# jiahuei/COMIC-Compact-Image-Captioning-with-Attention

Measured on NVIDIA B200. Metric: captions/sec COMIC-256 beam-3, higher is better.
Workload: dtype f32 storage and accumulation; GEMM / conv operands split into 3 bf16 terms on tcgen05 (bf16x3)

## Files before the change

### comic-compact-image-captioning-with-attention_b200/csrc/api.cu

```cuda
#include <stdarg.h>
#include <string.h>

#include <new>

#include "comic_internal.cuh"

namespace comic {

static thread_local char g_err[1024] = "";

void set_error(const char* fmt, ...) {
  va_list ap;
  va_start(ap, fmt);
  vsnprintf(g_err, sizeof(g_err), fmt, ap);
  va_end(ap);
}

}

using namespace comic;

extern "C" const char* comic_last_error(void) { return g_err; }
extern "C" const char* comic_version(void) { return "comic_b200 0.2 (sm_100a; fp32 FFMA + tcgen05 bf16x3)"; }

extern "C" int comic_create(const comic_cfg_t* cfg, comic_handle_t* out) {
  COMIC_REQUIRE(cfg && out, COMIC_E_BADARG, "create: null argument");
  COMIC_REQUIRE(cfg->rnn_size > 0 && cfg->rnn_size % 128 == 0, COMIC_E_UNSUPPORTED,
                "create: rnn_size %d must be a positive multiple of 128", cfg->rnn_size);
  COMIC_REQUIRE(cfg->word_size > 0 && cfg->word_size % 4 == 0, COMIC_E_UNSUPPORTED, "create: word_size %% 4 != 0");
  COMIC_REQUIRE(cfg->num_heads > 0 && cfg->rnn_size % cfg->num_heads == 0 &&
                    (cfg->rnn_size / cfg->num_heads) % 4 == 0,
                COMIC_E_UNSUPPORTED, "create: heads %d incompatible with rnn_size %d", cfg->num_heads, cfg->rnn_size);
  COMIC_REQUIRE(cfg->fm_channels > 0 && cfg->fm_channels % 4 == 0 && cfg->fm_positions > 0, COMIC_E_SHAPE,
                "create: bad feature map %d x %d", cfg->fm_positions, cfg->fm_channels);
  COMIC_REQUIRE(cfg->vocab > 1 && cfg->eos_id >= 0 && cfg->eos_id < cfg->vocab, COMIC_E_SHAPE, "create: bad vocab / eos");
  COMIC_REQUIRE(cfg->fm_projection >= 0 && cfg->fm_projection <= 2, COMIC_E_BADARG, "create: fm_projection");
  COMIC_REQUIRE(cfg->alignment == 0 || cfg->alignment == 1, COMIC_E_BADARG,
                "create: Invalid alignment method.");
  COMIC_REQUIRE(cfg->prob_fn == 0 || cfg->prob_fn == 1, COMIC_E_BADARG, "create: Invalid alignment method.");
  COMIC_REQUIRE(cfg->embed_size % 4 == 0, COMIC_E_SHAPE, "create: embed_size %% 4 != 0");
  comic_handle_s* h = new (std::nothrow) comic_handle_s();
  COMIC_REQUIRE(h, COMIC_E_BADARG, "create: out of host memory");
  h->cfg = *cfg;
  COMIC_CHECK_CUDA(cudaGetDevice(&h->dev));
  cudaDeviceProp prop;
  COMIC_CHECK_CUDA(cudaGetDeviceProperties(&prop, h->dev));
  h->num_sms = prop.multiProcessorCount;
  h->R = cfg->rnn_size; h->W = cfg->word_size; h->H = cfg->num_heads;
  h->C = cfg->fm_channels; h->M = cfg->fm_positions; h->E = cfg->embed_size; h->V = cfg->vocab;
  h->Vp = round_up(h->V, 4);
  h->VAL = (cfg->fm_projection == 0) ? h->C : h->R;
  h->A = (cfg->fm_projection == 0 && !cfg->context_layer) ? h->C : h->R;
  h->LQ = h->Vp + h->R;
  h->KX = h->W + h->A + h->R;
  if (h->VAL % h->H != 0) {
    delete h;
    set_error("create: value width %d not divisible by heads %d", h->VAL, h->H);
    return COMIC_E_SHAPE;
  }
  memset(&h->w, 0, sizeof(h->w));
  int rc = decoder_configure();
  if (rc) { delete h; return rc; }
  if (cudaMallocHost(&h->attn2_host, 16 * sizeof(float)) != cudaSuccess) {
    h->attn2_host = nullptr;
    (void)cudaGetLastError();
  }
  *out = h;
  return COMIC_OK;
}

extern "C" int comic_destroy(comic_handle_t h) {
  if (h && h->prof_ev) {
    for (int i = 0; i < 2 * kMaxProfEvents; ++i) cudaEventDestroy(h->prof_ev[i]);
    delete[] h->prof_ev;
    delete[] h->prof_tag;
  }
  if (h && h->attn2_host) cudaFreeHost(h->attn2_host);
  delete h;
  return COMIC_OK;
}

extern "C" int comic_profile_enable(comic_handle_t h, uint32_t tag_mask) {
  COMIC_REQUIRE(h, COMIC_E_BADARG, "profile_enable: null handle");
  if (tag_mask && !h->prof_ev) {
    h->prof_ev = new cudaEvent_t[2 * kMaxProfEvents];
    h->prof_tag = new int[kMaxProfEvents];
    for (int i = 0; i < 2 * kMaxProfEvents; ++i) COMIC_CHECK_CUDA(cudaEventCreate(&h->prof_ev[i]));
  }
  h->prof_mask = tag_mask;
  h->prof_used = 0;
  return COMIC_OK;
}

extern "C" int comic_profile_read(comic_handle_t h, int tag, double* total_ms, int64_t* count) {
  COMIC_REQUIRE(h && total_ms && count, COMIC_E_BADARG, "profile_read: null argument");
  double tot = 0.0;
  int64_t n = 0;
  for (int i = 0; i < h->prof_used; ++i) {
    if (h->prof_tag[i] != tag) continue;
    COMIC_CHECK_CUDA(cudaEventSynchronize(h->prof_ev[2 * i + 1]));
    float ms = 0.f;
    COMIC_CHECK_CUDA(cudaEventElapsedTime(&ms, h->prof_ev[2 * i], h->prof_ev[2 * i + 1]));
    tot += ms;
    ++n;
  }
  *total_ms = tot;
  *count = n;
  return COMIC_OK;
}

namespace comic {
int pack_tc_weight(comic_handle_t h, Carver& cv, const float* W, int K, int N, int ldw, int cin_src, int cin_dst,
                   tc::TcWeight& out, cudaStream_t st, bool dry, int gate_R) {
  (void)h;
  int ntaps = K / cin_src;
  int Kd = (cin_src == cin_dst) ? K : ntaps * cin_dst;
  out.N = N;
  out.K = Kd;
  out.Npad = round_up(N, 16);
  out.Kpad = round_up(Kd, tc::BK);
  size_t n = (size_t)out.Npad * out.Kpad;
  out.hi = cv.take<uint16_t>(n);
  out.lo = cv.take<uint16_t>(n);
  out.ready = false;
  if (dry) return COMIC_OK;
  tc::pack_bt_kernel<<<(unsigned)((n + 255) / 256), 256, 0, st>>>(W, K, N, ldw, out.hi, out.lo, out.Kpad, out.Npad,
                                                                 cin_src, cin_dst, gate_R);
  COMIC_CHECK_CUDA(cudaGetLastError());
  COMIC_REQUIRE(tc::make_weight_maps(out), COMIC_E_CUDA, "cuTensorMapEncodeTiled failed for a %d x %d weight", N, Kd);
  return COMIC_OK;
}
}

extern "C" int comic_set_precision(comic_handle_t h, int mode) {
  COMIC_REQUIRE(h && mode >= 0 && mode <= 2, COMIC_E_BADARG, "set_precision: mode must be 0 (f32), 1 (split tensor) or 2 (fast)");
  h->precision = mode;
  return COMIC_OK;
}

extern "C" int comic_set_option(comic_handle_t h, int option, int value) {
  COMIC_REQUIRE(h, COMIC_E_BADARG, "set_option: null handle");
  switch (option) {
    case COMIC_OPT_FUSED_ATTN_MIN_IMAGES: h->fused_min_images = value; return COMIC_OK;
    case COMIC_OPT_PERSISTENT_MAX_ROWS: h->persist_max_rows = value; return COMIC_OK;
    case COMIC_OPT_PERSISTENT_TRACE: h->persist_trace = value; return COMIC_OK;
    case COMIC_OPT_PERSISTENT_WATCHDOG_MS:
      if (value < 0) break;
      h->persist_watchdog_ms = value;
      return COMIC_OK;
    case COMIC_OPT_ENC_PLANES: h->enc_planes = value; return COMIC_OK;
    case COMIC_OPT_STEM_S2D: h->stem_s2d = value; return COMIC_OK;
    case COMIC_OPT_TC_MIN_ROWS: h->tc_min_rows = value; return COMIC_OK;
    case COMIC_OPT_TC_SPLITK: h->tc_splitk = value; return COMIC_OK;
    case COMIC_OPT_ATTN2: h->attn2 = value; return COMIC_OK;
    case COMIC_OPT_FUSE_LSTM: h->fuse_lstm = value; return COMIC_OK;
    case COMIC_OPT_TMA_A: h->tma_a = value; return COMIC_OK;
    case COMIC_OPT_GEMM_SMALL_TILES: tc::small_tiles() = value; return COMIC_OK;
    case COMIC_OPT_PDL: pdl_mode() = value; return COMIC_OK;
    case COMIC_OPT_GEMM_RESIDENT_B: tc::bres_mode() = value; return COMIC_OK;
    case COMIC_OPT_GEMM_PAIR: tc::pair_mode() = value; return COMIC_OK;
    case COMIC_OPT_GEMM_PAIR_MIN_TILES: tc::pair_min_tiles() = value; return COMIC_OK;
    case COMIC_OPT_GEMM_MC:
      if (value != 0 && value != 1 && value != 2 && value != 4) break;
      tc::mc_mode() = value;
      return COMIC_OK;
    case COMIC_OPT_ENC_CHUNK_STEM:
    case COMIC_OPT_ENC_CHUNK_28:
    case COMIC_OPT_ENC_CHUNK_14:
      COMIC_REQUIRE(value >= 1, COMIC_E_BADARG, "set_option: encoder chunk must be >= 1");
      h->enc_chunk[option - COMIC_OPT_ENC_CHUNK_STEM] = value;
      return COMIC_OK;
    default: break;
  }
  set_error("set_option: unknown option %d", option);
  return COMIC_E_BADARG;
}

extern "C" int comic_decode_trace(comic_handle_t h, int64_t* out, int max_steps, int* steps, void* stream) {
  COMIC_REQUIRE(h && out && steps, COMIC_E_BADARG, "decode_trace: null argument");
  int n = h->last_trace_steps < max_steps ? h->last_trace_steps : max_steps;
  *steps = n;
  if (n <= 0 || !h->last_trace) { *steps = 0; return COMIC_OK; }
  COMIC_CHECK_CUDA(cudaMemcpyAsync(out, h->last_trace, (size_t)n * 32 * sizeof(int64_t), cudaMemcpyDeviceToHost,
                                   (cudaStream_t)stream));
  COMIC_CHECK_CUDA(cudaStreamSynchronize((cudaStream_t)stream));
  return COMIC_OK;
}

extern "C" int comic_packed_bytes(comic_handle_t h, size_t* bytes) {
  COMIC_REQUIRE(h && bytes, COMIC_E_BADARG, "packed_bytes: null argument");
  Carver cv(nullptr);
  comic::Packed keep = h->pk;
  decoder_pack(h, cv, 0, true);
  encoder_pack(h, cv, 0, true);
  h->pk = keep;
  *bytes = cv.off + 256;
  return COMIC_OK;
}

extern "C" int comic_bind_weights(comic_handle_t h, const comic_weights_t* w, int with_cnn, void* packed,
                                  size_t packed_bytes, void* stream) {
  COMIC_REQUIRE(h && w && packed, COMIC_E_BADARG, "bind_weights: null argument");
  size_t need;
  comic_packed_bytes(h, &need);
  COMIC_REQUIRE(packed_bytes >= need, COMIC_E_WORKSPACE, "bind_weights: packed buffer %zu < %zu", packed_bytes, need);
  COMIC_REQUIRE(w->lstm_kernel && w->lstm_bias && w->init_weight && w->memory_kernel && w->query_kernel &&
                    w->out_kernel && w->out_bias && w->embedding_map,
                COMIC_E_BADARG, "bind_weights: missing decoder tensor");
  if (h->cfg.alignment == 0)
    COMIC_REQUIRE(w->attention_v && w->ln_gamma && w->ln_beta && w->temperature, COMIC_E_BADARG,
                  "bind_weights: missing add_LN attention tensor");
  if (h->cfg.fm_projection == 2) COMIC_REQUIRE(w->value_kernel, COMIC_E_BADARG, "bind_weights: missing value_layer");
  if (h->cfg.context_layer) COMIC_REQUIRE(w->a_layer, COMIC_E_BADARG, "bind_weights: missing a_layer");
  if (with_cnn) {
    for (int i = 0; i < COMIC_NUM_CONVS; ++i)
      COMIC_REQUIRE(w->conv_w[i] && w->bn_beta[i] && w->bn_mean[i] && w->bn_var[i], COMIC_E_BADARG,
                    "bind_weights: missing CNN tensor %d", i);
    if (h->cfg.legacy)
      COMIC_REQUIRE(w->enc_ln_gamma && w->enc_ln_beta && w->enc_embed_weight, COMIC_E_BADARG,
                    "bind_weights: missing legacy encoder head");
  }
  h->w = *w;
  cudaStream_t st = (cudaStream_t)stream;
  Carver cv(packed);
  int rc = decoder_pack(h, cv, st, false);
  if (rc) return rc;
  rc = encoder_pack(h, cv, st, !with_cnn);
  if (rc) return rc;
  h->bound = true;
  h->attn2_state = 0;
  h->cnn_bound = with_cnn != 0;
  return COMIC_OK;
}

extern "C" int comic_workspace_bytes(comic_handle_t h, int mode, int B, int k, int T, size_t* bytes) {
  COMIC_REQUIRE(h && bytes, COMIC_E_BADARG, "workspace_bytes: null argument");
  COMIC_REQUIRE(B > 0 && k > 0 && T >= 0, COMIC_E_SHAPE, "workspace_bytes: bad B=%d k=%d T=%d", B, k, T);
  if (mode == 0) return encoder_workspace_bytes(h, B, bytes);
  if (mode == 5) {
    *bytes = 2 * (size_t)round_up(B, 16) * round_up(k, tc::BK) * sizeof(float) + 2048;
    return COMIC_OK;
  }
  return decoder_workspace_bytes(h, mode, B, k, T, bytes);
}

extern "C" int comic_encode_fwd(comic_handle_t h, const float* images, int B, float* fm_out, float* im_embed_out,
                                float* mixed5c_out, void* ws, size_t ws_bytes, void* stream) {
  COMIC_REQUIRE(h && images && fm_out && im_embed_out && ws, COMIC_E_BADARG, "encode_fwd: null argument");
  COMIC_REQUIRE(B > 0, COMIC_E_SHAPE, "encode_fwd: bad batch %d", B);
  return encoder_forward(h, images, B, fm_out, im_embed_out, mixed5c_out, ws, ws_bytes, (cudaStream_t)stream);
}

extern "C" int comic_gemm_f32(comic_handle_t h, const float* A, int lda, const float* Bm, int ldb, const float* bias,
                              float* C, int ldc, int M, int N, int K, void* ws, size_t ws_bytes, void* stream) {
  COMIC_REQUIRE(h && A && Bm && C, COMIC_E_BADARG, "gemm_f32: null argument");
  COMIC_REQUIRE(M > 0 && N > 0 && K > 0, COMIC_E_SHAPE, "gemm_f32: bad shape");
  COMIC_REQUIRE(N % 4 == 0 && ldb % 4 == 0 && ldc % 4 == 0, COMIC_E_UNSUPPORTED, "gemm_f32: N, ldb, ldc must be multiples of 4");
  APlain a{};
  a.nseg = 1;
  a.seg[0] = ASeg{A, nullptr, lda, K, M};
  Epi e{};
  e.bias = bias;
  e.nroute = 1;
  e.r[0] = Route{0, N, C, ldc, 0};
  e.stop_n = 0x7fffffff;
  GemmPlan p = plan_gemm(M, N, K, h->num_sms, false);
  cudaError_t err;
  if (h->precision >= 1 && M >= 128 && K % 4 == 0 && lda % 4 == 0) {
    size_t need = 2 * (size_t)round_up(N, 16) * round_up(K, tc::BK) * sizeof(float) + 1024;
    COMIC_REQUIRE(ws && ws_bytes >= need, COMIC_E_WORKSPACE, "gemm_f32: tensor path needs %zu workspace bytes", need);
    Carver cv(ws);
    tc::TcWeight tw;
    int rc = pack_tc_weight(h, cv, Bm, K, N, ldb, 1, 1, tw, (cudaStream_t)stream, false);
    if (rc) return rc;
    err = tc::launch_gemm_tc<0>(a, tw, M, N, e, h->num_sms, (cudaStream_t)stream);
    h->launches += 2;
    COMIC_CHECK_CUDA(err);
    return COMIC_OK;
  }
  if (K % 4 == 0 && lda % 4 == 0) err = launch_gemm<0, 4>(a, Bm, ldb, M, N, K, e, p, (cudaStream_t)stream);
  else err = launch_gemm<0, 1>(a, Bm, ldb, M, N, K, e, p, (cudaStream_t)stream);
  h->launches++;
  COMIC_CHECK_CUDA(err);
  return COMIC_OK;
}

extern "C" int comic_launch_count(comic_handle_t h, int64_t* count) {
  COMIC_REQUIRE(h && count, COMIC_E_BADARG, "launch_count: null argument");
  *count = h->launches;
  return COMIC_OK;
}
```

### comic-compact-image-captioning-with-attention_b200/csrc/comic_internal.cuh

```cuda
#pragma once
#include <cuda_runtime.h>
#include <stdint.h>
#include <stdio.h>
#include <string>

#include "../../include/comic_b200.h"
#include "gemm_f32.cuh"
#include "gemm_tc.cuh"

namespace comic {

void set_error(const char* fmt, ...);

#define COMIC_CHECK_CUDA(expr)                                                         \
  do {                                                                                 \
    cudaError_t _e = (expr);                                                           \
    if (_e != cudaSuccess) {                                                           \
      comic::set_error("%s:%d CUDA error %s: %s", __FILE__, __LINE__, #expr,           \
                       cudaGetErrorString(_e));                                        \
      return COMIC_E_CUDA;                                                             \
    }                                                                                  \
  } while (0)

#define COMIC_REQUIRE(cond, code, ...)                                                 \
  do {                                                                                 \
    if (!(cond)) {                                                                     \
      comic::set_error(__VA_ARGS__);                                                   \
      return (code);                                                                   \
    }                                                                                  \
  } while (0)

struct BlockDesc {
  int cin, b0, b1a, b1b, b2a, b2b, b3;
  int conv[6];
};

constexpr int kNumBlocks = 9;

struct Packed {
  float* outq = nullptr;
  float* outq_bias = nullptr;
  float* bn_scale[COMIC_NUM_CONVS];
  float* bn_shift[COMIC_NUM_CONVS];
  float* grp_w[kNumBlocks];
  float* grp_scale[kNumBlocks];
  float* grp_shift[kNumBlocks];
  tc::TcWeight tc_conv[COMIC_NUM_CONVS];
  tc::TcWeight tc_grp[kNumBlocks];
  tc::TcWeight tc_lstm, tc_outq, tc_mem, tc_val, tc_init;
  tc::TcWeight tc_lstm_il;
  float* lstm_bias_il = nullptr;
  tc::TcWeight tc_stem_s2d;
};

}

namespace comic {
enum Tag { T_CONV = 0, T_POOL, T_PROJECT, T_INIT, T_GATES, T_LSTM, T_LQ, T_SCORES, T_CTX, T_BEAM, T_FINAL, T_MISC, T_PERSIST, T_COUNT };
constexpr int kMaxProfEvents = 16384;
}

struct comic_handle_s {
  comic_cfg_t cfg;
  int dev = 0;
  int num_sms = 148;
  int R, W, H, C, M, E, V, Vp, A, VAL, LQ, KX;
  comic_weights_t w;
  bool bound = false, cnn_bound = false;
  int precision = 1;
  int fused_min_images = 48;
  int attn2_min_images = 12;
  int fuse_lstm = 0;
  int tma_a = 1;
  int attn2 = 1;
  int attn2_state = 0;
  float* attn2_host = nullptr;
  int persist_trace = 0;
  long long* last_trace = nullptr;
  int last_trace_steps = 0;
  int persist_watchdog_ms = 2000;
  int persist_max_rows = 32;
  int tc_splitk = 3;
  int tc_min_rows = 64;
  int stem_s2d = 2;
  int enc_planes = 0;
  int enc_chunk[3] = {256, 512, 512};
  comic::Packed pk;
  int64_t launches = 0;
  uint32_t prof_mask = 0;
  cudaEvent_t* prof_ev = nullptr;
  int* prof_tag = nullptr;
  int prof_used = 0;
};

namespace comic {
struct Prof {
  comic_handle_t h;
  cudaStream_t st;
  int slot;
  Prof(comic_handle_t h_, int tag, cudaStream_t st_, int n = 1) : h(h_), st(st_), slot(-1) {
    h->launches += n;
    if (((h->prof_mask >> tag) & 1u) && h->prof_ev && h->prof_used < kMaxProfEvents) {
      slot = h->prof_used++;
      h->prof_tag[slot] = tag;
      cudaEventRecord(h->prof_ev[2 * slot], st);
    }
  }
  ~Prof() {
    if (slot >= 0) cudaEventRecord(h->prof_ev[2 * slot + 1], st);
  }
};
}

namespace comic {

struct Carver {
  char* base;
  size_t off = 0;
  explicit Carver(void* b) : base(static_cast<char*>(b)) {}
  template <typename T>
  T* take(size_t n) {
    size_t bytes = (n * sizeof(T) + 255) & ~size_t(255);
    T* p = base ? reinterpret_cast<T*>(base + off) : nullptr;
    off += bytes;
    return p;
  }
};

inline int round_up(int x, int m) { return (x + m - 1) / m * m; }

int pack_tc_weight(comic_handle_t h, Carver& cv, const float* W, int K, int N, int ldw, int cin_src, int cin_dst,
                   tc::TcWeight& out, cudaStream_t st, bool dry, int gate_R = 0);
inline bool use_tc(comic_handle_t h, const tc::TcWeight& w, int M) { return h->precision >= 1 && w.ready && M >= h->tc_min_rows; }
inline int tc_ksplit_shape(int num_sms, int M, int N, int K) {
  const int nk = (K + 63) / 64, tiles = ((M + 127) / 128) * ((N + 127) / 128);
  int ks = num_sms / tiles;
  if (ks > nk / 2) ks = nk / 2;
  if (ks > 8) ks = 8;
  return ks < 2 ? 1 : ks;
}
inline int tc_ksplit(comic_handle_t h, int M, int N, int K, int which) {
  if (!(h->tc_splitk & which)) return 1;
  if (which == 2 && M > 128) return 1;
  return tc_ksplit_shape(h->num_sms, M, N, K);
}
inline bool use_tc_step(comic_handle_t h, const tc::TcWeight& w, int M, int N, int K, int which) {
  return use_tc(h, w, M) || (h->precision >= 1 && w.ready && M > 32 && tc_ksplit(h, M, N, K, which) > 1);
}

int encoder_workspace_bytes(comic_handle_t h, int B, size_t* bytes);
int encoder_forward(comic_handle_t h, const float* images, int B, float* fm_out, float* im_embed_out,
                    float* mixed5c_out, void* ws, size_t ws_bytes, cudaStream_t st);
int encoder_pack(comic_handle_t h, Carver& cv, cudaStream_t st, bool dry);
const BlockDesc* block_table();
const comic_conv_desc_t* conv_table();
struct EncBufs {
  float *a, *b, *t1, *t2, *p;
};
void same_pads(int n, int k, int s, int* out, int* before);
int run_conv(comic_handle_t h, const float* x, int B, int H, int W, int ldx, int ci, float* dst, int ld_dst, int coff,
             int* Ho_out, int* Wo_out, cudaStream_t st);
int run_maxpool(comic_handle_t h, const float* x, float* y, int B, int H, int W, int C, int k, int s, int* Ho_out,
                int* Wo_out, cudaStream_t st);
void run_pad_c3_c4(comic_handle_t h, const float* img, float* dst, size_t npix, cudaStream_t st);
void run_avgpool_global(comic_handle_t h, const float* x, float* y, int B, int HW, int C, cudaStream_t st);
int run_block(comic_handle_t h, int bi, const float* x, float* y, int B, int S, EncBufs& eb, cudaStream_t st);

struct StepBufs {
  float* gates;
  float* lq_part;
  float* lq;
  float* scores;
  float* xdense;
  float* ctxraw;
  float* kstats;
  float* abound;
  float* a2_scratch;
  int* a2_counters;
  uint16_t *xp_hi, *xp_lo;
  uint16_t *hp_hi, *hp_lo;
  ATma xmaps, hmaps;
  bool tma_a;
};

struct StepIO {
  const float* keys;
  const float* values;
  const int* tok;
  const int* src;
  int src_limit;
  const float* c_prev;
  const float* h_prev;
  const float* ctx_prev;
  float* c_new;
  float* h_new;
  float* h_drop;
  float* ctx_new;
  float* hist_t;
  float* hist_scale;
  const float* in_mask; const float* out_mask; const float* att_mask;
  float in_keep, out_keep, att_keep;
  const int* fin_count; int t; int n_rows;
  float* gates_save; float* alpha_pre; int force_dense;
  int no_fused;
  const float* kstats; const float* abound;
  float* a2_scratch; int* a2_counters;
};

int run_step(comic_handle_t h, const StepIO& io, const StepBufs& sb, int B, int k, cudaStream_t st);
int attn2_prepare(comic_handle_t h, StepIO& io, const StepBufs& sb, int B, int k, bool masks, cudaStream_t st);
void carve_step(comic_handle_t h, Carver& cv, int N, StepBufs& sb, bool train_masks);
int decoder_workspace_bytes(comic_handle_t h, int mode, int B, int k, int T, size_t* bytes);
int decoder_pack(comic_handle_t h, Carver& cv, cudaStream_t st, bool dry);
int decoder_configure();

struct PersistCall {
  const float *keys, *values, *c0, *h0;
  int B, k, max_it, greedy;
  float lpw;
  float *c[2], *h[2], *ctx[2];
  float *lq, *scores, *hist;
  int *tok, *src;
  float* cum;
  uint8_t* fin;
  long long* len;
  int* fin_count;
  int *step_ids, *parents;
  float* sc;
  float* logits_out;
  unsigned* bar;
  long long* trace;
  float* part;
};
bool persist_applicable(comic_handle_t h, int B, int k, bool greedy);
int decode_persistent(comic_handle_t h, const PersistCall& pc, cudaStream_t st);

}
```

### comic-compact-image-captioning-with-attention_b200/csrc/encoder.cu

```cuda
#include "comic_internal.cuh"
#include <algorithm>

namespace comic {

static const comic_conv_desc_t kConvs[COMIC_NUM_CONVS] = {
    {7, 2, 3, 64},   {1, 1, 64, 64},  {3, 1, 64, 192},
    {1, 1, 192, 64}, {1, 1, 192, 96}, {3, 1, 96, 128}, {1, 1, 192, 16}, {3, 1, 16, 32}, {1, 1, 192, 32},
    {1, 1, 256, 128}, {1, 1, 256, 128}, {3, 1, 128, 192}, {1, 1, 256, 32}, {3, 1, 32, 96}, {1, 1, 256, 64},
    {1, 1, 480, 192}, {1, 1, 480, 96}, {3, 1, 96, 208}, {1, 1, 480, 16}, {3, 1, 16, 48}, {1, 1, 480, 64},
    {1, 1, 512, 160}, {1, 1, 512, 112}, {3, 1, 112, 224}, {1, 1, 512, 24}, {3, 1, 24, 64}, {1, 1, 512, 64},
    {1, 1, 512, 128}, {1, 1, 512, 128}, {3, 1, 128, 256}, {1, 1, 512, 24}, {3, 1, 24, 64}, {1, 1, 512, 64},
    {1, 1, 512, 112}, {1, 1, 512, 144}, {3, 1, 144, 288}, {1, 1, 512, 32}, {3, 1, 32, 64}, {1, 1, 512, 64},
    {1, 1, 528, 256}, {1, 1, 528, 160}, {3, 1, 160, 320}, {1, 1, 528, 32}, {3, 1, 32, 128}, {1, 1, 528, 128},
    {1, 1, 832, 256}, {1, 1, 832, 160}, {3, 1, 160, 320}, {1, 1, 832, 32}, {3, 1, 32, 128}, {1, 1, 832, 128},
    {1, 1, 832, 384}, {1, 1, 832, 192}, {3, 1, 192, 384}, {1, 1, 832, 48}, {3, 1, 48, 128}, {1, 1, 832, 128},
};

static BlockDesc make_block(int first) {
  BlockDesc b;
  b.cin = kConvs[first].c_in;
  b.b0 = kConvs[first].c_out;
  b.b1a = kConvs[first + 1].c_out;
  b.b1b = kConvs[first + 2].c_out;
  b.b2a = kConvs[first + 3].c_out;
  b.b2b = kConvs[first + 4].c_out;
  b.b3 = kConvs[first + 5].c_out;
  for (int i = 0; i < 6; ++i) b.conv[i] = first + i;
  return b;
}

static BlockDesc kBlocks[kNumBlocks];
static bool kBlocksInit = false;

const BlockDesc* block_table() {
  if (!kBlocksInit) {
    for (int i = 0; i < kNumBlocks; ++i) kBlocks[i] = make_block(3 + 6 * i);
    kBlocksInit = true;
  }
  return kBlocks;
}

const comic_conv_desc_t* conv_table() { return kConvs; }

__global__ void bn_fold_kernel(const float* __restrict__ beta, const float* __restrict__ mean,
                               const float* __restrict__ var, float* __restrict__ scale,
                               float* __restrict__ shift, int n, float eps) {
  int i = blockIdx.x * blockDim.x + threadIdx.x;
  if (i < n) {
    float s = 1.0f / sqrtf(var[i] + eps);
    scale[i] = s;
    shift[i] = beta[i] - mean[i] * s;
  }
}

__global__ void copy_cols_kernel(const float* __restrict__ src, int rows, int cols, float* __restrict__ dst,
                                 int ld, int coff) {
  int i = blockIdx.x * blockDim.x + threadIdx.x;
  if (i < rows * cols) {
    int r = i / cols, c = i - r * cols;
    dst[(size_t)r * ld + coff + c] = src[i];
  }
}

__global__ void pack_stem_s2d_kernel(const float* __restrict__ W, uint16_t* __restrict__ hi, uint16_t* __restrict__ lo);

int encoder_pack(comic_handle_t h, Carver& cv, cudaStream_t st, bool dry) {
  const BlockDesc* blk = block_table();
  for (int i = 0; i < COMIC_NUM_CONVS; ++i) {
    h->pk.bn_scale[i] = cv.take<float>(kConvs[i].c_out);
    h->pk.bn_shift[i] = cv.take<float>(kConvs[i].c_out);
  }
  for (int b = 0; b < kNumBlocks; ++b) {
    int ng = blk[b].b0 + blk[b].b1a + blk[b].b2a;
    h->pk.grp_w[b] = cv.take<float>((size_t)blk[b].cin * ng);
    h->pk.grp_scale[b] = cv.take<float>(ng);
    h->pk.grp_shift[b] = cv.take<float>(ng);
  }
  for (int i = 0; i < COMIC_NUM_CONVS; ++i) {
    bool grouped = false;
    for (int b = 0; b < kNumBlocks; ++b)
      if (i == blk[b].conv[0] || i == blk[b].conv[1] || i == blk[b].conv[3]) grouped = true;
    if (grouped) continue;
    const comic_conv_desc_t& d = kConvs[i];
    int K = d.k * d.k * d.c_in;
    int cdst = (d.c_in == 3) ? 4 : d.c_in;
    int rc = pack_tc_weight(h, cv, dry ? nullptr : h->w.conv_w[i], K, d.c_out, d.c_out, d.c_in, cdst,
                            h->pk.tc_conv[i], st, dry);
    if (rc) return rc;
  }
  for (int b = 0; b < kNumBlocks; ++b) {
    h->pk.tc_grp[b].hi = cv.take<uint16_t>((size_t)round_up(blk[b].b0 + blk[b].b1a + blk[b].b2a, 16) *
                                        round_up(blk[b].cin, tc::BK));
    h->pk.tc_grp[b].lo = cv.take<uint16_t>((size_t)round_up(blk[b].b0 + blk[b].b1a + blk[b].b2a, 16) *
                                        round_up(blk[b].cin, tc::BK));
  }
  {
    tc::TcWeight& tw = h->pk.tc_stem_s2d;
    tw.N = 64; tw.K = 256; tw.Npad = 64; tw.Kpad = 256;
    tw.hi = cv.take<uint16_t>(64 * 256);
    tw.lo = cv.take<uint16_t>(64 * 256);
    tw.ready = false;
  }
  if (dry) return COMIC_OK;
  pack_stem_s2d_kernel<<<(64 * 256 + 255) / 256, 256, 0, st>>>(h->w.conv_w[0], h->pk.tc_stem_s2d.hi, h->pk.tc_stem_s2d.lo);
  COMIC_REQUIRE(tc::make_weight_maps(h->pk.tc_stem_s2d), COMIC_E_CUDA, "cuTensorMapEncodeTiled failed (stem panel)");
  for (int i = 0; i < COMIC_NUM_CONVS; ++i) {
    int n = kConvs[i].c_out;
    bn_fold_kernel<<<(n + 255) / 256, 256, 0, st>>>(h->w.bn_beta[i], h->w.bn_mean[i], h->w.bn_var[i],
                                                   h->pk.bn_scale[i], h->pk.bn_shift[i], n, 1e-3f);
  }
  for (int b = 0; b < kNumBlocks; ++b) {
    int ng = blk[b].b0 + blk[b].b1a + blk[b].b2a;
    int src_conv[3] = {blk[b].conv[0], blk[b].conv[1], blk[b].conv[3]};
    int coff = 0;
    for (int j = 0; j < 3; ++j) {
      int ci = src_conv[j];
      int n = kConvs[ci].c_out;
      int tot = blk[b].cin * n;
      copy_cols_kernel<<<(tot + 255) / 256, 256, 0, st>>>(h->w.conv_w[ci], blk[b].cin, n, h->pk.grp_w[b], ng, coff);
      copy_cols_kernel<<<(n + 255) / 256, 256, 0, st>>>(h->pk.bn_scale[ci], 1, n, h->pk.grp_scale[b], ng, coff);
      copy_cols_kernel<<<(n + 255) / 256, 256, 0, st>>>(h->pk.bn_shift[ci], 1, n, h->pk.grp_shift[b], ng, coff);
      coff += n;
    }
    tc::TcWeight& tw = h->pk.tc_grp[b];
    tw.N = ng; tw.K = blk[b].cin; tw.Npad = round_up(ng, 16); tw.Kpad = round_up(blk[b].cin, tc::BK);
    size_t n = (size_t)tw.Npad * tw.Kpad;
    tc::pack_bt_kernel<<<(unsigned)((n + 255) / 256), 256, 0, st>>>(h->pk.grp_w[b], blk[b].cin, ng, ng, tw.hi, tw.lo,
                                                                   tw.Kpad, tw.Npad, 1, 1);
    COMIC_REQUIRE(tc::make_weight_maps(tw), COMIC_E_CUDA, "cuTensorMapEncodeTiled failed (grouped panel %d)", b);
  }
  COMIC_CHECK_CUDA(cudaGetLastError());
  return COMIC_OK;
}

__global__ void pad_c3_c4_kernel(const float* __restrict__ x, float* __restrict__ y, size_t npix) {
  size_t i = (size_t)blockIdx.x * blockDim.x + threadIdx.x;
  if (i < npix) {
    float4 v = make_float4(x[i * 3 + 0], x[i * 3 + 1], x[i * 3 + 2], 0.f);
    reinterpret_cast<float4*>(y)[i] = v;
  }
}


__global__ void __launch_bounds__(256)
s2d_split_kernel(const float* __restrict__ x, uint16_t* __restrict__ hi, uint16_t* __restrict__ lo, size_t npix2) {
  size_t i = (size_t)blockIdx.x * 256 + threadIdx.x;
  if (i >= npix2) return;
  const size_t j2 = i % 112, t = i / 112;
  const size_t i2 = t % 112, n = t / 112;
  const float* r0 = x + ((n * 224 + 2 * i2) * 224 + 2 * j2) * 3;
  const float* r1 = r0 + 224 * 3;
  float v[16];
#pragma unroll
  for (int q = 0; q < 6; ++q) { v[q] = __ldg(r0 + q); v[6 + q] = __ldg(r1 + q); }
  v[12] = v[13] = v[14] = v[15] = 0.f;
  uint2 h[4], l[4];
#pragma unroll
  for (int q = 0; q < 4; ++q) tc::split4(make_float4(v[4 * q], v[4 * q + 1], v[4 * q + 2], v[4 * q + 3]), h[q], l[q]);
  uint4* ph = reinterpret_cast<uint4*>(hi + i * 16);
  uint4* pl = reinterpret_cast<uint4*>(lo + i * 16);
  ph[0] = make_uint4(h[0].x, h[0].y, h[1].x, h[1].y);
  ph[1] = make_uint4(h[2].x, h[2].y, h[3].x, h[3].y);
  pl[0] = make_uint4(l[0].x, l[0].y, l[1].x, l[1].y);
  pl[1] = make_uint4(l[2].x, l[2].y, l[3].x, l[3].y);
}

__global__ void pack_stem_s2d_kernel(const float* __restrict__ W, uint16_t* __restrict__ hi, uint16_t* __restrict__ lo) {
  int i = blockIdx.x * blockDim.x + threadIdx.x;
  if (i >= 64 * 256) return;
  const int n = i / 256, kp = i % 256;
  const int di = kp / 64, dj = (kp / 16) % 4, ch = kp % 16;
  float v = 0.f;
  if (ch < 12) {
    const int a = ch / 6, b = (ch / 3) % 2, c = ch % 3;
    const int kh = 2 * di + a, kw = 2 * dj + b;
    if (kh < 7 && kw < 7) v = W[((kh * 7 + kw) * 3 + c) * 64 + n];
  }
  uint32_t h = tc::pack_bf16x2(v, 0.f) & 0xffffu;
  float hf = __uint_as_float(h << 16);
  uint32_t l = tc::pack_bf16x2(v - hf, 0.f) & 0xffffu;
  hi[i] = (uint16_t)h;
  lo[i] = (uint16_t)l;
}

template <int K>
__global__ void __launch_bounds__(256)
maxpool_nhwc_kernel(const float* __restrict__ x, float* __restrict__ y, unsigned total, int H, int W, int C4,
                    int stride, int pad_t, int pad_l, int Ho, int Wo) {
  unsigned i = blockIdx.x * 256u + threadIdx.x;
  if (i >= total) return;
  unsigned c4 = i % (unsigned)C4, p = i / (unsigned)C4;
  unsigned wo = p % (unsigned)Wo, q = p / (unsigned)Wo;
  unsigned ho = q % (unsigned)Ho, b = q / (unsigned)Ho;
  const int h0 = (int)ho * stride - pad_t, w0 = (int)wo * stride - pad_l;
  const float4* xb = reinterpret_cast<const float4*>(x) + (size_t)b * H * W * C4 + c4;
  float4 v[K * K];
#pragma unroll
  for (int dh = 0; dh < K; ++dh) {
#pragma unroll
    for (int dw = 0; dw < K; ++dw) {
      const int hi = h0 + dh, wi = w0 + dw;
      const bool ok = hi >= 0 && hi < H && wi >= 0 && wi < W;
      v[dh * K + dw] = ok ? __ldg(xb + ((size_t)hi * W + wi) * C4)
                          : make_float4(-INFINITY, -INFINITY, -INFINITY, -INFINITY);
    }
  }
  float4 m = v[0];
#pragma unroll
  for (int j = 1; j < K * K; ++j) {
    m.x = fmaxf(m.x, v[j].x); m.y = fmaxf(m.y, v[j].y); m.z = fmaxf(m.z, v[j].z); m.w = fmaxf(m.w, v[j].w);
  }
  reinterpret_cast<float4*>(y)[(size_t)p * C4 + c4] = m;
}


template <int ROWS>
__global__ void __launch_bounds__(256)
maxpool3s1_rows_kernel(const float* __restrict__ x, float* __restrict__ y, unsigned total, int H, int W, int C4, int HB) {
  const unsigned i = blockIdx.x * 256u + threadIdx.x;
  if (i >= total) return;
  const unsigned c4 = i % (unsigned)C4, q = i / (unsigned)C4;
  const int hb = (int)(q % (unsigned)HB);
  const unsigned b = q / (unsigned)HB;
  const int ho0 = hb * ROWS;
  const float4* xb = reinterpret_cast<const float4*>(x) + (size_t)b * H * W * C4 + c4;
  float4* yb = reinterpret_cast<float4*>(y) + (size_t)b * H * W * C4 + c4;
  const float4 ninf = make_float4(-INFINITY, -INFINITY, -INFINITY, -INFINITY);
  auto mx = [](const float4& a, const float4& c) {
    return make_float4(fmaxf(a.x, c.x), fmaxf(a.y, c.y), fmaxf(a.z, c.z), fmaxf(a.w, c.w));
  };
  bool ok[ROWS + 2];
#pragma unroll
  for (int j = 0; j < ROWS + 2; ++j) ok[j] = (ho0 - 1 + j) >= 0 && (ho0 - 1 + j) < H;
  float4 p1[ROWS], p2[ROWS];
#pragma unroll
  for (int o = 0; o < ROWS; ++o) { p1[o] = ninf; p2[o] = ninf; }
#pragma unroll 4
  for (int w = 0; w <= W; ++w) {
    float4 cm[ROWS];
    if (w < W) {
      float4 r[ROWS + 2];
#pragma unroll
      for (int j = 0; j < ROWS + 2; ++j)
        r[j] = ok[j] ? __ldg(xb + ((size_t)(ho0 - 1 + j) * W + w) * C4) : ninf;
#pragma unroll
      for (int o = 0; o < ROWS; ++o) cm[o] = mx(mx(r[o], r[o + 1]), r[o + 2]);
    } else {
#pragma unroll
      for (int o = 0; o < ROWS; ++o) cm[o] = ninf;
    }
    if (w >= 1) {
#pragma unroll
      for (int o = 0; o < ROWS; ++o)
        if (ho0 + o < H) yb[((size_t)(ho0 + o) * W + (w - 1)) * C4] = mx(mx(p2[o], p1[o]), cm[o]);
    }
#pragma unroll
    for (int o = 0; o < ROWS; ++o) { p2[o] = p1[o]; p1[o] = cm[o]; }
  }
}


struct Planes {
  uint16_t* hi;
  uint16_t* lo;
};

static inline Planes planes_of(float* buf, size_t cap_elems) {
  Planes p;
  p.hi = reinterpret_cast<uint16_t*>(buf);
  p.lo = p.hi + cap_elems;
  return p;
}
static inline Planes planes_at(Planes p, size_t off) { return Planes{p.hi + off, p.lo + off}; }

__device__ __forceinline__ void unpack8(const uint4& h, const uint4& l, float (&v)[8]) {
  const uint32_t hw[4] = {h.x, h.y, h.z, h.w}, lw[4] = {l.x, l.y, l.z, l.w};
#pragma unroll
  for (int j = 0; j < 4; ++j) {
    v[2 * j] = __uint_as_float(hw[j] << 16) + __uint_as_float(lw[j] << 16);
    v[2 * j + 1] = __uint_as_float(hw[j] & 0xffff0000u) + __uint_as_float(lw[j] & 0xffff0000u);
  }
}

template <int K, bool IN_F32>
__global__ void __launch_bounds__(256)
maxpool_planes_kernel(const uint16_t* __restrict__ xh, const uint16_t* __restrict__ xl, const float* __restrict__ xf,
                      uint16_t* __restrict__ yh, uint16_t* __restrict__ yl, unsigned total, int H, int W, int C8,
                      int stride, int pad_t, int pad_l, int Ho, int Wo) {
  unsigned i = blockIdx.x * 256u + threadIdx.x;
  if (i >= total) return;
  unsigned c8 = i % (unsigned)C8, p = i / (unsigned)C8;
  unsigned wo = p % (unsigned)Wo, q = p / (unsigned)Wo;
  unsigned ho = q % (unsigned)Ho, b = q / (unsigned)Ho;
  const int h0 = (int)ho * stride - pad_t, w0 = (int)wo * stride - pad_l;
  const size_t base = (size_t)b * H * W * C8 + c8;
  float m[8];
#pragma unroll
  for (int j = 0; j < 8; ++j) m[j] = -INFINITY;
  if (IN_F32) {
    float4 va[K * K], vb[K * K];
    const float4* xb = reinterpret_cast<const float4*>(xf) + base * 2;
#pragma unroll
    for (int dh = 0; dh < K; ++dh)
#pragma unroll
      for (int dw = 0; dw < K; ++dw) {
        const int hi = h0 + dh, wi = w0 + dw;
        const bool ok = hi >= 0 && hi < H && wi >= 0 && wi < W;
        const float4 ninf = make_float4(-INFINITY, -INFINITY, -INFINITY, -INFINITY);
        va[dh * K + dw] = ok ? __ldg(xb + ((size_t)hi * W + wi) * C8 * 2) : ninf;
        vb[dh * K + dw] = ok ? __ldg(xb + ((size_t)hi * W + wi) * C8 * 2 + 1) : ninf;
      }
#pragma unroll
    for (int t = 0; t < K * K; ++t) {
      m[0] = fmaxf(m[0], va[t].x); m[1] = fmaxf(m[1], va[t].y); m[2] = fmaxf(m[2], va[t].z); m[3] = fmaxf(m[3], va[t].w);
      m[4] = fmaxf(m[4], vb[t].x); m[5] = fmaxf(m[5], vb[t].y); m[6] = fmaxf(m[6], vb[t].z); m[7] = fmaxf(m[7], vb[t].w);
    }
  } else {
    uint4 vh[K * K], vl[K * K];
    bool okv[K * K];
    const uint4* hb = reinterpret_cast<const uint4*>(xh) + base;
    const uint4* lb = reinterpret_cast<const uint4*>(xl) + base;
#pragma unroll
    for (int dh = 0; dh < K; ++dh)
#pragma unroll
      for (int dw = 0; dw < K; ++dw) {
        const int hi = h0 + dh, wi = w0 + dw;
        const bool ok = hi >= 0 && hi < H && wi >= 0 && wi < W;
        okv[dh * K + dw] = ok;
        const size_t o = ok ? ((size_t)hi * W + wi) * C8 : 0;
        vh[dh * K + dw] = __ldg(hb + o);
        vl[dh * K + dw] = __ldg(lb + o);
      }
#pragma unroll
    for (int t = 0; t < K * K; ++t) {
      float v[8];
      unpack8(vh[t], vl[t], v);
      if (okv[t]) {
#pragma unroll
        for (int j = 0; j < 8; ++j) m[j] = fmaxf(m[j], v[j]);
      }
    }
  }
  uint2 h0p, l0p, h1p, l1p;
  tc::split4(make_float4(m[0], m[1], m[2], m[3]), h0p, l0p);
  tc::split4(make_float4(m[4], m[5], m[6], m[7]), h1p, l1p);
  reinterpret_cast<uint4*>(yh)[(size_t)p * C8 + c8] = make_uint4(h0p.x, h0p.y, h1p.x, h1p.y);
  reinterpret_cast<uint4*>(yl)[(size_t)p * C8 + c8] = make_uint4(l0p.x, l0p.y, l1p.x, l1p.y);
}

__global__ void avgpool_global_kernel(const float* __restrict__ x, float* __restrict__ y, int B, int HW, int C) {
  int i = blockIdx.x * blockDim.x + threadIdx.x;
  if (i >= B * C) return;
  int b = i / C, c = i - b * C;
  float s = 0.f;
  for (int p = 0; p < HW; ++p) s += x[((size_t)b * HW + p) * C + c];
  y[i] = s / (float)HW;
}

__global__ void ln_tanh_rows_kernel(const float* __restrict__ x, const float* __restrict__ gamma,
                                    const float* __restrict__ beta, float* __restrict__ y, int n, float eps) {
  __shared__ float red[32];
  int row = blockIdx.x;
  const float* xr = x + (size_t)row * n;
  float s = 0.f;
  for (int i = threadIdx.x; i < n; i += blockDim.x) s += xr[i];
  for (int o = 16; o; o >>= 1) s += __shfl_xor_sync(0xffffffffu, s, o);
  if ((threadIdx.x & 31) == 0) red[threadIdx.x >> 5] = s;
  __syncthreads();
  float tot = 0.f;
  for (int i = 0; i < (int)(blockDim.x >> 5); ++i) tot += red[i];
  float mean = tot / n;
  __syncthreads();
  float v = 0.f;
  for (int i = threadIdx.x; i < n; i += blockDim.x) { float d = xr[i] - mean; v += d * d; }
  for (int o = 16; o; o >>= 1) v += __shfl_xor_sync(0xffffffffu, v, o);
  if ((threadIdx.x & 31) == 0) red[threadIdx.x >> 5] = v;
  __syncthreads();
  float vt = 0.f;
  for (int i = 0; i < (int)(blockDim.x >> 5); ++i) vt += red[i];
  float rstd = 1.0f / sqrtf(vt / n + eps);
  for (int i = threadIdx.x; i < n; i += blockDim.x) {
    float inv = rstd * gamma[i];
    y[(size_t)row * n + i] = tanhf(xr[i] * inv + (beta[i] - mean * inv));
  }
}

void same_pads(int n, int k, int s, int* out, int* before) {
  *out = (n + s - 1) / s;
  int pad = (*out - 1) * s + k - n;
  if (pad < 0) pad = 0;
  *before = pad / 2;
}

struct EncPlan {
  int cs, c3, c4;
  size_t ab, t1, t2, p, p2, p3, head;
};

static EncPlan enc_plan(comic_handle_t h, int B) {
  EncPlan pl;
  pl.cs = B < h->enc_chunk[0] ? B : h->enc_chunk[0];
  pl.c3 = B < h->enc_chunk[1] ? B : h->enc_chunk[1];
  pl.c4 = B < h->enc_chunk[2] ? B : h->enc_chunk[2];
  auto mx = [](size_t x, size_t y) { return x > y ? x : y; };
  pl.ab = mx(mx((size_t)pl.cs * 112 * 112 * 64, (size_t)pl.c3 * 28 * 28 * 480), (size_t)pl.c4 * 14 * 14 * 832);
  pl.t1 = mx((size_t)pl.c3 * 28 * 28 * 128, (size_t)pl.c4 * 14 * 14 * 192);
  pl.t2 = mx((size_t)pl.c3 * 28 * 28 * 32, (size_t)pl.c4 * 14 * 14 * 48);
  pl.p = mx((size_t)pl.c3 * 28 * 28 * 256, (size_t)pl.c4 * 14 * 14 * 832);
  pl.p2 = (size_t)B * 28 * 28 * 192;
  pl.p3 = (size_t)B * 14 * 14 * 480;
  pl.head = (size_t)pl.c4 * 1024;
  return pl;
}

int encoder_workspace_bytes(comic_handle_t h, int B, size_t* bytes) {
  EncPlan pl = enc_plan(h, B);
  Carver cv(nullptr);
  cv.take<float>(pl.ab); cv.take<float>(pl.ab); cv.take<float>(pl.t1); cv.take<float>(pl.t2); cv.take<float>(pl.p);
  cv.take<float>(pl.p2); cv.take<float>(pl.p3); cv.take<float>(pl.head);
  *bytes = cv.off;
  return COMIC_OK;
}

int run_conv(comic_handle_t h, const float* x, int B, int H, int W, int ldx, int ci, float* dst,
                    int ld_dst, int coff, int* Ho_out, int* Wo_out, cudaStream_t st) {
  const comic_conv_desc_t& d = kConvs[ci];
  AConv a;
  a.x = x; a.H = H; a.W = W; a.Cin = (d.c_in == 3 && ldx == 4) ? 4 : d.c_in; a.ldx = ldx;
  a.KH = d.k; a.KW = d.k; a.stride = d.stride;
  same_pads(H, d.k, d.stride, &a.Ho, &a.pad_t);
  same_pads(W, d.k, d.stride, &a.Wo, &a.pad_l);
  int M = B * a.Ho * a.Wo, N = d.c_out, K = d.k * d.k * d.c_in;
  Epi e{};
  e.bias = h->pk.bn_shift[ci];
  e.scale = h->pk.bn_scale[ci];
  e.relu = 1;
  e.nroute = 1;
  e.r[0] = Route{0, N, dst, ld_dst, coff};
  e.split_stride = 0;
  GemmPlan p = plan_gemm(M, N, K, h->num_sms, false);
  cudaError_t err;
  if (use_tc(h, h->pk.tc_conv[ci], M) && a.Cin % 4 == 0) {
    Prof pf(h, T_CONV, st);
    err = tc::launch_gemm_tc<1>(a, h->pk.tc_conv[ci], M, N, e, h->num_sms, st);
  } else {
    Prof pf(h, T_CONV, st);
    if (d.c_in % 4 == 0) err = launch_gemm<1, 4>(a, h->w.conv_w[ci], N, M, N, K, e, p, st);
    else err = launch_gemm<1, 1>(a, h->w.conv_w[ci], N, M, N, K, e, p, st);
  }
  COMIC_CHECK_CUDA(err);
  if (Ho_out) *Ho_out = a.Ho;
  if (Wo_out) *Wo_out = a.Wo;
  return COMIC_OK;
}

int run_maxpool(comic_handle_t h, const float* x, float* y, int B, int H, int W, int C, int k, int s,
                       int* Ho_out, int* Wo_out, cudaStream_t st) {
  int Ho, Wo, pt, pl;
  same_pads(H, k, s, &Ho, &pt);
  same_pads(W, k, s, &Wo, &pl);
  size_t total = (size_t)B * Ho * Wo * (C / 4);
  COMIC_REQUIRE(total < 0xffffffffull && C % 4 == 0 && (k == 2 || k == 3), COMIC_E_UNSUPPORTED,
                "maxpool: unsupported shape (total %zu, C %d, k %d)", total, C, k);
  unsigned grid = (unsigned)((total + 255) / 256);
  {
    Prof pf(h, T_POOL, st);
    if (k == 3 && s == 1) {
      const int HB = (H + 1) / 2;
      const size_t tot = (size_t)B * HB * (C / 4);
      maxpool3s1_rows_kernel<2><<<(unsigned)((tot + 255) / 256), 256, 0, st>>>(x, y, (unsigned)tot, H, W, C / 4, HB);
    } else if (k == 3)
      maxpool_nhwc_kernel<3><<<grid, 256, 0, st>>>(x, y, (unsigned)total, H, W, C / 4, s, pt, pl, Ho, Wo);
    else
      maxpool_nhwc_kernel<2><<<grid, 256, 0, st>>>(x, y, (unsigned)total, H, W, C / 4, s, pt, pl, Ho, Wo);
  }
  COMIC_CHECK_CUDA(cudaGetLastError());
  if (Ho_out) *Ho_out = Ho;
  if (Wo_out) *Wo_out = Wo;
  return COMIC_OK;
}

void run_pad_c3_c4(comic_handle_t h, const float* img, float* dst, size_t npix, cudaStream_t st) {
  Prof pf(h, T_POOL, st);
  pad_c3_c4_kernel<<<(unsigned)((npix + 255) / 256), 256, 0, st>>>(img, dst, npix);
}

void run_avgpool_global(comic_handle_t h, const float* x, float* y, int B, int HW, int C, cudaStream_t st) {
  Prof pf(h, T_POOL, st);
  avgpool_global_kernel<<<(B * C + 255) / 256, 256, 0, st>>>(x, y, B, HW, C);
}

int run_block(comic_handle_t h, int bi, const float* x, float* y, int B, int S, EncBufs& eb,
                     cudaStream_t st) {
  const BlockDesc& bd = block_table()[bi];
  int cout = bd.b0 + bd.b1b + bd.b2b + bd.b3;
  int M = B * S * S;
  {
    APlain a{};
    a.nseg = 1;
    a.seg[0] = ASeg{x, nullptr, bd.cin, bd.cin, M};
    int ng = bd.b0 + bd.b1a + bd.b2a;
    Epi e{};
    e.bias = h->pk.grp_shift[bi];
    e.scale = h->pk.grp_scale[bi];
    e.relu = 1;
    e.nroute = 3;
    e.r[0] = Route{0, bd.b0, y, cout, 0};
    e.r[1] = Route{bd.b0, bd.b0 + bd.b1a, eb.t1, bd.b1a, 0};
    e.r[2] = Route{bd.b0 + bd.b1a, ng, eb.t2, bd.b2a, 0};
    GemmPlan p = plan_gemm(M, ng, bd.cin, h->num_sms, false);
    cudaError_t err;
    {
      Prof pf(h, T_CONV, st);
      if (use_tc(h, h->pk.tc_grp[bi], M)) err = tc::launch_gemm_tc<0>(a, h->pk.tc_grp[bi], M, ng, e, h->num_sms, st);
      else err = launch_gemm<0, 4>(a, h->pk.grp_w[bi], ng, M, ng, bd.cin, e, p, st);
    }
    COMIC_CHECK_CUDA(err);
  }
  int rc;
  if ((rc = run_conv(h, eb.t1, B, S, S, bd.b1a, bd.conv[2], y, cout, bd.b0, nullptr, nullptr, st))) return rc;
  if ((rc = run_conv(h, eb.t2, B, S, S, bd.b2a, bd.conv[4], y, cout, bd.b0 + bd.b1b, nullptr, nullptr, st))) return rc;
  if ((rc = run_maxpool(h, x, eb.p, B, S, S, bd.cin, 3, 1, nullptr, nullptr, st))) return rc;
  if ((rc = run_conv(h, eb.p, B, S, S, bd.cin, bd.conv[5], y, cout, bd.b0 + bd.b1b + bd.b2b, nullptr, nullptr, st))) return rc;
  return COMIC_OK;
}


static int run_maxpool_p(comic_handle_t h, Planes x, const float* xf, Planes y, int B, int H, int W, int C, int k, int s,
                         cudaStream_t st) {
  int Ho, Wo, pt, pl;
  same_pads(H, k, s, &Ho, &pt);
  same_pads(W, k, s, &Wo, &pl);
  size_t total = (size_t)B * Ho * Wo * (C / 8);
  COMIC_REQUIRE(total < 0xffffffffull && C % 8 == 0 && (k == 2 || k == 3), COMIC_E_UNSUPPORTED,
                "maxpool (planes): unsupported shape (total %zu, C %d, k %d)", total, C, k);
  unsigned grid = (unsigned)((total + 255) / 256);
  {
    Prof pf(h, T_POOL, st);
    if (xf) {
      if (k == 3) maxpool_planes_kernel<3, true><<<grid, 256, 0, st>>>(nullptr, nullptr, xf, y.hi, y.lo, (unsigned)total, H, W, C / 8, s, pt, pl, Ho, Wo);
      else maxpool_planes_kernel<2, true><<<grid, 256, 0, st>>>(nullptr, nullptr, xf, y.hi, y.lo, (unsigned)total, H, W, C / 8, s, pt, pl, Ho, Wo);
    } else {
      if (k == 3) maxpool_planes_kernel<3, false><<<grid, 256, 0, st>>>(x.hi, x.lo, nullptr, y.hi, y.lo, (unsigned)total, H, W, C / 8, s, pt, pl, Ho, Wo);
      else maxpool_planes_kernel<2, false><<<grid, 256, 0, st>>>(x.hi, x.lo, nullptr, y.hi, y.lo, (unsigned)total, H, W, C / 8, s, pt, pl, Ho, Wo);
    }
  }
  COMIC_CHECK_CUDA(cudaGetLastError());
  return COMIC_OK;
}

static int run_conv_p(comic_handle_t h, Planes x, int B, int H, int W, int ldx, int ci, float* dst, Planes dp, int ld_dst,
                      int coff, cudaStream_t st) {
  const comic_conv_desc_t& d = kConvs[ci];
  AConvP a;
  a.hi = x.hi; a.lo = x.lo; a.H = H; a.W = W; a.Cin = d.c_in; a.ldx = ldx;
  a.KH = d.k; a.KW = d.k; a.stride = d.stride;
  same_pads(H, d.k, d.stride, &a.Ho, &a.pad_t);
  same_pads(W, d.k, d.stride, &a.Wo, &a.pad_l);
  int M = B * a.Ho * a.Wo, N = d.c_out;
  Epi e{};
  e.bias = h->pk.bn_shift[ci];
  e.scale = h->pk.bn_scale[ci];
  e.relu = 1;
  e.nroute = 1;
  e.r[0] = Route{0, N, dst, ld_dst, coff, dp.hi, dp.lo};
  cudaError_t err;
  {
    Prof pf(h, T_CONV, st);
    err = tc::launch_gemm_tc<2>(a, h->pk.tc_conv[ci], M, N, e, h->num_sms, st);
  }
  COMIC_CHECK_CUDA(err);
  return COMIC_OK;
}

static int run_stem_s2d(comic_handle_t h, const float* img, int nb, float* scratch, float* dst, uint16_t* dhi,
                        uint16_t* dlo, cudaStream_t st) {
  const size_t npix2 = (size_t)nb * 112 * 112;
  uint16_t* xh = reinterpret_cast<uint16_t*>(scratch);
  uint16_t* xl = xh + npix2 * 16;
  {
    Prof pf(h, T_POOL, st);
    s2d_split_kernel<<<(unsigned)((npix2 + 255) / 256), 256, 0, st>>>(img, xh, xl, npix2);
  }
  AConvP a;
  a.hi = xh; a.lo = xl; a.H = 112; a.W = 112; a.Cin = 16; a.ldx = 16;
  a.KH = 4; a.KW = 4; a.stride = 1; a.pad_t = 1; a.pad_l = 1; a.Ho = 112; a.Wo = 112;
  Epi e{};
  e.bias = h->pk.bn_shift[0]; e.scale = h->pk.bn_scale[0]; e.relu = 1; e.nroute = 1;
  e.r[0] = Route{0, 64, dst, 64, 0, dhi, dlo};
  cudaError_t err;
  {
    Prof pf(h, T_CONV, st);
    if (h->stem_s2d >= 2) {
      AHalo ah;
      ah.hi = xh; ah.lo = xl; ah.nimg = nb;
      err = tc::launch_stem_halo(ah, h->pk.tc_stem_s2d, e, h->num_sms, st);
    } else {
      err = tc::launch_gemm_tc<2>(a, h->pk.tc_stem_s2d, nb * 112 * 112, 64, e, h->num_sms, st);
    }
  }
  COMIC_CHECK_CUDA(err);
  return COMIC_OK;
}

struct PBufs {
  Planes t1, t2, p;
};

static int run_block_p(comic_handle_t h, int bi, Planes x, float* y32, Planes yp, int B, int S, const PBufs& pb,
                       cudaStream_t st) {
  const BlockDesc& bd = block_table()[bi];
  int cout = bd.b0 + bd.b1b + bd.b2b + bd.b3;
  int M = B * S * S;
  {
    AConvP a;
    a.hi = x.hi; a.lo = x.lo; a.H = S; a.W = S; a.Cin = bd.cin; a.ldx = bd.cin;
    a.KH = 1; a.KW = 1; a.stride = 1; a.pad_t = 0; a.pad_l = 0; a.Ho = S; a.Wo = S;
    int ng = bd.b0 + bd.b1a + bd.b2a;
    Epi e{};
    e.bias = h->pk.grp_shift[bi];
    e.scale = h->pk.grp_scale[bi];
    e.relu = 1;
    e.nroute = 3;
    e.r[0] = Route{0, bd.b0, y32, cout, 0, yp.hi, yp.lo};
    e.r[1] = Route{bd.b0, bd.b0 + bd.b1a, nullptr, bd.b1a, 0, pb.t1.hi, pb.t1.lo};
    e.r[2] = Route{bd.b0 + bd.b1a, ng, nullptr, bd.b2a, 0, pb.t2.hi, pb.t2.lo};
    cudaError_t err;
    {
      Prof pf(h, T_CONV, st);
      err = tc::launch_gemm_tc<2>(a, h->pk.tc_grp[bi], M, ng, e, h->num_sms, st);
    }
    COMIC_CHECK_CUDA(err);
  }
  int rc;
  if ((rc = run_conv_p(h, pb.t1, B, S, S, bd.b1a, bd.conv[2], y32, yp, cout, bd.b0, st))) return rc;
  if ((rc = run_conv_p(h, pb.t2, B, S, S, bd.b2a, bd.conv[4], y32, yp, cout, bd.b0 + bd.b1b, st))) return rc;
  if ((rc = run_maxpool_p(h, x, nullptr, pb.p, B, S, S, bd.cin, 3, 1, st))) return rc;
  if ((rc = run_conv_p(h, pb.p, B, S, S, bd.cin, bd.conv[5], y32, yp, cout, bd.b0 + bd.b1b + bd.b2b, st))) return rc;
  return COMIC_OK;
}

static int encoder_forward_planes(comic_handle_t h, const float* images, int B, float* fm_out, float* im_embed_out,
                                  float* mixed5c_out, void* ws, cudaStream_t st) {
  const EncPlan pl = enc_plan(h, B);
  Carver cv(ws);
  float* fa = cv.take<float>(pl.ab);
  float* fb = cv.take<float>(pl.ab);
  float* ft1 = cv.take<float>(pl.t1);
  float* ft2 = cv.take<float>(pl.t2);
  float* fp = cv.take<float>(pl.p);
  float* fpool2 = cv.take<float>(pl.p2);
  float* fpool3 = cv.take<float>(pl.p3);
  cv.take<float>(pl.head);
  const Planes pa = planes_of(fa, pl.ab), pbn = planes_of(fb, pl.ab);
  PBufs pb;
  pb.t1 = planes_of(ft1, pl.t1); pb.t2 = planes_of(ft2, pl.t2); pb.p = planes_of(fp, pl.p);
  const Planes pool2 = planes_of(fpool2, pl.p2), pool3 = planes_of(fpool3, pl.p3);
  const Planes none{nullptr, nullptr};
  int rc;
  for (int b0 = 0; b0 < B; b0 += pl.cs) {
    int nb = (B - b0 < pl.cs) ? (B - b0) : pl.cs;
    const float* img = images + (size_t)b0 * 224 * 224 * 3;
    if (h->stem_s2d) {
      if ((rc = run_stem_s2d(h, img, nb, fb, nullptr, pa.hi, pa.lo, st))) return rc;
    } else {
      run_pad_c3_c4(h, img, fb, (size_t)nb * 224 * 224, st);
      const comic_conv_desc_t& d = kConvs[0];
      AConv a;
      a.x = fb; a.H = 224; a.W = 224; a.Cin = 4; a.ldx = 4; a.KH = d.k; a.KW = d.k; a.stride = d.stride;
      same_pads(224, d.k, d.stride, &a.Ho, &a.pad_t);
      same_pads(224, d.k, d.stride, &a.Wo, &a.pad_l);
      Epi e{};
      e.bias = h->pk.bn_shift[0]; e.scale = h->pk.bn_scale[0]; e.relu = 1; e.nroute = 1;
      e.r[0] = Route{0, 64, nullptr, 64, 0, pa.hi, pa.lo};
      cudaError_t err;
      {
        Prof pf(h, T_CONV, st);
        err = tc::launch_gemm_tc<1>(a, h->pk.tc_conv[0], nb * 112 * 112, 64, e, h->num_sms, st);
      }
      COMIC_CHECK_CUDA(err);
    }
    if ((rc = run_maxpool_p(h, pa, nullptr, pbn, nb, 112, 112, 64, 3, 2, st))) return rc;
    if ((rc = run_conv_p(h, pbn, nb, 56, 56, 64, 1, nullptr, pa, 64, 0, st))) return rc;
    if ((rc = run_conv_p(h, pa, nb, 56, 56, 64, 2, nullptr, pbn, 192, 0, st))) return rc;
    if ((rc = run_maxpool_p(h, pbn, nullptr, planes_at(pool2, (size_t)b0 * 28 * 28 * 192), nb, 56, 56, 192, 3, 2, st)))
      return rc;
  }
  for (int b0 = 0; b0 < B; b0 += pl.c3) {
    int nb = (B - b0 < pl.c3) ? (B - b0) : pl.c3;
    if ((rc = run_block_p(h, 0, planes_at(pool2, (size_t)b0 * 28 * 28 * 192), nullptr, pbn, nb, 28, pb, st))) return rc;
    if ((rc = run_block_p(h, 1, pbn, nullptr, pa, nb, 28, pb, st))) return rc;
    if ((rc = run_maxpool_p(h, pa, nullptr, planes_at(pool3, (size_t)b0 * 14 * 14 * 480), nb, 28, 28, 480, 3, 2, st)))
      return rc;
  }
  for (int b0 = 0; b0 < B; b0 += pl.c4) {
    int nb = (B - b0 < pl.c4) ? (B - b0) : pl.c4;
    if ((rc = run_block_p(h, 2, planes_at(pool3, (size_t)b0 * 14 * 14 * 480), nullptr, pa, nb, 14, pb, st))) return rc;
    if ((rc = run_block_p(h, 3, pa, nullptr, pbn, nb, 14, pb, st))) return rc;
    if ((rc = run_block_p(h, 4, pbn, nullptr, pa, nb, 14, pb, st))) return rc;
    if ((rc = run_block_p(h, 5, pa, nullptr, pbn, nb, 14, pb, st))) return rc;
    float* fm = fm_out + (size_t)b0 * 196 * 832;
    if ((rc = run_block_p(h, 6, pbn, fm, none, nb, 14, pb, st))) return rc;
    if ((rc = run_maxpool_p(h, none, fm, pa, nb, 14, 14, 832, 2, 2, st))) return rc;
    if ((rc = run_block_p(h, 7, pa, nullptr, pbn, nb, 7, pb, st))) return rc;
    float* m5c = mixed5c_out ? mixed5c_out + (size_t)b0 * 49 * 1024 : fa;
    if ((rc = run_block_p(h, 8, pbn, m5c, none, nb, 7, pb, st))) return rc;
    run_avgpool_global(h, m5c, im_embed_out + (size_t)b0 * 1024, nb, 49, 1024, st);
    COMIC_CHECK_CUDA(cudaGetLastError());
  }
  return COMIC_OK;
}

int encoder_forward(comic_handle_t h, const float* images, int B, float* fm_out, float* im_embed_out,
                    float* mixed5c_out, void* ws, size_t ws_bytes, cudaStream_t st) {
  COMIC_REQUIRE(h->cnn_bound, COMIC_E_BADARG, "encode_fwd: CNN weights not bound");
  COMIC_REQUIRE(h->C == 832, COMIC_E_UNSUPPORTED, "encode_fwd: only cnn_fm_attention=Mixed_4f (C=832) is built");
  size_t need;
  encoder_workspace_bytes(h, B, &need);
  COMIC_REQUIRE(ws_bytes >= need, COMIC_E_WORKSPACE, "encode_fwd: workspace %zu < %zu", ws_bytes, need);
  const EncPlan pl = enc_plan(h, B);
  {
    auto tail = [](int n, int c) { return n % c ? n % c : c; };
    const int min_imgs = std::min(std::min(tail(B, pl.cs), tail(B, pl.c3)), tail(B, pl.c4));
    if (h->precision >= 1 && h->enc_planes && !h->cfg.legacy && h->pk.tc_conv[0].ready && min_imgs * 49 >= 128)
      return encoder_forward_planes(h, images, B, fm_out, im_embed_out, mixed5c_out, ws, st);
  }
  Carver cv(ws);
  EncBufs eb;
  eb.a = cv.take<float>(pl.ab); eb.b = cv.take<float>(pl.ab);
  eb.t1 = cv.take<float>(pl.t1); eb.t2 = cv.take<float>(pl.t2); eb.p = cv.take<float>(pl.p);
  float* pool2 = cv.take<float>(pl.p2);
  float* pool3 = cv.take<float>(pl.p3);
  float* head = cv.take<float>(pl.head);
  int rc;
  for (int b0 = 0; b0 < B; b0 += pl.cs) {
    int nb = (B - b0 < pl.cs) ? (B - b0) : pl.cs;
    const float* img = images + (size_t)b0 * 224 * 224 * 3;
    int Ho, Wo;
    if (use_tc(h, h->pk.tc_stem_s2d, nb * 112 * 112) && h->stem_s2d) {
      if ((rc = run_stem_s2d(h, img, nb, eb.b, eb.a, nullptr, nullptr, st))) return rc;
    } else if (use_tc(h, h->pk.tc_conv[0], nb * 112 * 112)) {
      size_t npix = (size_t)nb * 224 * 224;
      {
        Prof pf(h, T_POOL, st);
        pad_c3_c4_kernel<<<(unsigned)((npix + 255) / 256), 256, 0, st>>>(img, eb.b, npix);
      }
      if ((rc = run_conv(h, eb.b, nb, 224, 224, 4, 0, eb.a, 64, 0, &Ho, &Wo, st))) return rc;
    } else {
      if ((rc = run_conv(h, img, nb, 224, 224, 3, 0, eb.a, 64, 0, &Ho, &Wo, st))) return rc;
    }
    if ((rc = run_maxpool(h, eb.a, eb.b, nb, 112, 112, 64, 3, 2, &Ho, &Wo, st))) return rc;
    if ((rc = run_conv(h, eb.b, nb, 56, 56, 64, 1, eb.a, 64, 0, nullptr, nullptr, st))) return rc;
    if ((rc = run_conv(h, eb.a, nb, 56, 56, 64, 2, eb.b, 192, 0, nullptr, nullptr, st))) return rc;
    if ((rc = run_maxpool(h, eb.b, pool2 + (size_t)b0 * 28 * 28 * 192, nb, 56, 56, 192, 3, 2, nullptr, nullptr, st)))
      return rc;
  }
  for (int b0 = 0; b0 < B; b0 += pl.c3) {
    int nb = (B - b0 < pl.c3) ? (B - b0) : pl.c3;
    if ((rc = run_block(h, 0, pool2 + (size_t)b0 * 28 * 28 * 192, eb.b, nb, 28, eb, st))) return rc;
    if ((rc = run_block(h, 1, eb.b, eb.a, nb, 28, eb, st))) return rc;
    if ((rc = run_maxpool(h, eb.a, pool3 + (size_t)b0 * 14 * 14 * 480, nb, 28, 28, 480, 3, 2, nullptr, nullptr, st)))
      return rc;
  }
  for (int b0 = 0; b0 < B; b0 += pl.c4) {
    int nb = (B - b0 < pl.c4) ? (B - b0) : pl.c4;
    if ((rc = run_block(h, 2, pool3 + (size_t)b0 * 14 * 14 * 480, eb.a, nb, 14, eb, st))) return rc;
    if ((rc = run_block(h, 3, eb.a, eb.b, nb, 14, eb, st))) return rc;
    if ((rc = run_block(h, 4, eb.b, eb.a, nb, 14, eb, st))) return rc;
    if ((rc = run_block(h, 5, eb.a, eb.b, nb, 14, eb, st))) return rc;
    float* fm = fm_out + (size_t)b0 * 196 * 832;
    if ((rc = run_block(h, 6, eb.b, fm, nb, 14, eb, st))) return rc;
    if ((rc = run_maxpool(h, fm, eb.a, nb, 14, 14, 832, 2, 2, nullptr, nullptr, st))) return rc;
    if ((rc = run_block(h, 7, eb.a, eb.b, nb, 7, eb, st))) return rc;
    float* m5c = mixed5c_out ? mixed5c_out + (size_t)b0 * 49 * 1024 : eb.a;
    if ((rc = run_block(h, 8, eb.b, m5c, nb, 7, eb, st))) return rc;
    float* emb = im_embed_out + (size_t)b0 * 1024;
    if (!h->cfg.legacy) {
      Prof pf(h, T_POOL, st);
      avgpool_global_kernel<<<(nb * 1024 + 255) / 256, 256, 0, st>>>(m5c, emb, nb, 49, 1024);
    } else {
      avgpool_global_kernel<<<(nb * 1024 + 255) / 256, 256, 0, st>>>(m5c, head, nb, 49, 1024);
      ln_tanh_rows_kernel<<<nb, 256, 0, st>>>(head, h->w.enc_ln_gamma, h->w.enc_ln_beta, eb.t1, 1024, 1e-12f);
      h->launches += 2;
      APlain a{};
      a.nseg = 1;
      a.seg[0] = ASeg{eb.t1, nullptr, 1024, 1024, nb};
      Epi e{};
      e.nroute = 1;
      e.r[0] = Route{0, 1024, emb, 1024, 0};
      GemmPlan p = plan_gemm(nb, 1024, 1024, h->num_sms, false);
      cudaError_t err;
      {
        Prof pf(h, T_MISC, st);
        err = launch_gemm<0, 4>(a, h->w.enc_embed_weight, 1024, nb, 1024, 1024, e, p, st);
      }
      COMIC_CHECK_CUDA(err);
    }
    COMIC_CHECK_CUDA(cudaGetLastError());
  }
  return COMIC_OK;
}

}

namespace comic {
__global__ void __launch_bounds__(256)
preprocess_eval_kernel(const uint8_t* __restrict__ img, int B, int H, int W, int RS, int out_h, int out_w,
                       float* __restrict__ out, const int* __restrict__ crop_yx = nullptr,
                       const uint8_t* __restrict__ flip = nullptr) {
  const size_t i = (size_t)blockIdx.x * blockDim.x + threadIdx.x;
  if (i >= (size_t)B * out_h * out_w) return;
  const int x = (int)(i % out_w), y = (int)((i / out_w) % out_h), b = (int)(i / ((size_t)out_w * out_h));
  int ry = (out_h <= RS) ? y + (RS - out_h) / 2 : y - (out_h - RS) / 2;
  int rx = (out_w <= RS) ? x + (RS - out_w) / 2 : x - (out_w - RS) / 2;
  if (crop_yx != nullptr) {
    ry = y + crop_yx[2 * b];
    rx = x + crop_yx[2 * b + 1];
    if (flip != nullptr && flip[b]) rx = RS - 1 - rx;
  }
  float v[3] = {0.f, 0.f, 0.f};
  if (ry >= 0 && ry < RS && rx >= 0 && rx < RS) {
    const float sy = (float)H / (float)RS, sx = (float)W / (float)RS;
    const float fy = __fmul_rn((float)ry, sy), fx = __fmul_rn((float)rx, sx);
    const int y0 = (int)floorf(fy), x0 = (int)floorf(fx);
    const int y1 = min(y0 + 1, H - 1), x1 = min(x0 + 1, W - 1);
    const float ly = __fsub_rn(fy, (float)y0), lx = __fsub_rn(fx, (float)x0);
    const uint8_t* p = img + (size_t)b * H * W * 3;
    const float k = 1.0f / 255.0f;
#pragma unroll
    for (int c = 0; c < 3; ++c) {
      const float tl = (float)p[((size_t)y0 * W + x0) * 3 + c] * k, tr = (float)p[((size_t)y0 * W + x1) * 3 + c] * k;
      const float bl = (float)p[((size_t)y1 * W + x0) * 3 + c] * k, br = (float)p[((size_t)y1 * W + x1) * 3 + c] * k;
      const float top = __fadd_rn(tl, __fmul_rn(__fsub_rn(tr, tl), lx)), bot = __fadd_rn(bl, __fmul_rn(__fsub_rn(br, bl), lx));
      v[c] = __fadd_rn(top, __fmul_rn(__fsub_rn(bot, top), ly));
    }
  }
  float* o = out + i * 3;
#pragma unroll
  for (int c = 0; c < 3; ++c) o[c] = __fmul_rn(__fsub_rn(v[c], 0.5f), 2.0f);
}
}

extern "C" int comic_preprocess_eval(comic_handle_t h, const uint8_t* images, int B, int H, int W, int out_h,
                                     int out_w, float* out, void* stream) {
  COMIC_REQUIRE(h && images && out, COMIC_E_BADARG, "preprocess_eval: null argument");
  COMIC_REQUIRE(B > 0 && H > 0 && W > 0 && out_h > 0 && out_w > 0, COMIC_E_SHAPE,
                "preprocess_eval: bad shape B=%d H=%d W=%d out=%dx%d", B, H, W, out_h, out_w);
  const size_t n = (size_t)B * out_h * out_w;
  comic::preprocess_eval_kernel<<<(unsigned)((n + 255) / 256), 256, 0, (cudaStream_t)stream>>>(images, B, H, W, 256,
                                                                                            out_h, out_w, out);
  h->launches++;
  COMIC_CHECK_CUDA(cudaGetLastError());
  return COMIC_OK;
}

extern "C" int comic_preprocess_train(comic_handle_t h, const uint8_t* images, int B, int H, int W, int out_h, int out_w,
                                      const int32_t* crop_yx, const uint8_t* flip, float* out, void* stream) {
  COMIC_REQUIRE(h && images && out && crop_yx, COMIC_E_BADARG, "preprocess_train: null argument");
  COMIC_REQUIRE(B > 0 && H > 0 && W > 0 && out_h > 0 && out_w > 0 && out_h <= 256 && out_w <= 256, COMIC_E_SHAPE,
                "preprocess_train: bad shape B=%d H=%d W=%d out=%dx%d (tf.random_crop needs out <= 256)", B, H, W, out_h,
                out_w);
  const size_t n = (size_t)B * out_h * out_w;
  comic::preprocess_eval_kernel<<<(unsigned)((n + 255) / 256), 256, 0, (cudaStream_t)stream>>>(images, B, H, W, 256,
                                                                                            out_h, out_w, out, crop_yx, flip);
  h->launches++;
  COMIC_CHECK_CUDA(cudaGetLastError());
  return COMIC_OK;
}

extern "C" const comic_conv_desc_t* comic_conv_table(void) { return comic::conv_table(); }
```

### comic-compact-image-captioning-with-attention_b200/csrc/gemm_f32.cuh

```cuda
#pragma once
#include <cuda.h>

#include "pdl.cuh"
#include <cuda_runtime.h>
#include <stdint.h>

namespace comic {

struct PerDeviceOnce {
  bool done[64] = {};
  template <typename F>
  cudaError_t operator()(F&& configure) {
    int dev = 0;
    cudaError_t e = cudaGetDevice(&dev);
    if (e != cudaSuccess) return e;
    if (dev < 0 || dev >= 64) return configure();
    if (done[dev]) return cudaSuccess;
    e = configure();
    if (e == cudaSuccess) done[dev] = true;
    return e;
  }
};


struct ASeg {
  const float* ptr;
  const int* idx;
  int ld;
  int ncols;
  int idx_limit;
};

struct APlain {
  ASeg seg[3];
  int nseg;
};

struct AConv {
  const float* x;
  int H, W, Cin, ldx;
  int KH, KW, stride, pad_t, pad_l, Ho, Wo;
};

struct Route {
  int n0, n1;
  float* dst;
  int ld;
  int coff;
  uint16_t* hi;
  uint16_t* lo;
};

struct Epi {
  const float* bias;
  const float* scale;
  int relu;
  int nroute;
  Route r[3];
  long long split_stride;
  int ksplit;
  const int* stop;
  int stop_n;
  int pdl;
  const float* lstm_c_prev;
  const int* lstm_src;
  int lstm_src_limit;
  float* lstm_c;
  float* lstm_h;
  int lstm_R;
};

template <bool FAST>
__device__ __forceinline__ float sig_(float x) {
  if (FAST) return __frcp_rn(1.0f + __expf(-x));
  return 1.0f / (1.0f + expf(-x));
}
template <bool FAST>
__device__ __forceinline__ float tanh_(float x) {
  if (FAST) {
    const float e = __expf(-2.0f * fabsf(x));
    return copysignf((1.0f - e) * __frcp_rn(1.0f + e), x);
  }
  return tanhf(x);
}

struct AConvP {
  const uint16_t* hi;
  const uint16_t* lo;
  int H, W, Cin, ldx;
  int KH, KW, stride, pad_t, pad_l, Ho, Wo;
};

struct AHalo {
  const uint16_t* hi;
  const uint16_t* lo;
  int nimg;
};

template <int AMODE> struct AParam;
template <> struct AParam<0> { typedef APlain type; };
template <> struct AParam<1> { typedef AConv type; };
template <> struct AParam<2> { typedef AConvP type; };
template <> struct AParam<3> { typedef AHalo type; };
struct ATma {
  CUtensorMap hi, lo;
};
template <> struct AParam<4> { typedef ATma type; };

__device__ __forceinline__ float4 ldg4(const float* p) {
  return __ldg(reinterpret_cast<const float4*>(p));
}

template <int AMODE> struct RowCtx;
template <> struct RowCtx<0> {
  const float* base[3];
  bool valid;
};
template <> struct RowCtx<1> {
  const float* base;
  int hi0, wi0;
  bool valid;
};

template <int AMODE>
__device__ __forceinline__ void make_row(const typename AParam<AMODE>::type& a, int m, int M,
                                         RowCtx<AMODE>& rc);

template <>
__device__ __forceinline__ void make_row<0>(const APlain& a, int m, int M, RowCtx<0>& rc) {
  rc.valid = m < M;
#pragma unroll
  for (int s = 0; s < 3; ++s) {
    rc.base[s] = nullptr;
    if (s < a.nseg && rc.valid) {
      int r = m;
      if (a.seg[s].idx) r = a.seg[s].idx[m];
      if (r >= 0 && r < a.seg[s].idx_limit) rc.base[s] = a.seg[s].ptr + (size_t)r * a.seg[s].ld;
    }
  }
}

template <>
__device__ __forceinline__ void make_row<1>(const AConv& a, int m, int M, RowCtx<1>& rc) {
  rc.valid = m < M;
  int hw = a.Ho * a.Wo;
  int b = rc.valid ? m / hw : 0;
  int rem = rc.valid ? m - b * hw : 0;
  int ho = rem / a.Wo;
  int wo = rem - ho * a.Wo;
  rc.hi0 = ho * a.stride - a.pad_t;
  rc.wi0 = wo * a.stride - a.pad_l;
  rc.base = a.x + (size_t)b * a.H * a.W * a.ldx;
}

template <int AMODE, int VEC>
__device__ __forceinline__ float4 load_a4(const typename AParam<AMODE>::type& a,
                                          const RowCtx<AMODE>& rc, int kk, int K);

template <>
__device__ __forceinline__ float4 load_a4<0, 4>(const APlain& a, const RowCtx<0>& rc, int kk, int K) {
  float4 z = make_float4(0.f, 0.f, 0.f, 0.f);
  if (!rc.valid || kk >= K) return z;
  int k0 = kk;
#pragma unroll
  for (int s = 0; s < 3; ++s) {
    if (s < a.nseg) {
      if (k0 < a.seg[s].ncols) {
        return rc.base[s] ? ldg4(rc.base[s] + k0) : z;
      }
      k0 -= a.seg[s].ncols;
    }
  }
  return z;
}

template <>
__device__ __forceinline__ float4 load_a4<0, 1>(const APlain& a, const RowCtx<0>& rc, int kk, int K) {
  float v[4] = {0.f, 0.f, 0.f, 0.f};
  if (rc.valid) {
#pragma unroll
    for (int j = 0; j < 4; ++j) {
      int k0 = kk + j;
      if (k0 < K) {
#pragma unroll
        for (int s = 0; s < 3; ++s) {
          if (s < a.nseg) {
            if (k0 >= 0 && k0 < a.seg[s].ncols) {
              if (rc.base[s]) v[j] = __ldg(rc.base[s] + k0);
              k0 = -1;
            } else if (k0 >= 0) {
              k0 -= a.seg[s].ncols;
            }
          }
        }
      }
    }
  }
  return make_float4(v[0], v[1], v[2], v[3]);
}

template <>
__device__ __forceinline__ float4 load_a4<1, 4>(const AConv& a, const RowCtx<1>& rc, int kk, int K) {
  float4 z = make_float4(0.f, 0.f, 0.f, 0.f);
  if (!rc.valid || kk >= K) return z;
  int tap = kk / a.Cin;
  int ci = kk - tap * a.Cin;
  int kh = tap / a.KW;
  int kw = tap - kh * a.KW;
  int hi = rc.hi0 + kh, wi = rc.wi0 + kw;
  if (hi < 0 || hi >= a.H || wi < 0 || wi >= a.W) return z;
  return ldg4(rc.base + ((size_t)hi * a.W + wi) * a.ldx + ci);
}

template <>
__device__ __forceinline__ float4 load_a4<1, 1>(const AConv& a, const RowCtx<1>& rc, int kk, int K) {
  float v[4] = {0.f, 0.f, 0.f, 0.f};
  if (rc.valid) {
#pragma unroll
    for (int j = 0; j < 4; ++j) {
      int k0 = kk + j;
      if (k0 < K) {
        int tap = k0 / a.Cin;
        int ci = k0 - tap * a.Cin;
        int kh = tap / a.KW;
        int kw = tap - kh * a.KW;
        int hi = rc.hi0 + kh, wi = rc.wi0 + kw;
        if (hi >= 0 && hi < a.H && wi >= 0 && wi < a.W)
          v[j] = __ldg(rc.base + ((size_t)hi * a.W + wi) * a.ldx + ci);
      }
    }
  }
  return make_float4(v[0], v[1], v[2], v[3]);
}

template <int BM, int BN, int BK, int TM, int TN, int AMODE, int VEC>
__global__ void __launch_bounds__(256, 2)
gemm_f32_kernel(typename AParam<AMODE>::type a, const float* __restrict__ Bm, int ldb, int M, int N,
                int K, int k_per_split, Epi epi) {
  static_assert((BM / TM) * (BN / TN) == 256, "thread tiling must cover the CTA tile");
  constexpr int LA = BM * BK / 1024;
  constexpr int LB = BK * BN / 1024;
  static_assert(LA >= 1 && LB >= 1, "tile too small");
  constexpr int PAD = 4;
  __shared__ __align__(16) float As[2][BK][BM + PAD];
  __shared__ __align__(16) float Bs[2][BK][BN];

  if (epi.stop != nullptr && *epi.stop >= epi.stop_n) return;
  const int tid = threadIdx.x;
  const int m0 = blockIdx.y * BM;
  const int n0 = blockIdx.x * BN;
  const int kbeg = blockIdx.z * k_per_split;
  const int kend = min(K, kbeg + k_per_split);

  RowCtx<AMODE> rc[LA];
  int a_row[LA], a_kq[LA];
#pragma unroll
  for (int i = 0; i < LA; ++i) {
    int s = tid + 256 * i;
    a_row[i] = s / (BK / 4);
    a_kq[i] = s % (BK / 4);
// ... 192 lines not shown
```

### comic-compact-image-captioning-with-attention_b200/csrc/gemm_tc.cuh

```cuda
#pragma once
#include <cuda.h>
#include <cuda_bf16.h>
#include <cuda_runtime.h>
#include <stdint.h>

#include "gemm_f32.cuh"

namespace comic {
namespace tc {

constexpr int BM = 128;
constexpr int BK = 64;
constexpr int A_TILE_BYTES = BM * BK * 2;
constexpr int kEpiWarps = 8;
constexpr int kMmaWarp = kEpiWarps;
constexpr int kTmaWarp = kEpiWarps + 1;
constexpr int kLoaderGroups = 2;
constexpr int kFirstLoaderWarp = kEpiWarps + 2;
constexpr int kThreads = (kFirstLoaderWarp + 4 * kLoaderGroups) * 32;

__device__ __forceinline__ uint32_t smem_u32(const void* p) {
  return static_cast<uint32_t>(__cvta_generic_to_shared(p));
}
__device__ __forceinline__ void mbar_init(uint64_t* bar, uint32_t count) {
  asm volatile("mbarrier.init.shared::cta.b64 [%0], %1;" ::"r"(smem_u32(bar)), "r"(count) : "memory");
}
__device__ __forceinline__ void mbar_arrive(uint64_t* bar) {
  asm volatile("mbarrier.arrive.shared::cta.b64 _, [%0];" ::"r"(smem_u32(bar)) : "memory");
}
__device__ __forceinline__ void mbar_arrive_expect_tx(uint64_t* bar, uint32_t bytes) {
  asm volatile("mbarrier.arrive.expect_tx.shared::cta.b64 _, [%0], %1;" ::"r"(smem_u32(bar)), "r"(bytes)
               : "memory");
}
__device__ __forceinline__ void mbar_wait(uint64_t* bar, uint32_t parity) {
  uint32_t addr = smem_u32(bar);
  uint32_t done;
  do {
    asm volatile(
        "{\n\t.reg .pred p;\n\t"
        "mbarrier.try_wait.parity.shared::cta.b64 p, [%1], %2;\n\t"
        "selp.u32 %0, 1, 0, p;\n\t}"
        : "=r"(done)
        : "r"(addr), "r"(parity)
        : "memory");
  } while (!done);
}
__device__ __forceinline__ void fence_barrier_init() {
  asm volatile("fence.mbarrier_init.release.cluster;" ::: "memory");
}
__device__ __forceinline__ void fence_proxy_async() {
  asm volatile("fence.proxy.async.shared::cta;" ::: "memory");
}
__device__ __forceinline__ void tc_fence_before() {
  asm volatile("tcgen05.fence::before_thread_sync;" ::: "memory");
}
__device__ __forceinline__ void tc_fence_after() {
  asm volatile("tcgen05.fence::after_thread_sync;" ::: "memory");
}
__device__ __forceinline__ void named_bar_sync(int id, int nthreads) {
  asm volatile("bar.sync %0, %1;" ::"r"(id), "r"(nthreads) : "memory");
}
__device__ __forceinline__ void tma_load_2d(uint32_t smem_dst, const CUtensorMap* tm, uint64_t* bar, int c0,
                                            int c1) {
  asm volatile(
      "cp.async.bulk.tensor.2d.shared::cluster.global.mbarrier::complete_tx::bytes [%0], [%1, {%3, %4}], [%2];"
      ::"r"(smem_dst), "l"(reinterpret_cast<uint64_t>(tm)), "r"(smem_u32(bar)), "r"(c0), "r"(c1)
      : "memory");
}
__device__ __forceinline__ void umma_bf16(uint32_t tmem_d, uint64_t adesc, uint64_t bdesc, uint32_t idesc,
                                          uint32_t accumulate) {
  asm volatile(
      "{\n\t.reg .pred p;\n\t"
      "setp.ne.b32 p, %4, 0;\n\t"
      "tcgen05.mma.cta_group::1.kind::f16 [%0], %1, %2, %3, p;\n\t}"
      ::"r"(tmem_d), "l"(adesc), "l"(bdesc), "r"(idesc), "r"(accumulate)
      : "memory");
}
__device__ __forceinline__ void umma_commit(uint64_t* bar) {
  asm volatile("tcgen05.commit.cta_group::1.mbarrier::arrive::one.shared::cluster.b64 [%0];" ::"r"(smem_u32(bar))
               : "memory");
}

__device__ __forceinline__ uint32_t pack_bf16x2(float x, float y) {
  uint32_t r;
  asm("cvt.rn.bf16x2.f32 %0, %1, %2;" : "=r"(r) : "f"(y), "f"(x));
  return r;
}
__device__ __forceinline__ void split4(const float4& v, uint2& hi, uint2& lo) {
  hi.x = pack_bf16x2(v.x, v.y);
  hi.y = pack_bf16x2(v.z, v.w);
  float hx = __uint_as_float(hi.x << 16), hy = __uint_as_float(hi.x & 0xffff0000u);
  float hz = __uint_as_float(hi.y << 16), hw = __uint_as_float(hi.y & 0xffff0000u);
  lo.x = pack_bf16x2(v.x - hx, v.y - hy);
  lo.y = pack_bf16x2(v.z - hz, v.w - hw);
}

__device__ __forceinline__ uint64_t make_desc_sw128(uint32_t smem_addr) {
  uint64_t d = 0;
  d |= (uint64_t)((smem_addr >> 4) & 0x3FFF);
  d |= (uint64_t)1 << 16;
  d |= (uint64_t)(1024 >> 4) << 32;
  d |= (uint64_t)1 << 46;
  d |= (uint64_t)2 << 61;
  return d;
}

__host__ __device__ constexpr uint32_t make_idesc_bf16(int M, int N) {
  return (1u << 4) | (1u << 7) | (1u << 10) | ((uint32_t)(N >> 3) << 17) | ((uint32_t)(M >> 4) << 24);
}

__device__ __forceinline__ uint32_t cluster_ctarank() {
  uint32_t r;
  asm volatile("mov.u32 %0, %%cluster_ctarank;" : "=r"(r));
  return r;
}
__device__ __forceinline__ void cluster_sync_all() {
  asm volatile("barrier.cluster.arrive.release.aligned;" ::: "memory");
  asm volatile("barrier.cluster.wait.acquire.aligned;" ::: "memory");
}
__device__ __forceinline__ void mbar_arrive_cluster(uint64_t* bar, uint32_t rank) {
  uint32_t remote;
  asm volatile("mapa.shared::cluster.u32 %0, %1, %2;" : "=r"(remote) : "r"(smem_u32(bar)), "r"(rank));
  asm volatile("mbarrier.arrive.release.cluster.shared::cluster.b64 _, [%0];" ::"r"(remote) : "memory");
}
__device__ __forceinline__ void mbar_wait_cluster(uint64_t* bar, uint32_t parity) {
  uint32_t addr = smem_u32(bar);
  uint32_t done;
  do {
    asm volatile(
        "{\n\t.reg .pred p;\n\t"
        "mbarrier.try_wait.parity.acquire.cluster.shared::cta.b64 p, [%1], %2;\n\t"
        "selp.u32 %0, 1, 0, p;\n\t}"
        : "=r"(done)
        : "r"(addr), "r"(parity)
        : "memory");
  } while (!done);
}
__device__ __forceinline__ void tma_load_2d_pair(uint32_t smem_dst, const CUtensorMap* tm, uint64_t* bar, int c0,
                                                 int c1) {
  const uint32_t leader_bar = smem_u32(bar) & 0xFEFFFFFFu;
  asm volatile(
      "cp.async.bulk.tensor.2d.cta_group::2.shared::cluster.global.mbarrier::complete_tx::bytes [%0], [%1, {%3, %4}], [%2];"
      ::"r"(smem_dst), "l"(reinterpret_cast<uint64_t>(tm)), "r"(leader_bar), "r"(c0), "r"(c1)
      : "memory");
}
__device__ __forceinline__ void umma_bf16_pair(uint32_t tmem_d, uint64_t adesc, uint64_t bdesc, uint32_t idesc,
                                               uint32_t accumulate) {
  asm volatile(
      "{\n\t.reg .pred p;\n\t"
      "setp.ne.b32 p, %4, 0;\n\t"
      "tcgen05.mma.cta_group::2.kind::f16 [%0], %1, %2, %3, p;\n\t}"
      ::"r"(tmem_d), "l"(adesc), "l"(bdesc), "r"(idesc), "r"(accumulate)
      : "memory");
}
__device__ __forceinline__ void umma_commit_pair(uint64_t* bar) {
  asm volatile(
      "tcgen05.commit.cta_group::2.mbarrier::arrive::one.shared::cluster.multicast::cluster.b64 [%0], %1;"
      ::"r"(smem_u32(bar)), "h"((uint16_t)3)
      : "memory");
}
__device__ __forceinline__ void tma_load_2d_mc(uint32_t smem_dst, const CUtensorMap* tm, uint64_t* bar, int c0, int c1,
                                               uint16_t mask) {
  asm volatile(
      "cp.async.bulk.tensor.2d.shared::cluster.global.mbarrier::complete_tx::bytes.multicast::cluster [%0], [%1, {%3, %4}], [%2], %5;"
      ::"r"(smem_dst), "l"(reinterpret_cast<uint64_t>(tm)), "r"(smem_u32(bar)), "r"(c0), "r"(c1), "h"(mask)
      : "memory");
}
__device__ __forceinline__ void umma_commit_mc(uint64_t* bar, uint16_t mask) {
  asm volatile(
      "tcgen05.commit.cta_group::1.mbarrier::arrive::one.shared::cluster.multicast::cluster.b64 [%0], %1;"
      ::"r"(smem_u32(bar)), "h"(mask)
      : "memory");
}
__device__ __forceinline__ void sts_v2(uint32_t addr, uint32_t a, uint32_t b) {
  asm volatile("st.shared.v2.b32 [%0], {%1, %2};" ::"r"(addr), "r"(a), "r"(b) : "memory");
}

struct RowEntry {
  const void* ptr;
  unsigned long long mask;
};

constexpr int kHaloRows = 11, kHaloCols = 19;
constexpr int kHaloPlaneBytes = ((kHaloRows * kHaloCols * 32 + 127) / 128) * 128;
constexpr int kHaloBytes = 2 * 2 * kHaloPlaneBytes;

template <int BN, int STAGES, bool PAIR, int NKRES = 0, bool HALO = false>
struct SmemLayout {
  static constexpr int B_TILE_BYTES = (PAIR ? BN / 2 : BN) * BK * 2;
  static constexpr int STAGE_BYTES = 2 * A_TILE_BYTES + (NKRES ? 0 : 2 * B_TILE_BYTES);
  static constexpr int PANEL_OFF = STAGES * STAGE_BYTES;
  static constexpr int TILES_BYTES = PANEL_OFF + NKRES * 2 * B_TILE_BYTES;
  static constexpr int ROWTAB_BYTES = BM * 3 * 8;
  static constexpr int BAR_BYTES = ((3 * STAGES + 4) * 8 + 8 + 15) & ~15;
  static constexpr int EPI_STRIDE = 20;
  static constexpr int EPI_BYTES = kEpiWarps * 32 * EPI_STRIDE * 4;
  static constexpr int HALO_OFF = TILES_BYTES + kLoaderGroups * ROWTAB_BYTES + BAR_BYTES + EPI_BYTES;
  static constexpr int TOTAL = HALO_OFF + (HALO ? kHaloBytes : 0) + 1024;
  static constexpr int TMEM_COLS = (2 * BN <= 32) ? 32 : (2 * BN <= 64) ? 64 : (2 * BN <= 128) ? 128 : (2 * BN <= 256) ? 256 : 512;
};

template <int BN, int STAGES, int AMODE, bool PAIR, int NKRES = 0, int MC = 1>
__device__ __forceinline__ void gemm_bf16x3_body(const typename AParam<AMODE>::type& a, const CUtensorMap* tm_hi,
                                                 const CUtensorMap* tm_lo, int M, int N, int K, const Epi& epi) {
  static_assert(!(PAIR && NKRES), "resident weight panel: single-CTA kernel only");
  static_assert(MC == 1 || (!PAIR && NKRES == 0 && AMODE != 3 && (BN / MC) % 64 == 0), "multicast: plain kernel, slices of >= 64 rows");
  static_assert(AMODE != 4 || (!PAIR && NKRES == 0 && MC == 1), "TMA-staged A: plain kernel only");
  constexpr bool CL = PAIR || MC > 1;
  constexpr uint16_t kMcMask = (uint16_t)((1u << MC) - 1u);
  static_assert(AMODE != 3 || (NKRES > 0 && BN == 64), "halo loader: resident-panel stem kernel only");
  using L = SmemLayout<BN, STAGES, PAIR, NKRES, AMODE == 3>;
  constexpr int TM = (PAIR ? 2 : MC) * BM;
  constexpr int MMA_M = PAIR ? 2 * BM : BM;
  extern __shared__ uint8_t smem_raw[];
  pdl_launch_dependents();
  const uint32_t smem = (smem_u32(smem_raw) + 1023u) & ~1023u;
  uint8_t* smem_g = smem_raw + (smem - smem_u32(smem_raw));
  uint8_t* rowtab0 = smem_g + L::TILES_BYTES;
  uint64_t* bars = reinterpret_cast<uint64_t*>(rowtab0 + kLoaderGroups * L::ROWTAB_BYTES);
  uint64_t* full_a = bars;
  uint64_t* full_b = bars + STAGES;
  uint64_t* empty = bars + 2 * STAGES;
  uint64_t* tmem_full = bars + 3 * STAGES;
  uint64_t* tmem_empty = bars + 3 * STAGES + 2;
  uint32_t* tmem_slot = reinterpret_cast<uint32_t*>(bars + 3 * STAGES + 4);

  const int tid = threadIdx.x, warp = tid >> 5, lane = tid & 31;
  const uint32_t rank = CL ? cluster_ctarank() : 0u;
  const bool leader = PAIR ? rank == 0 : true;
  const int nk = (K + BK - 1) / BK;
  const int n_tiles = (N + BN - 1) / BN;
  const int m_tiles = (M + TM - 1) / TM;
  const int ksplit = (AMODE == 0 && !PAIR && MC == 1 && NKRES == 0 && epi.ksplit > 1) ? epi.ksplit : 1;
  const int mn_tiles = m_tiles * n_tiles;
  const int total_tiles = mn_tiles * ksplit;
  const int first_tile = PAIR ? (int)(blockIdx.x >> 1) : (int)blockIdx.x / MC;
  const int tile_step = PAIR ? (int)(gridDim.x >> 1) : (int)gridDim.x / MC;

  if (tid == 0) {
    for (int s = 0; s < STAGES; ++s) {
      mbar_init(&full_a[s], (AMODE >= 2 ? 256 : 128) * (PAIR ? 2 : 1));
      mbar_init(&full_b[s], 1);
      mbar_init(&empty[s], MC);
    }
    for (int i = 0; i < 2; ++i) {
      mbar_init(&tmem_full[i], 1);
      mbar_init(&tmem_empty[i], PAIR ? 2 * kEpiWarps : kEpiWarps);
    }
    fence_barrier_init();
  }
  if (warp == kMmaWarp) {
    if constexpr (PAIR) {
      asm volatile("tcgen05.alloc.cta_group::2.sync.aligned.shared::cta.b32 [%0], %1;" ::"r"(smem_u32(tmem_slot)),
                   "r"((uint32_t)L::TMEM_COLS)
                   : "memory");
      asm volatile("tcgen05.relinquish_alloc_permit.cta_group::2.sync.aligned;" ::: "memory");
    } else {
      asm volatile("tcgen05.alloc.cta_group::1.sync.aligned.shared::cta.b32 [%0], %1;" ::"r"(smem_u32(tmem_slot)),
                   "r"((uint32_t)L::TMEM_COLS)
                   : "memory");
      asm volatile("tcgen05.relinquish_alloc_permit.cta_group::1.sync.aligned;" ::: "memory");
    }
  }
  tc_fence_before();
  __syncthreads();
  if constexpr (CL) cluster_sync_all();
  tc_fence_after();
  const uint32_t tmem_base = *tmem_slot;
  pdl_wait();
  const bool stopped = epi.stop != nullptr && *epi.stop >= epi.stop_n;

  if (stopped) {
  } else if (warp < kEpiWarps) {
    const int nr = epi.nroute;
    const int b1 = nr > 1 ? epi.r[1].n0 : 0x7fffffff;
    const int b2 = nr > 2 ? epi.r[2].n0 : 0x7fffffff;
    const int quad = warp & 3, half = warp >> 2;
    float* stage_buf = reinterpret_cast<float*>(reinterpret_cast<uint8_t*>(bars) + L::BAR_BYTES) + warp * 32 * L::EPI_STRIDE;
    const uint32_t stage_u32 = smem_u32(stage_buf);
    const int srow = lane >> 2, scol = (lane & 3) * 4;
    int iter = 0;
    for (int tile = first_tile; tile < total_tiles; tile += tile_step, ++iter) {
      const int kz = tile / mn_tiles, mn = tile - kz * mn_tiles;
      const int m0 = (mn / n_tiles) * TM + (int)rank * BM;
      const int n0 = (mn % n_tiles) * BN;
      const int acc = iter & 1;
      const int n_umma = min(BN, ((N - n0) + 15) & ~15);
      mbar_wait(&tmem_full[acc], (uint32_t)((iter >> 1) & 1));
      tc_fence_after();
      const int mw = m0 + quad * 32;
      const int t_img = AMODE == 3 ? tile / 98 : 0, t_rem = AMODE == 3 ? tile - t_img * 98 : 0;
      const int t_y0 = (t_rem / 7) * 8, t_x0 = (t_rem % 7) * 16;
      auto row_to_m = [&](int row) -> int {
        if constexpr (AMODE == 3) {
          const int r = quad * 32 + row;
          return (t_img * 112 + t_y0 + (r >> 4)) * 112 + t_x0 + (r & 15);
        } else {
          return mw + row;
        }
      };
      const float* cprow[4] = {nullptr, nullptr, nullptr, nullptr};
      float cp_next[4] = {0.f, 0.f, 0.f, 0.f};
      if (epi.lstm_h != nullptr && epi.lstm_c_prev != nullptr) {
#pragma unroll
        for (int q = 0; q < 4; ++q) {
          const int m = row_to_m(q * 8 + srow);
          if (m < M) {
            const int rr = epi.lstm_src ? epi.lstm_src[m] : m;
            if (rr >= 0 && rr < epi.lstm_src_limit) cprow[q] = epi.lstm_c_prev + (size_t)rr * epi.lstm_R;
          }
        }
        const int u0 = (n0 + half * 16 + scol) >> 2;
        if (n0 + half * 16 + scol < N) {
#pragma unroll
          for (int q = 0; q < 4; ++q) if (cprow[q]) cp_next[q] = __ldg(cprow[q] + u0);
        }
      }
#pragma unroll 1
      for (int c0 = half * 16; c0 < n_umma; c0 += 32) {
        uint32_t r[16];
        float cp_cur[4];
#pragma unroll
        for (int q = 0; q < 4; ++q) cp_cur[q] = cp_next[q];
        if (epi.lstm_h != nullptr && c0 + 32 < n_umma && n0 + c0 + 32 + scol < N) {
          const int un = (n0 + c0 + 32 + scol) >> 2;
#pragma unroll
          for (int q = 0; q < 4; ++q) cp_next[q] = cprow[q] ? __ldg(cprow[q] + un) : 0.f;
        }
        uint32_t taddr = tmem_base + ((uint32_t)(quad * 32) << 16) + (uint32_t)(acc * BN + c0);
        asm volatile(
            "tcgen05.ld.sync.aligned.32x32b.x16.b32 {%0, %1, %2, %3, %4, %5, %6, %7, %8, %9, %10, %11, %12, %13, "
            "%14, %15}, [%16];"
            : "=r"(r[0]), "=r"(r[1]), "=r"(r[2]), "=r"(r[3]), "=r"(r[4]), "=r"(r[5]), "=r"(r[6]), "=r"(r[7]),
              "=r"(r[8]), "=r"(r[9]), "=r"(r[10]), "=r"(r[11]), "=r"(r[12]), "=r"(r[13]), "=r"(r[14]), "=r"(r[15])
            : "r"(taddr));
        asm volatile("tcgen05.wait::ld.sync.aligned;" ::: "memory");
#pragma unroll
        for (int g = 0; g < 4; ++g)
          asm volatile("st.shared.v4.b32 [%0], {%1, %2, %3, %4};" ::"r"(stage_u32 + (uint32_t)(lane * L::EPI_STRIDE + g * 4) * 4u),
                       "r"(r[g * 4 + 0]), "r"(r[g * 4 + 1]), "r"(r[g * 4 + 2]), "r"(r[g * 4 + 3])
                       : "memory");
        __syncwarp();
        const int n = n0 + c0 + scol;
        if (n < N) {
          const int rt = n >= b2 ? 2 : (n >= b1 ? 1 : 0);
          float* const fdst = epi.r[rt].dst;
          uint16_t* const hdst = epi.r[rt].hi;
          uint16_t* const ldst = epi.r[rt].lo;
          const long long ld = epi.r[rt].ld;
          const long long cofs = (long long)epi.r[rt].coff - epi.r[rt].n0 + n + (long long)kz * epi.split_stride;
          const float4 sc = epi.scale ? ldg4(epi.scale + n) : make_float4(1.f, 1.f, 1.f, 1.f);
          const float4 bs = epi.bias ? ldg4(epi.bias + n) : make_float4(0.f, 0.f, 0.f, 0.f);
          if (epi.lstm_h != nullptr) {
            const int u = n >> 2;
#pragma unroll
            for (int q = 0; q < 4; ++q) {
              const int row = q * 8 + srow;
              const int m = row_to_m(row);
              if (m < M) {
                const float4 v = *reinterpret_cast<const float4*>(stage_buf + row * L::EPI_STRIDE + scol);
                const float cp = cp_cur[q];
                const float cn = cp * sig_<true>((v.z + bs.z) + 1.0f) + sig_<true>(v.x + bs.x) * tanh_<true>(v.y + bs.y);
                const float hn = tanh_<true>(cn) * sig_<true>(v.w + bs.w);
                epi.lstm_c[(size_t)m * epi.lstm_R + u] = cn;
                epi.lstm_h[(size_t)m * epi.lstm_R + u] = hn;
              }
            }
            __syncwarp();
            continue;
          }
#pragma unroll
          for (int q = 0; q < 4; ++q) {
            const int row = q * 8 + srow;
            const int m = row_to_m(row);
            if (m < M) {
              float4 v = *reinterpret_cast<const float4*>(stage_buf + row * L::EPI_STRIDE + scol);
              if (epi.scale) { v.x *= sc.x; v.y *= sc.y; v.z *= sc.z; v.w *= sc.w; }
              if (epi.bias) { v.x += bs.x; v.y += bs.y; v.z += bs.z; v.w += bs.w; }
              if (epi.relu) {
                v.x = fmaxf(v.x, 0.f); v.y = fmaxf(v.y, 0.f); v.z = fmaxf(v.z, 0.f); v.w = fmaxf(v.w, 0.f);
              }
              const long long o = (long long)m * ld + cofs;
              if (fdst) *reinterpret_cast<float4*>(fdst + o) = v;
              if (hdst) {
                uint2 sh, sl;
                split4(v, sh, sl);
                *reinterpret_cast<uint2*>(hdst + o) = sh;
                *reinterpret_cast<uint2*>(ldst + o) = sl;
              }
            }
          }
        }
        __syncwarp();
      }
      tc_fence_before();
      __syncwarp();
      if (lane == 0) {
        if constexpr (PAIR) mbar_arrive_cluster(&tmem_empty[acc], 0);
        else mbar_arrive(&tmem_empty[acc]);
      }
    }
  } else if (warp == kMmaWarp) {
    if (leader && lane == 0) {
      int iter = 0;
      uint32_t it = 0;
      if constexpr (NKRES > 0) mbar_wait(&full_b[0], 0);
      for (int tile = first_tile; tile < total_tiles; tile += tile_step, ++iter) {
        const int kz = tile / mn_tiles, mn = tile - kz * mn_tiles;
        const int kt0 = (int)(((long long)kz * nk) / ksplit), kt1 = (int)(((long long)(kz + 1) * nk) / ksplit);
        const int n0 = (mn % n_tiles) * BN;
        const int acc = iter & 1;
        const int n_umma = min(BN, ((N - n0) + 15) & ~15);
        const uint32_t idesc = make_idesc_bf16(MMA_M, n_umma);
        const uint32_t d_tmem = tmem_base + (uint32_t)(acc * BN);
        if constexpr (PAIR) mbar_wait_cluster(&tmem_empty[acc], (uint32_t)(((iter >> 1) & 1) ^ 1));
        else mbar_wait(&tmem_empty[acc], (uint32_t)(((iter >> 1) & 1) ^ 1));
        tc_fence_after();
        for (int kt = kt0; kt < kt1; ++kt, ++it) {
          const int s = it % STAGES;
          const uint32_t ph = (it / STAGES) & 1;
          if constexpr (PAIR) {
            mbar_wait_cluster(&full_a[s], ph);
            mbar_wait_cluster(&full_b[s], ph);
          } else {
            if constexpr (AMODE != 4) mbar_wait(&full_a[s], ph);
            if constexpr (NKRES == 0) mbar_wait(&full_b[s], ph);
          }
          tc_fence_after();
          const uint32_t a_hi = smem + s * L::STAGE_BYTES;
          const uint32_t a_lo = a_hi + A_TILE_BYTES;
          const uint32_t b_hi = NKRES ? smem + L::PANEL_OFF + kt * 2 * L::B_TILE_BYTES : a_lo + A_TILE_BYTES;
          const uint32_t b_lo = b_hi + L::B_TILE_BYTES;
          const uint64_t dah = make_desc_sw128(a_hi), dal = make_desc_sw128(a_lo);
          const uint64_t dbh = make_desc_sw128(b_hi), dbl = make_desc_sw128(b_lo);
#pragma unroll
          for (int k16 = 0; k16 < BK / 16; ++k16) {
            const uint64_t adv = (uint64_t)((k16 * 16 * 2) >> 4);
            const uint32_t first = (kt > kt0 || k16 > 0) ? 1u : 0u;
            if constexpr (PAIR) {
              umma_bf16_pair(d_tmem, dah + adv, dbh + adv, idesc, first);
              umma_bf16_pair(d_tmem, dal + adv, dbh + adv, idesc, 1u);
              umma_bf16_pair(d_tmem, dah + adv, dbl + adv, idesc, 1u);
            } else {
              umma_bf16(d_tmem, dah + adv, dbh + adv, idesc, first);
              umma_bf16(d_tmem, dal + adv, dbh + adv, idesc, 1u);
              umma_bf16(d_tmem, dah + adv, dbl + adv, idesc, 1u);
            }
          }
          if constexpr (PAIR) umma_commit_pair(&empty[s]);
          else if constexpr (MC > 1) umma_commit_mc(&empty[s], kMcMask);
          else umma_commit(&empty[s]);
        }
        if constexpr (PAIR) umma_commit_pair(&tmem_full[acc]);
        else umma_commit(&tmem_full[acc]);
      }
    }
    __syncwarp();
  } else if (warp == kTmaWarp) {
    if constexpr (NKRES > 0) {
      if (lane == 0 && first_tile < total_tiles) {
        mbar_arrive_expect_tx(&full_b[0], (uint32_t)nk * 2u * L::B_TILE_BYTES);
        for (int kt = 0; kt < nk; ++kt) {
          const uint32_t b_hi = smem + L::PANEL_OFF + kt * 2 * L::B_TILE_BYTES;
          tma_load_2d(b_hi, tm_hi, &full_b[0], kt * BK, 0);
          tma_load_2d(b_hi + L::B_TILE_BYTES, tm_lo, &full_b[0], kt * BK, 0);
        }
      }
    } else
    if (lane == 0) {
      uint32_t it = 0;
      for (int tile = first_tile; tile < total_tiles; tile += tile_step) {
        const int kz = tile / mn_tiles, mn = tile - kz * mn_tiles;
        const int kt0 = (int)(((long long)kz * nk) / ksplit), kt1 = (int)(((long long)(kz + 1) * nk) / ksplit);
        const int n0 = (mn % n_tiles) * BN;
        const int n_umma = min(BN, ((N - n0) + 15) & ~15);
        const int nrow = PAIR ? n0 + (int)rank * (n_umma >> 1) : n0 + (int)rank * (BN / MC);
        for (int kt = kt0; kt < kt1; ++kt, ++it) {
          const int s = it % STAGES;
          const uint32_t ph = (it / STAGES) & 1;
          mbar_wait(&empty[s], ph ^ 1);
          const uint32_t b_hi = smem + s * L::STAGE_BYTES + 2 * A_TILE_BYTES;
          const uint32_t b_lo = b_hi + L::B_TILE_BYTES;
          if constexpr (PAIR) {
            if (leader) mbar_arrive_expect_tx(&full_b[s], 4 * L::B_TILE_BYTES);
            tma_load_2d_pair(b_hi, tm_hi, &full_b[s], kt * BK, nrow);
            tma_load_2d_pair(b_lo, tm_lo, &full_b[s], kt * BK, nrow);
          } else if constexpr (MC > 1) {
            mbar_arrive_expect_tx(&full_b[s], 2 * L::B_TILE_BYTES);
            const uint32_t slice = rank * (uint32_t)((BN / MC) * BK * 2);
            tma_load_2d_mc(b_hi + slice, tm_hi, &full_b[s], kt * BK, nrow, kMcMask);
            tma_load_2d_mc(b_lo + slice, tm_lo, &full_b[s], kt * BK, nrow, kMcMask);
          } else if constexpr (AMODE == 4) {
            const int m0 = (mn / n_tiles) * TM;
            const uint32_t a_hi = smem + s * L::STAGE_BYTES;
            mbar_arrive_expect_tx(&full_b[s], 2 * L::B_TILE_BYTES + 2 * A_TILE_BYTES);
            tma_load_2d(a_hi, &a.hi, &full_b[s], kt * BK, m0);
            tma_load_2d(a_hi + A_TILE_BYTES, &a.lo, &full_b[s], kt * BK, m0);
            tma_load_2d(b_hi, tm_hi, &full_b[s], kt * BK, nrow);
            tma_load_2d(b_lo, tm_lo, &full_b[s], kt * BK, nrow);
          } else {
            mbar_arrive_expect_tx(&full_b[s], 2 * L::B_TILE_BYTES);
            tma_load_2d(b_hi, tm_hi, &full_b[s], kt * BK, nrow);
            tma_load_2d(b_lo, tm_lo, &full_b[s], kt * BK, nrow);
          }
        }
      }
    }
    __syncwarp();
  } else {
    if constexpr (AMODE == 4) {
    } else if constexpr (AMODE == 3) {
      const int lw = warp - kFirstLoaderWarp;
      const int tg = lw * 32 + lane;
      const int c8 = lane & 7, r4 = lane >> 3;
      uint8_t* halo_g = smem_g + L::HALO_OFF;
      const uint32_t halo = smem + L::HALO_OFF;
      auto fetch_halo = [&](int tile, int buf) {
        if (tile < total_tiles) {
          const int img = tile / 98, rem = tile - img * 98;
          const int y0 = (rem / 7) * 8 - 1, x0 = (rem % 7) * 16 - 1;
          for (int i = tg; i < kHaloRows * kHaloCols * 4; i += 256) {
            const int plane = i & 1, ch = (i >> 1) & 1, px = i >> 2;
            const int hr = px / kHaloCols, hc = px - hr * kHaloCols;
            const int y = y0 + hr, x = x0 + hc;
            const bool ok = y >= 0 && y < 112 && x >= 0 && x < 112;
            const long long go = ok ? (((long long)img * 112 + y) * 112 + x) * 16 + ch * 8 : 0;
            const uint32_t so = halo + (uint32_t)((buf * 2 + plane) * kHaloPlaneBytes + px * 32 + ch * 16);
            const uint32_t nbytes = ok ? 16u : 0u;
            asm volatile("cp.async.cg.shared.global [%0], [%1], 16, %2;" ::"r"(so), "l"((plane ? a.lo : a.hi) + go), "r"(nbytes)
                         : "memory");
          }
        }
        asm volatile("cp.async.commit_group;" ::: "memory");
      };
      uint32_t it = 0;
      int tcount = 0;
      fetch_halo(first_tile, 0);
      for (int tile = first_tile; tile < total_tiles; tile += tile_step, ++tcount) {
        const int buf = tcount & 1;
        named_bar_sync(1, 256);
        fetch_halo(tile + tile_step, buf ^ 1);
        asm volatile("cp.async.wait_group 1;" ::: "memory");
        named_bar_sync(1, 256);
        const uint8_t* hb = halo_g + (size_t)(buf * 2) * kHaloPlaneBytes;
        for (int kt = 0; kt < nk; ++kt, ++it) {
          const int s = it % STAGES;
          const uint32_t ph = (it / STAGES) & 1;
          const uint32_t a_hi = smem + s * L::STAGE_BYTES;
          mbar_wait(&empty[s], ph ^ 1);
#pragma unroll
          for (int i = 0; i < 4; ++i) {
            const int row = lw * 16 + i * 4 + r4;
            const int src = (((row >> 4) + kt) * kHaloCols + (row & 15)) * 32 + c8 * 16;
            const uint4 vh = *reinterpret_cast<const uint4*>(hb + src);
            const uint4 vl = *reinterpret_cast<const uint4*>(hb + kHaloPlaneBytes + src);
            const uint32_t so = (uint32_t)row * 128u + ((uint32_t)(c8 ^ (row & 7)) << 4);
            asm volatile("st.shared.v4.b32 [%0], {%1, %2, %3, %4};" ::"r"(a_hi + so), "r"(vh.x), "r"(vh.y), "r"(vh.z), "r"(vh.w)
                         : "memory");
            asm volatile("st.shared.v4.b32 [%0], {%1, %2, %3, %4};" ::"r"(a_hi + A_TILE_BYTES + so), "r"(vl.x), "r"(vl.y),
                         "r"(vl.z), "r"(vl.w)
                         : "memory");
          }
          fence_proxy_async();
          mbar_arrive(&full_a[s]);
        }
      }
      asm volatile("cp.async.wait_group 0;" ::: "memory");
    } else if constexpr (AMODE == 2) {
      const int lw = warp - kFirstLoaderWarp;
      const int tg = lw * 32 + lane;
      const int c8 = lane & 7, r4 = lane >> 3;
      RowEntry* re = reinterpret_cast<RowEntry*>(rowtab0);
      uint32_t it = 0, retired = 0;
      auto retire = [&]() {
        fence_proxy_async();
        uint64_t* bar = &full_a[retired % STAGES];
        if constexpr (PAIR) mbar_arrive_cluster(bar, 0);
        else mbar_arrive(bar);
        ++retired;
      };
      for (int tile = first_tile; tile < total_tiles; tile += tile_step) {
        const int m0 = (tile / n_tiles) * TM + (int)rank * BM;
        named_bar_sync(1, 256);
        if (tg < BM) {
          const int m = m0 + tg;
          RowEntry e;
          e.ptr = nullptr; e.mask = 0ull;
          if (m < M) {
            const int hw = a.Ho * a.Wo;
            const int b = m / hw, rem = m - b * hw;
            const int ho = rem / a.Wo, wo = rem - ho * a.Wo;
            const int hi0 = ho * a.stride - a.pad_t, wi0 = wo * a.stride - a.pad_l;
            e.ptr = reinterpret_cast<const void*>((((long long)b * a.H + hi0) * a.W + wi0) * a.ldx);
            for (int kh = 0; kh < a.KH; ++kh)
              for (int kw = 0; kw < a.KW; ++kw) {
                const int hi = hi0 + kh, wi = wi0 + kw;
                if (hi >= 0 && hi < a.H && wi >= 0 && wi < a.W) e.mask |= 1ull << (kh * a.KW + kw);
              }
          }
          re[tg] = e;
        }
        named_bar_sync(1, 256);
        for (int kt = 0; kt < nk; ++kt, ++it) {
          const int s = it % STAGES;
          const uint32_t ph = (it / STAGES) & 1;
          const uint32_t a_hi = smem + s * L::STAGE_BYTES;
          const int kk8 = kt * BK + c8 * 8;
          unsigned long long bit = 0ull;
          long long tapoff = 0;
          if (kk8 < K) {
            const int tap = kk8 / a.Cin, ci = kk8 - tap * a.Cin;
            const int kh = tap / a.KW, kw = tap - kh * a.KW;
            bit = 1ull << tap;
            tapoff = ((long long)kh * a.W + kw) * a.ldx + ci;
          }
          mbar_wait(&empty[s], ph ^ 1);
#pragma unroll
          for (int i = 0; i < 4; ++i) {
            const int row = lw * 16 + i * 4 + r4;
            const RowEntry e = re[row];
            const bool ok = (e.mask & bit) != 0ull;
            const long long go = ok ? reinterpret_cast<long long>(e.ptr) + tapoff : 0;
            const uint32_t so = (uint32_t)row * 128u + ((uint32_t)(c8 ^ (row & 7)) << 4);
            const uint32_t nbytes = ok ? 16u : 0u;
            asm volatile("cp.async.cg.shared.global [%0], [%1], 16, %2;" ::"r"(a_hi + so), "l"(a.hi + go), "r"(nbytes)
                         : "memory");
            asm volatile("cp.async.cg.shared.global [%0], [%1], 16, %2;" ::"r"(a_hi + A_TILE_BYTES + so), "l"(a.lo + go),
                         "r"(nbytes)
                         : "memory");
          }
          asm volatile("cp.async.commit_group;" ::: "memory");
          if (it + 1 - retired == (uint32_t)STAGES) {
            asm volatile("cp.async.wait_group %0;" ::"n"(STAGES - 1) : "memory");
            retire();
          }
        }
      }
      asm volatile("cp.async.wait_group 0;" ::: "memory");
      while (retired < it) retire();
    } else {
    const int grp = (warp - kFirstLoaderWarp) >> 2;
    const int wg = (warp - kFirstLoaderWarp) & 3;
    const int tg = wg * 32 + lane;
    uint8_t* rowtab = rowtab0 + grp * L::ROWTAB_BYTES;
    uint32_t it = 0;
    for (int tile = first_tile; tile < total_tiles; tile += tile_step) {
      const int kz = tile / mn_tiles, mn = tile - kz * mn_tiles;
      const int kt0 = (int)(((long long)kz * nk) / ksplit), kt1 = (int)(((long long)(kz + 1) * nk) / ksplit);
      const int m0 = (mn / n_tiles) * TM + (int)rank * BM;
      named_bar_sync(1 + grp, 128);
      {
        int m = m0 + tg;
        if constexpr (AMODE == 0) {
          const float** rp = reinterpret_cast<const float**>(rowtab);
#pragma unroll
          for (int s = 0; s < 3; ++s) {
            const float* p = nullptr;
            if (s < a.nseg && m < M) {
              int r = m;
              if (a.seg[s].idx) r = a.seg[s].idx[m];
              if (r >= 0 && r < a.seg[s].idx_limit) p = a.seg[s].ptr + (size_t)r * a.seg[s].ld;
            }
            rp[s * BM + tg] = p;
// ... 123 lines not shown
  gemm_bf16x3_body<BN, STAGES, AMODE, false, 0, MC>(a, &tm_hi, &tm_lo, M, N, K, epi);
}

template <int BN, int STAGES, int AMODE>
__global__ void __cluster_dims__(2, 1, 1) __launch_bounds__(kThreads, 1)
gemm_bf16x3_pair_kernel(const __grid_constant__ typename AParam<AMODE>::type a, const __grid_constant__ CUtensorMap tm_hi,
                        const __grid_constant__ CUtensorMap tm_lo, int M, int N, int K,
                        const __grid_constant__ Epi epi) {
  gemm_bf16x3_body<BN, STAGES, AMODE, true>(a, &tm_hi, &tm_lo, M, N, K, epi);
}


struct TcWeight {
  uint16_t* hi = nullptr;
  uint16_t* lo = nullptr;
  int N = 0, K = 0, Npad = 0, Kpad = 0;
  CUtensorMap tm_hi[5], tm_lo[5];
  bool ready = false;
};

typedef CUresult (*EncodeTiledFn)(CUtensorMap*, CUtensorMapDataType, cuuint32_t, void*, const cuuint64_t*,
                                  const cuuint64_t*, const cuuint32_t*, const cuuint32_t*, CUtensorMapInterleave,
                                  CUtensorMapSwizzle, CUtensorMapL2promotion, CUtensorMapFloatOOBfill);

inline EncodeTiledFn get_encode_fn() {
  static EncodeTiledFn fn = nullptr;
  if (!fn) {
    void* p = nullptr;
    cudaDriverEntryPointQueryResult q;
    if (cudaGetDriverEntryPoint("cuTensorMapEncodeTiled", &p, cudaEnableDefault, &q) == cudaSuccess &&
        q == cudaDriverEntryPointSuccess)
      fn = reinterpret_cast<EncodeTiledFn>(p);
  }
  return fn;
}

inline bool make_weight_maps(TcWeight& w) {
  EncodeTiledFn enc = get_encode_fn();
  if (!enc) return false;
  const int bns[5] = {64, 128, 256, 176, 192};
  for (int i = 0; i < 5; ++i) {
    cuuint64_t dims[2] = {(cuuint64_t)w.Kpad, (cuuint64_t)w.Npad};
    cuuint64_t strides[1] = {(cuuint64_t)w.Kpad * sizeof(uint16_t)};
    cuuint32_t box[2] = {(cuuint32_t)BK, (cuuint32_t)bns[i]};
    cuuint32_t estr[2] = {1, 1};
    CUresult r1 = enc(&w.tm_hi[i], CU_TENSOR_MAP_DATA_TYPE_BFLOAT16, 2, w.hi, dims, strides, box, estr,
                      CU_TENSOR_MAP_INTERLEAVE_NONE, CU_TENSOR_MAP_SWIZZLE_128B, CU_TENSOR_MAP_L2_PROMOTION_L2_256B,
                      CU_TENSOR_MAP_FLOAT_OOB_FILL_NONE);
    CUresult r2 = enc(&w.tm_lo[i], CU_TENSOR_MAP_DATA_TYPE_BFLOAT16, 2, w.lo, dims, strides, box, estr,
                      CU_TENSOR_MAP_INTERLEAVE_NONE, CU_TENSOR_MAP_SWIZZLE_128B, CU_TENSOR_MAP_L2_PROMOTION_L2_256B,
                      CU_TENSOR_MAP_FLOAT_OOB_FILL_NONE);
    if (r1 != CUDA_SUCCESS || r2 != CUDA_SUCCESS) return false;
  }
  w.ready = true;
  return true;
}

static __global__ void pack_bt_kernel(const float* __restrict__ W, int K, int N, int ldw, uint16_t* __restrict__ hi,
                                      uint16_t* __restrict__ lo, int Kpad, int Npad, int cin_src, int cin_dst,
                                      int gate_R = 0) {
  size_t i = (size_t)blockIdx.x * blockDim.x + threadIdx.x;
  if (i >= (size_t)Npad * Kpad) return;
  int n = (int)(i / Kpad), kp = (int)(i % Kpad);
  float v = 0.f;
  const int n_src = gate_R > 0 ? (n & 3) * gate_R + (n >> 2) : n;
  if (n < N) {
    int k = kp;
    bool ok = kp < K;
    if (cin_src != cin_dst) {
      int tap = kp / cin_dst, ci = kp - tap * cin_dst;
      ok = ci < cin_src && tap < K / cin_src;
      k = tap * cin_src + ci;
    }
    if (ok) v = W[(size_t)k * ldw + n_src];
  }
  uint32_t h = pack_bf16x2(v, 0.f) & 0xffffu;
  float hf = __uint_as_float(h << 16);
  uint32_t l = pack_bf16x2(v - hf, 0.f) & 0xffffu;
  hi[i] = (uint16_t)h;
  lo[i] = (uint16_t)l;
}

template <int BN, int STAGES, int AMODE>
inline cudaError_t launch_one(const typename AParam<AMODE>::type& a, const TcWeight& w, int bn_idx, int M, int N,
                              const Epi& epi, int num_sms, cudaStream_t st) {
  using L = SmemLayout<BN, STAGES, false>;
  static PerDeviceOnce once;
  {
    cudaError_t e = once([&] { return cudaFuncSetAttribute(gemm_bf16x3_kernel<BN, STAGES, AMODE>,
                                         cudaFuncAttributeMaxDynamicSharedMemorySize, L::TOTAL); });
    if (e != cudaSuccess) return e;
  }
  int tiles = ((N + BN - 1) / BN) * ((M + BM - 1) / BM) * ((AMODE == 0 && epi.ksplit > 1) ? epi.ksplit : 1);
  int grid = tiles < num_sms ? tiles : num_sms;
  if (epi.pdl) return launch_pdl(gemm_bf16x3_kernel<BN, STAGES, AMODE>, dim3(grid), dim3(kThreads), L::TOTAL, st, a,
                                 w.tm_hi[bn_idx], w.tm_lo[bn_idx], M, N, w.K, epi);
  gemm_bf16x3_kernel<BN, STAGES, AMODE><<<grid, kThreads, L::TOTAL, st>>>(a, w.tm_hi[bn_idx], w.tm_lo[bn_idx], M,
                                                                          N, w.K, epi);
  return cudaGetLastError();
}

inline int pick_bn(int M, int N, int num_sms, bool small_ok = false) {
  if (N <= 64) return 64;
  if (N <= 128) return 128;
  const int mt = (M + BM - 1) / BM;
  const int t256 = mt * ((N + 255) / 256), t128 = mt * ((N + 127) / 128);
  if (small_ok && t256 < num_sms) {
    const int cand[4] = {256, 176, 128, 64};
    int best = 256;
    long best_cost = -1;
    for (int i = 0; i < 4; ++i) {
      const int bn = cand[i];
      const int tiles = mt * ((N + bn - 1) / bn);
      const long cost = (long)((tiles + num_sms - 1) / num_sms) * (bn + 48);
      if (best_cost < 0 || cost < best_cost) { best_cost = cost; best = bn; }
    }
    return best;
  }
  if (t256 < num_sms && t128 <= num_sms) return 128;
  return 256;
}

template <int STAGES, int NKRES, int AMODE>
inline cudaError_t launch_bres(const typename AParam<AMODE>::type& a, const TcWeight& w, int M, int N, const Epi& epi,
                               int num_sms, cudaStream_t st) {
  using L = SmemLayout<64, STAGES, false, NKRES>;
  static_assert(L::TOTAL <= 232448, "resident-panel kernel exceeds the shared memory of an SM");
  static PerDeviceOnce once;
  {
    cudaError_t e = once([&] { return cudaFuncSetAttribute(gemm_bf16x3_bres_kernel<STAGES, NKRES, AMODE>,
                                         cudaFuncAttributeMaxDynamicSharedMemorySize, L::TOTAL); });
    if (e != cudaSuccess) return e;
  }
  int tiles = (M + BM - 1) / BM;
  int grid = tiles < num_sms ? tiles : num_sms;
  gemm_bf16x3_bres_kernel<STAGES, NKRES, AMODE><<<grid, kThreads, L::TOTAL, st>>>(a, w.tm_hi[0], w.tm_lo[0], M, N, w.K, epi);
  return cudaGetLastError();
}

inline cudaError_t launch_stem_halo(const AHalo& a, const TcWeight& w, const Epi& epi, int num_sms, cudaStream_t st) {
  using L = SmemLayout<64, 3, false, 4, true>;
  static_assert(L::TOTAL <= 232448, "halo stem kernel exceeds the shared memory of an SM");
  static PerDeviceOnce once;
  {
    cudaError_t e = once([&] { return cudaFuncSetAttribute(gemm_bf16x3_bres_kernel<3, 4, 3>, cudaFuncAttributeMaxDynamicSharedMemorySize, L::TOTAL); });
    if (e != cudaSuccess) return e;
  }
  const int tiles = a.nimg * 98;
  const int grid = tiles < num_sms ? tiles : num_sms;
  gemm_bf16x3_bres_kernel<3, 4, 3><<<grid, kThreads, L::TOTAL, st>>>(a, w.tm_hi[0], w.tm_lo[0], a.nimg * 12544, 64, 256, epi);
  return cudaGetLastError();
}

inline int& bres_mode() { static int v = 1; return v; }

template <int BN, int STAGES, int AMODE>
inline cudaError_t launch_pair(const typename AParam<AMODE>::type& a, const TcWeight& w, int half_idx, int M, int N,
                               const Epi& epi, int num_sms, cudaStream_t st) {
  using L = SmemLayout<BN, STAGES, true>;
  static PerDeviceOnce once;
  {
    cudaError_t e = once([&] { return cudaFuncSetAttribute(gemm_bf16x3_pair_kernel<BN, STAGES, AMODE>,
                                         cudaFuncAttributeMaxDynamicSharedMemorySize, L::TOTAL); });
    if (e != cudaSuccess) return e;
  }
  int tiles = ((N + BN - 1) / BN) * ((M + 2 * BM - 1) / (2 * BM));
  int grid = 2 * tiles < (num_sms & ~1) ? 2 * tiles : (num_sms & ~1);
  gemm_bf16x3_pair_kernel<BN, STAGES, AMODE><<<grid, kThreads, L::TOTAL, st>>>(a, w.tm_hi[half_idx], w.tm_lo[half_idx],
                                                                               M, N, w.K, epi);
  return cudaGetLastError();
}

template <int BN, int STAGES, int AMODE, int MC>
inline cudaError_t launch_mc(const typename AParam<AMODE>::type& a, const TcWeight& w, int box_idx, int M, int N,
                             const Epi& epi, int num_sms, cudaStream_t st) {
  using L = SmemLayout<BN, STAGES, false>;
  auto kern = gemm_bf16x3_mc_kernel<BN, STAGES, AMODE, MC>;
  static PerDeviceOnce once;
  {
    cudaError_t e = once([&] {
      cudaError_t e1 = cudaFuncSetAttribute(kern, cudaFuncAttributeMaxDynamicSharedMemorySize, L::TOTAL);
      if (e1 != cudaSuccess) return e1;
      return cudaFuncSetAttribute(kern, cudaFuncAttributeNonPortableClusterSizeAllowed, 0);
    });
    if (e != cudaSuccess) return e;
  }
  const int super_tiles = ((N + BN - 1) / BN) * ((M + MC * BM - 1) / (MC * BM));
  const int max_clusters = num_sms / MC;
  const int clusters = super_tiles < max_clusters ? super_tiles : max_clusters;
  cudaLaunchConfig_t cfg{};
  cfg.gridDim = dim3((unsigned)(clusters * MC), 1, 1);
  cfg.blockDim = dim3(kThreads, 1, 1);
  cfg.dynamicSmemBytes = L::TOTAL;
  cfg.stream = st;
  cudaLaunchAttribute at[1];
  at[0].id = cudaLaunchAttributeClusterDimension;
  at[0].val.clusterDim.x = MC;
  at[0].val.clusterDim.y = 1;
  at[0].val.clusterDim.z = 1;
  cfg.attrs = at;
  cfg.numAttrs = 1;
  int K = w.K;
  return cudaLaunchKernelEx(&cfg, kern, a, w.tm_hi[box_idx], w.tm_lo[box_idx], M, N, K, epi);
}

inline int& small_tiles() { static int v = 1; return v; }

inline int& mc_mode() { static int v = 0; return v; }

inline int& pair_mode() { static int v = 0; return v; }
inline int& pair_min_tiles() { static int v = 74; return v; }

inline bool make_a_maps(ATma& a, const uint16_t* hi, const uint16_t* lo, int rows, int K) {
  EncodeTiledFn enc = get_encode_fn();
  if (!enc) return false;
  cuuint64_t dims[2] = {(cuuint64_t)K, (cuuint64_t)rows};
  cuuint64_t strides[1] = {(cuuint64_t)K * sizeof(uint16_t)};
  cuuint32_t box[2] = {(cuuint32_t)BK, (cuuint32_t)BM};
  cuuint32_t estr[2] = {1, 1};
  CUresult r1 = enc(&a.hi, CU_TENSOR_MAP_DATA_TYPE_BFLOAT16, 2, const_cast<uint16_t*>(hi), dims, strides, box, estr,
                    CU_TENSOR_MAP_INTERLEAVE_NONE, CU_TENSOR_MAP_SWIZZLE_128B, CU_TENSOR_MAP_L2_PROMOTION_L2_256B,
                    CU_TENSOR_MAP_FLOAT_OOB_FILL_NONE);
  CUresult r2 = enc(&a.lo, CU_TENSOR_MAP_DATA_TYPE_BFLOAT16, 2, const_cast<uint16_t*>(lo), dims, strides, box, estr,
                    CU_TENSOR_MAP_INTERLEAVE_NONE, CU_TENSOR_MAP_SWIZZLE_128B, CU_TENSOR_MAP_L2_PROMOTION_L2_256B,
                    CU_TENSOR_MAP_FLOAT_OOB_FILL_NONE);
  return r1 == CUDA_SUCCESS && r2 == CUDA_SUCCESS;
}

template <int AMODE>
inline cudaError_t launch_gemm_tc(const typename AParam<AMODE>::type& a, const TcWeight& w, int M, int N,
                                  const Epi& epi, int num_sms, cudaStream_t st) {
  if constexpr (AMODE != 2 && AMODE != 4) {
    if (pair_mode() && N > 64) {
      bool planes = false;
      for (int r = 0; r < epi.nroute; ++r) planes = planes || epi.r[r].hi != nullptr;
      const int mp = (M + 2 * BM - 1) / (2 * BM);
      const int bnp = (N <= 128) ? 128 : 256;
      if (!planes && mp * ((N + bnp - 1) / bnp) >= pair_min_tiles()) {
        if (bnp == 128) return launch_pair<128, 4, AMODE>(a, w, 0, M, N, epi, num_sms, st);
        return launch_pair<256, 3, AMODE>(a, w, 1, M, N, epi, num_sms, st);
      }
    }
  }
  int bn = pick_bn(M, N, num_sms, (AMODE == 0 || AMODE == 4) && small_tiles());
  if constexpr (AMODE == 0) {
    if (epi.ksplit > 1) return launch_one<128, 3, 0>(a, w, 1, M, N, epi, num_sms, st);
  }
  if constexpr (AMODE == 0 || AMODE == 4) {
    if (bn == 176) return launch_one<176, 2, AMODE>(a, w, 3, M, N, epi, num_sms, st);
  }
  if constexpr (AMODE == 1) {
    if (small_tiles() && N > 256 && N <= 352 && w.K >= 512) return launch_one<176, 2, 1>(a, w, 3, M, N, epi, num_sms, st);
    if (small_tiles() && N == 192 && a.KH == 3 && a.Cin == 64) return launch_one<192, 2, 1>(a, w, 4, M, N, epi, num_sms, st);
  }
  if constexpr (AMODE != 0 && AMODE != 4) {
    if (bn == 64 && bres_mode() && (M + BM - 1) / BM >= 2 * num_sms) {
      const int nkb = (w.K + BK - 1) / BK;
      if (nkb <= 4) return launch_bres<4, 4, AMODE>(a, w, M, N, epi, num_sms, st);
      if (nkb <= 6) return launch_bres<3, 6, AMODE>(a, w, M, N, epi, num_sms, st);
      if (nkb <= 8) return launch_bres<2, 8, AMODE>(a, w, M, N, epi, num_sms, st);
    }
  }
  if constexpr (AMODE != 2 && AMODE != 3 && AMODE != 4) {
    const int mc = mc_mode();
    const int m_tiles = (M + BM - 1) / BM;
    if (mc >= 2 && bn >= 128 && m_tiles >= 2 * mc) {
      if (bn == 128) return launch_mc<128, 3, AMODE, 2>(a, w, 0, M, N, epi, num_sms, st);
      if (mc >= 4) return launch_mc<256, 2, AMODE, 4>(a, w, 0, M, N, epi, num_sms, st);
      return launch_mc<256, 2, AMODE, 2>(a, w, 1, M, N, epi, num_sms, st);
    }
  }
  if (bn == 64) return launch_one<64, 4, AMODE>(a, w, 0, M, N, epi, num_sms, st);
  if (bn == 128) return launch_one<128, 3, AMODE>(a, w, 1, M, N, epi, num_sms, st);
  return launch_one<256, 2, AMODE>(a, w, 2, M, N, epi, num_sms, st);
}

}
}
```

### comic-compact-image-captioning-with-attention_b200/engine.py

```python
from __future__ import annotations

import ctypes as C
import os

import numpy as np

from . import weights as wts

_HERE = os.path.dirname(os.path.abspath(__file__))
LIB_PATH = os.path.join(_HERE, 'libcomic_b200.so')
NUM_CONVS = 57

FM_PROJ = {None: 0, 'none': 0, 'tied': 1, 'independent': 2}
ALIGN = {'add_LN': 0, 'dot': 1}
PROB = {'softmax': 0, 'sigmoid': 1}
INIT = {'first_input': 0, 'project_hidden': 1}


class ComicCfg(C.Structure):
    _fields_ = [(n, C.c_int32) for n in (
        'rnn_size', 'word_size', 'num_heads', 'fm_channels', 'fm_positions', 'embed_size', 'vocab',
        'fm_projection', 'context_layer', 'init_method', 'alignment', 'prob_fn', 'embed_lookup',
        'legacy', 'go_id', 'eos_id')]


_FP = C.c_void_p


class ComicWeights(C.Structure):
    _fields_ = [(n, _FP) for n in (
        'lstm_kernel', 'lstm_bias', 'init_weight', 'memory_kernel', 'value_kernel', 'query_kernel',
        'attention_v', 'ln_gamma', 'ln_beta', 'temperature', 'a_layer', 'out_kernel', 'out_bias',
        'embedding_map', 'enc_ln_gamma', 'enc_ln_beta', 'enc_embed_weight')] + [
        ('conv_w', _FP * NUM_CONVS), ('bn_beta', _FP * NUM_CONVS), ('bn_mean', _FP * NUM_CONVS),
        ('bn_var', _FP * NUM_CONVS)]


class ComicTrainMasks(C.Structure):
    _fields_ = [('init_in', _FP), ('inp', _FP), ('out', _FP), ('att', _FP),
                ('in_keep', C.c_float), ('out_keep', C.c_float), ('att_keep', C.c_float)]


GRAD_FIELDS = ('lstm_kernel', 'lstm_bias', 'init_weight', 'memory_kernel', 'value_kernel', 'query_kernel',
               'attention_v', 'ln_gamma', 'ln_beta', 'temperature', 'out_kernel', 'out_bias', 'embedding_map', 'a_layer')


class ComicDecoderGrads(C.Structure):
    _fields_ = [(n, _FP) for n in GRAD_FIELDS]


class ComicCnnGrads(C.Structure):
    _fields_ = [('conv_w', _FP * NUM_CONVS), ('bn_beta', _FP * NUM_CONVS)]


class ComicConvDesc(C.Structure):
    _fields_ = [('k', C.c_int32), ('stride', C.c_int32), ('c_in', C.c_int32), ('c_out', C.c_int32)]


class ComicError(RuntimeError):
    pass


_lib = None

_I, _F, _SZ, _P = C.c_int, C.c_float, C.c_size_t, C.c_void_p
SIGNATURES = {
    'comic_last_error': (C.c_char_p, []),
    'comic_version': (C.c_char_p, []),
    'comic_conv_table': (C.POINTER(ComicConvDesc), []),
    'comic_create': (_I, [C.POINTER(ComicCfg), C.POINTER(_P)]),
    'comic_destroy': (_I, [_P]),
    'comic_packed_bytes': (_I, [_P, C.POINTER(_SZ)]),
    'comic_bind_weights': (_I, [_P, C.POINTER(ComicWeights), _I, _P, _SZ, _P]),
    'comic_workspace_bytes': (_I, [_P, _I, _I, _I, _I, C.POINTER(_SZ)]),
    'comic_encode_fwd': (_I, [_P, _P, _I, _P, _P, _P, _P, _SZ, _P]),
    'comic_preprocess_eval': (_I, [_P, _P, _I, _I, _I, _I, _I, _P, _P]),
    'comic_project_fm': (_I, [_P, _P, _I, _P, _P, _P]),
    'comic_rnn_init': (_I, [_P, _P, _I, _P, _P, _P, _F, _P, _SZ, _P]),
    'comic_decode_step': (_I, [_P, _P, _P, _I, _I, _P, _P, _P, _P, _P, _P, _P, _P, _P, _P, _P, _P,
                               _F, _F, _F, _P, _SZ, _P]),
    'comic_decode_greedy': (_I, [_P, _P, _P, _P, _P, _I, _I, _P, _P, _P, _P, _P, _SZ, _P]),
    'comic_decode_beam': (_I, [_P, _P, _P, _P, _P, _I, _I, _F, _I, _P, _P, _P, _P, _P, _P, _P, _P, _SZ, _P]),
    'comic_beam_step': (_I, [_P, _P, _I, _I, _I, _I, _I, _F, _P, _P, _P, _P, _P, _P, _P]),
    'comic_gather_tree': (_I, [_P, _P, _P, _P, _I, _I, _I, _I, _P, _P]),
    'comic_gemm_f32': (_I, [_P, _P, _I, _P, _I, _P, _P, _I, _I, _I, _I, _P, _SZ, _P]),
    'comic_launch_count': (_I, [_P, C.POINTER(C.c_int64)]),
    'comic_set_precision': (_I, [_P, _I]),
    'comic_set_option': (_I, [_P, _I, _I]),
    'comic_preprocess_train': (_I, [_P, _P, _I, _I, _I, _I, _I, _P, _P, _P, _P]),
    'comic_decode_trace': (_I, [_P, _P, _I, _P, _P]),
    'comic_train_workspace_bytes': (_I, [_P, _I, _I, C.POINTER(_SZ)]),
    'comic_dropout_masks': (_I, [_P, _P, _SZ, _F, C.c_uint64, C.c_uint64, _P]),
    'comic_train_fwd_bwd': (_I, [_P, _P, _P, _I, _P, _P, _P, _P, _I, _I, C.POINTER(ComicTrainMasks), _F, _P, _P, _P,
                                 C.POINTER(ComicDecoderGrads), _P, _SZ, _P]),
    'comic_l2_regularise': (_I, [_P, _P, _P, _SZ, _F, _P, _P, _SZ, _P]),
    'comic_adam_step': (_I, [_P, _P, _P, _P, _P, _SZ, _F, _F, _F, _F, _I, _F, _P]),
    'comic_momentum_step': (_I, [_P, _P, _P, _P, _SZ, _F, _F, _F, _P]),
    'comic_clip_by_norm': (_I, [_P, _P, _P, _P, _I, _F, _P]),
    'comic_refresh_packed': (_I, [_P, _P, _SZ, _P]),
    'comic_refresh_packed_cnn': (_I, [_P, _P, _SZ, _P]),
    'comic_train_encoder_grads': (_I, [_P, _I, _I, _P, _P, _P, _SZ, _P]),
    'comic_legacy_head_bwd_bytes': (_I, [_P, _I, _P]),
    'comic_legacy_head_bwd': (_I, [_P, _P, _I, _P, _P, _P, _P, _P, _SZ, _P]),
    'comic_encode_train_bytes': (_I, [_P, _I, C.POINTER(_SZ), C.POINTER(_SZ)]),
    'comic_encode_train_fwd': (_I, [_P, _P, _I, _P, _P, _P, _SZ, _P, _SZ, _P]),
    'comic_encode_bwd': (_I, [_P, _P, _I, _P, _P, _P, _SZ, C.POINTER(ComicCnnGrads), _P, _SZ, _P]),
    'comic_profile_enable': (_I, [_P, C.c_uint32]),
    'comic_profile_read': (_I, [_P, _I, C.POINTER(C.c_double), C.POINTER(C.c_int64)]),
}

KERNEL_TAGS = ['conv', 'pool', 'project', 'init', 'gates', 'lstm', 'lq', 'scores', 'ctx', 'beam',
               'final', 'misc', 'persist']


def load_library(path=LIB_PATH):
    global _lib
    if _lib is not None:
        return _lib
    path = os.environ.get('COMIC_B200_LIB', path)
    if not os.path.exists(path):
        raise ComicError('libcomic_b200.so not built (%s); run `python __graft_entry__.py build`' % path)
    lib = C.CDLL(path)
    for name, (res, args) in SIGNATURES.items():
        fn = getattr(lib, name)
        fn.restype = res
        fn.argtypes = args
    _lib = lib
    return lib


def executed_steps(T):
    t = int(T.item())
    if t < 0:
        raise ComicError('decode loop aborted: the persistent kernel gave up at a grid barrier')
    return t


def _ptr(t):
    if t is None:
        return None
    return C.c_void_p(t.data_ptr())


class Engine(object):

    def __init__(self, config, device=None):
        import torch
        if not torch.cuda.is_available():
            raise ComicError('comic_b200 requires a CUDA device (B200, sm_100a); no CPU fallback exists')
        self.torch = torch
        self.lib = load_library()
        self.device = torch.device('cuda', torch.cuda.current_device() if device is None else device)
        torch.cuda.set_device(self.device)
        self.c = config
        d = self.dims = wts.Dims(config)
        if config.rnn_name != 'LSTM':
            raise ComicError('rnn_name=%s is not built (LSTM only)' % config.rnn_name)
        if config.attn_alignment_method not in ALIGN:
            raise ValueError('Invalid alignment method.')
        if config.attn_probability_fn not in PROB:
            raise ValueError('Invalid alignment method.')
        if config.token_type == 'radix':
            go, eos = config.radix_base, config.radix_base + 1
        else:
            go, eos = config.wtoi['<GO>'], config.wtoi['<EOS>']
        self.go, self.eos = int(go), int(eos)
        cfg = ComicCfg(
            rnn_size=d.R, word_size=d.W, num_heads=d.H, fm_channels=d.C, fm_positions=d.M,
            embed_size=d.E, vocab=d.V, fm_projection=FM_PROJ[config.cnn_fm_projection],
            context_layer=int(bool(config.attn_context_layer)), init_method=INIT[config.rnn_init_method],
            alignment=ALIGN[config.attn_alignment_method], prob_fn=PROB[config.attn_probability_fn],
            embed_lookup=int(config.token_type == 'word'), legacy=int(bool(config.legacy)),
            go_id=self.go, eos_id=self.eos)
        self._h = C.c_void_p()
        self._check(self.lib.comic_create(C.byref(cfg), C.byref(self._h)))
        self._dev_weights = {}
        self._packed = None
        self._ws = {}
        self.bound_cnn = False
        for kv in filter(None, os.environ.get('COMIC_B200_OPTS', '').split(',')):
            name, value = kv.split('=')
            self.set_option(name.strip(), int(value))

    def _check(self, rc):
        if rc != 0:
            msg = self.lib.comic_last_error().decode()
            if rc == -4:
                raise NotImplementedError(msg)
            if rc in (-1, -2):
                raise ValueError(msg)
            raise ComicError('comic_b200 error %d: %s' % (rc, msg))

    def __del__(self):
        try:
            if self._h:
                self.lib.comic_destroy(self._h)
                self._h = C.c_void_p()
        except Exception:
            pass

    def stream(self):
        return C.c_void_p(self.torch.cuda.current_stream(self.device).cuda_stream)

    def _workspace(self, mode, B, k, T):
        n = C.c_size_t()
        self._check(self.lib.comic_workspace_bytes(self._h, mode, B, k, T, C.byref(n)))
        key = mode
        buf = self._ws.get(key)
        if buf is None or buf.numel() < n.value:
            buf = self.torch.empty(n.value, dtype=self.torch.uint8, device=self.device)
            self._ws[key] = buf
        return buf

    def f32(self, *shape):
        return self.torch.empty(shape, dtype=self.torch.float32, device=self.device)

    def to_dev(self, a, dtype=None):
        t = self.torch.as_tensor(a)
        if dtype is not None:
            t = t.to(dtype)
        return t.to(self.device).contiguous()

    def bind_weights(self, W, with_cnn=True):
        torch = self.torch
        c = self.c
        dev = {}
        for k, v in W.items():
            dev[k] = torch.as_tensor(np.ascontiguousarray(v) if isinstance(v, np.ndarray) else v,
                                     dtype=torch.float32).to(self.device).contiguous()
        self._dev_weights = dev
        self._bind_generation = getattr(self, '_bind_generation', 0) + 1
        D, ENC, CNN = wts.DEC, wts.ENC, wts.CNN
        cs = wts.cell_scope(c)
        att = D + 'multi_add_attention/'

        def g(name):
            t = dev.get(name)
            return None if t is None else C.c_void_p(t.data_ptr())
        w = ComicWeights()
        w.lstm_kernel = g(cs + 'kernel')
        w.lstm_bias = g(cs + 'bias')
        w.init_weight = g(D + ('rnn_init_input/projection/weight' if c.rnn_init_method == 'first_input'
                               else 'rnn_initial_state/weight'))
        w.memory_kernel = g(D + 'memory_layer/kernel')
        w.value_kernel = g(D + 'value_layer/kernel')
        w.query_kernel = g(att + 'query_layer/kernel')
        w.attention_v = g(att + 'attention_v')
        w.ln_gamma = g(att + 'LN_tanh/gamma')
        w.ln_beta = g(att + 'LN_tanh/beta')
        if (D + 'softmax_temperature') in dev:
            dev[D + 'softmax_temperature'] = dev[D + 'softmax_temperature'].reshape(1).contiguous()
        w.temperature = g(D + 'softmax_temperature')
        w.a_layer = g(D + 'a_layer/kernel')
        w.out_kernel = g(D + 'output_projection/kernel')
        w.out_bias = g(D + 'output_projection/bias')
        w.embedding_map = g(D + 'embedding_map')
        w.enc_ln_gamma = g(ENC + 'LN_tanh/gamma')
        w.enc_ln_beta = g(ENC + 'LN_tanh/beta')
        w.enc_embed_weight = g(ENC + 'im_embed/weight')
        have_cnn = with_cnn and (CNN + 'Conv2d_1a_7x7/weights') in dev
        if have_cnn:
            for i, (scope, _k, _s, _ci, _co) in enumerate(wts.cnn_conv_list()):
                w.conv_w[i] = g(CNN + scope + '/weights')
                w.bn_beta[i] = g(CNN + scope + '/BatchNorm/beta')
                w.bn_mean[i] = g(CNN + scope + '/BatchNorm/moving_mean')
                w.bn_var[i] = g(CNN + scope + '/BatchNorm/moving_variance')
        n = C.c_size_t()
        self._check(self.lib.comic_packed_bytes(self._h, C.byref(n)))
        self._packed = torch.empty(n.value, dtype=torch.uint8, device=self.device)
        self._check(self.lib.comic_bind_weights(self._h, C.byref(w), int(have_cnn), _ptr(self._packed),
                                                n.value, self.stream()))
        self.bound_cnn = bool(have_cnn)
        self._wstruct = w

    def encode(self, images, want_mixed5c=False):
        torch = self.torch
        images = images.contiguous()
        if images.dim() != 4 or tuple(images.shape[1:]) != (224, 224, 3):
            raise ValueError('images must be [B,224,224,3] NHWC, got %s' % (tuple(images.shape),))
        B = images.shape[0]
        fm = self.f32(B, self.dims.M, self.dims.C)
        emb = self.f32(B, self.dims.E)
        m5c = self.f32(B, 7, 7, 1024) if want_mixed5c else None
        ws = self._workspace(0, B, 1, 1)
        self._check(self.lib.comic_encode_fwd(self._h, _ptr(images), B, _ptr(fm), _ptr(emb), _ptr(m5c),
                                              _ptr(ws), ws.numel(), self.stream()))
        return (emb, fm, m5c) if want_mixed5c else (emb, fm)

    def preprocess_eval(self, images_u8, out_hw=(224, 224)):
        torch = self.torch
        images_u8 = images_u8.contiguous()
        if images_u8.dtype != torch.uint8 or images_u8.dim() != 4 or images_u8.shape[3] != 3:
            raise ValueError('images must be uint8 [B,H,W,3], got %s %s' % (images_u8.dtype, tuple(images_u8.shape)))
        B, H, W = (int(v) for v in images_u8.shape[:3])
        out = self.f32(B, int(out_hw[0]), int(out_hw[1]), 3)
        self._check(self.lib.comic_preprocess_eval(self._h, _ptr(images_u8), B, H, W, int(out_hw[0]), int(out_hw[1]),
                                                   _ptr(out), self.stream()))
        return out

    def preprocess_train(self, images_u8, crop_yx, flip=None, out_hw=(224, 224)):
        torch = self.torch
        images_u8 = images_u8.contiguous()
        if images_u8.dtype != torch.uint8 or images_u8.dim() != 4 or images_u8.shape[3] != 3:
            raise ValueError('images must be uint8 [B,H,W,3], got %s %s' % (images_u8.dtype, tuple(images_u8.shape)))
        B, H, W = (int(v) for v in images_u8.shape[:3])
        crop = torch.as_tensor(crop_yx).to(device=self.device, dtype=torch.int32).contiguous()
        if tuple(crop.shape) != (B, 2):
            raise ValueError('crop_yx must be [B, 2]')
        if int(crop.min()) < 0 or int(crop[:, 0].max()) > 256 - out_hw[0] or int(crop[:, 1].max()) > 256 - out_hw[1]:
            raise ValueError('crop offsets must lie in [0, 256 - out]')
        fl = None if flip is None else torch.as_tensor(flip).to(device=self.device, dtype=torch.uint8).contiguous()
        out = self.f32(B, int(out_hw[0]), int(out_hw[1]), 3)
        self._check(self.lib.comic_preprocess_train(self._h, _ptr(images_u8), B, H, W, int(out_hw[0]), int(out_hw[1]),
                                                    _ptr(crop), _ptr(fl), _ptr(out), self.stream()))
        return out

    def project_fm(self, fm):
        B = fm.shape[0]
        d = self.dims
        keys = self.f32(B, d.M, d.R)
        values = self.f32(B, d.M, d.R) if d.fm_projection == 'independent' else None
        self._check(self.lib.comic_project_fm(self._h, _ptr(fm.contiguous()), B, _ptr(keys), _ptr(values),
                                              self.stream()))
        if d.fm_projection is None:
            values = fm
        elif d.fm_projection == 'tied':
            values = keys
        return keys, values

    def rnn_init(self, im_embed, in_mask=None, in_keep=1.0):
        B = im_embed.shape[0]
        c0, h0 = self.f32(B, self.dims.R), self.f32(B, self.dims.R)
        ws = self._workspace(4, B, 1, 1)
        self._check(self.lib.comic_rnn_init(self._h, _ptr(im_embed.contiguous()), B, _ptr(c0), _ptr(h0),
                                            _ptr(in_mask), float(in_keep), _ptr(ws), ws.numel(), self.stream()))
        return c0, h0

    def decode_step(self, keys, values, B, k, tokens, c_in, h_in, ctx_in, in_mask=None, out_mask=None,
                    att_mask=None, keeps=(1.0, 1.0, 1.0)):
        d = self.dims
        N = B * k
        c_out, h_out = self.f32(N, d.R), self.f32(N, d.R)
        ctx_out = self.f32(N, d.A)
        align = self.f32(N, d.H * d.M)
        logits = self.f32(N, d.V)
        ws = self._workspace(3, B, k, 1)
        vals = None if d.fm_projection == 'tied' else values
        self._check(self.lib.comic_decode_step(
            self._h, _ptr(keys), _ptr(vals), B, k, _ptr(tokens), _ptr(c_in), _ptr(h_in), _ptr(ctx_in),
            _ptr(c_out), _ptr(h_out), _ptr(ctx_out), _ptr(align), _ptr(logits),
            _ptr(in_mask), _ptr(out_mask), _ptr(att_mask), float(keeps[0]), float(keeps[1]), float(keeps[2]),
            _ptr(ws), ws.numel(), self.stream()))
        return dict(c=c_out, h=h_out, attention=ctx_out, alignments=align, logits=logits)

    def decode_greedy(self, keys, values, c0, h0, max_it, want_logits=True, want_attn=True):
        torch = self.torch
        d = self.dims
        B = c0.shape[0]
        ids = torch.empty((max(max_it, 1), B), dtype=torch.int32, device=self.device)
        logits = self.f32(max(max_it, 1), B, d.V) if want_logits else None
        attn = self.f32(B, d.H, max(max_it, 1), d.M) if want_attn else None
        T = torch.zeros(1, dtype=torch.int32, device=self.device)
        ws = self._workspace(1, B, 1, max(max_it, 1))
        vals = None if d.fm_projection == 'tied' else values
        self._check(self.lib.comic_decode_greedy(self._h, _ptr(keys), _ptr(vals), _ptr(c0), _ptr(h0), B, max_it,
                                                 _ptr(ids), _ptr(logits), _ptr(attn), _ptr(T), _ptr(ws),
                                                 ws.numel(), self.stream()))
        return dict(ids=ids, logits=logits, attn=attn, T=T)

    def decode_beam(self, keys, values, c0, h0, beam, lpw, max_it, want_attn=True):
        torch = self.torch
        d = self.dims
        B = c0.shape[0]
        Tm = max(max_it, 1)
        i32 = dict(dtype=torch.int32, device=self.device)
        pred = torch.empty((Tm, B, beam), **i32)
        step_ids = torch.empty((Tm, B, beam), **i32)
        parents = torch.empty((Tm, B, beam), **i32)
        scores = self.f32(Tm, B, beam)
        lengths = torch.empty((B, beam), dtype=torch.int64, device=self.device)
        attn = self.f32(B, d.H, Tm, d.M) if want_attn else None
        T = torch.zeros(1, dtype=torch.int32, device=self.device)
        ws = self._workspace(2, B, beam, Tm)
        vals = None if d.fm_projection == 'tied' else values
        self._check(self.lib.comic_decode_beam(self._h, _ptr(keys), _ptr(vals), _ptr(c0), _ptr(h0), B, beam,
                                               float(lpw), max_it, _ptr(pred), _ptr(step_ids), _ptr(parents),
                                               _ptr(scores), _ptr(lengths), _ptr(attn), _ptr(T), _ptr(ws),
                                               ws.numel(), self.stream()))
        return dict(predicted_ids=pred, step_ids=step_ids, parent_ids=parents, scores=scores,
                    lengths=lengths, attn=attn, T=T)

    def beam_step(self, logits, log_probs, finished, lengths, eos, lpw):
        torch = self.torch
        B, k, V = logits.shape
        logits = logits.contiguous()
        scores = self.f32(B, k)
        word = torch.empty((B, k), dtype=torch.int32, device=self.device)
        parent = torch.empty((B, k), dtype=torch.int32, device=self.device)
        self._check(self.lib.comic_beam_step(self._h, _ptr(logits), V, B, k, V, int(eos), float(lpw),
                                             _ptr(log_probs), _ptr(finished), _ptr(lengths), _ptr(scores),
                                             _ptr(word), _ptr(parent), self.stream()))
        return scores, word, parent

    def gather_tree(self, step_ids, parent_ids, max_seq_len, end_token):
        T, B, k = step_ids.shape
        out = self.torch.empty_like(step_ids)
        self._check(self.lib.comic_gather_tree(self._h, _ptr(step_ids.contiguous()), _ptr(parent_ids.contiguous()),
                                               _ptr(max_seq_len.contiguous()), T, B, k, int(end_token), _ptr(out),
                                               self.stream()))
        return out

    def gemm(self, A, Bm, bias=None):
        M, K = A.shape
        N = Bm.shape[1]
        out = self.f32(M, N)
        ws = self._workspace(5, N, K, 1)
        self._check(self.lib.comic_gemm_f32(self._h, _ptr(A), A.stride(0), _ptr(Bm), Bm.stride(0), _ptr(bias),
                                            _ptr(out), N, M, N, K, _ptr(ws), ws.numel(), self.stream()))
        return out

    def set_precision(self, mode):
        self._check(self.lib.comic_set_precision(self._h, {'f32': 0, 'tf32x3': 1, 'split': 1, 'fast': 2}[mode]))

    def set_option(self, name, value):
        self._check(self.lib.comic_set_option(self._h, {'fused_attn_min_images': 0, 'enc_chunk_stem': 1, 'enc_chunk_28': 2, 'enc_chunk_14': 3, 'persistent_max_rows': 4, 'persistent_trace': 5, 'enc_planes': 6, 'gemm_pair': 7, 'gemm_pair_min_tiles': 8, 'stem_s2d': 9, 'gemm_resident_b': 10, 'tc_min_rows': 11, 'attn2': 12, 'fuse_lstm': 13, 'gemm_mc': 14, 'tma_a': 15, 'gemm_small_tiles': 16, 'pdl': 17, 'persistent_watchdog_ms': 18, 'tc_splitk': 19}[name], int(value)))

    def decode_trace(self, max_steps=256):
        import numpy as np
        out = np.zeros((max_steps, 2, 16), np.int64)
        n = C.c_int()
        self._check(self.lib.comic_decode_trace(self._h, out.ctypes.data_as(C.c_void_p), max_steps, C.byref(n),
                                                self.stream()))
        return out[:n.value]

    def profile_enable(self, tags):
        mask = 0
        for t in tags:
            mask |= 1 << KERNEL_TAGS.index(t)
        self._profiling = mask != 0
        self._check(self.lib.comic_profile_enable(self._h, mask))

    def graphed(self, key, fn, *inputs):
        torch = self.torch
        if not getattr(self, 'infer_graph', True) or getattr(self, '_profiling', False):
            return fn(*inputs)
        if not hasattr(self, '_graphs'):
            self._graphs, self.replayed_launches = {}, 0
            self.infer_graph = os.environ.get('COMIC_B200_INFER_GRAPH', '1') != '0'
            if not self.infer_graph:
                return fn(*inputs)

        def signature():
            return (tuple((t.data_ptr(), tuple(t.shape), t.dtype) for t in inputs), getattr(self, '_bind_generation', 0),
                    tuple(sorted((k, v.data_ptr()) for k, v in self._ws.items() if hasattr(v, 'data_ptr'))))
        ent = self._graphs.get(key)
        if ent is not None and ent['sig'] != signature():
            ent = None
        if ent is None:
            out = fn(*inputs)
            self._graphs[key] = {'sig': signature(), 'graph': None}
            return out
        if ent['graph'] is None:
            torch.cuda.synchronize(self.device)
            g = torch.cuda.CUDAGraph()
            n0 = self.launch_count()
            try:
                with torch.cuda.graph(g):
                    ent['out'] = fn(*inputs)
            except Exception:
                self.infer_graph = False
                torch.cuda.synchronize(self.device)
                return fn(*inputs)
            ent['graph'], ent['launches'] = g, self.launch_count() - n0
            if ent['sig'] != signature():
                self._graphs.pop(key)
                return fn(*inputs)
        ent['graph'].replay()
        self.replayed_launches += ent['launches']
        return ent['out']

    def profile_read(self, tag):
        ms, n = C.c_double(), C.c_int64()
        self._check(self.lib.comic_profile_read(self._h, KERNEL_TAGS.index(tag), C.byref(ms), C.byref(n)))
        return ms.value, n.value

    def variable_to_grad_field(self):
        c = self.c
        D = wts.DEC
        att = D + 'multi_add_attention/'
        cs = wts.cell_scope(c)
        m = {cs + 'kernel': 'lstm_kernel', cs + 'bias': 'lstm_bias',
             D + 'rnn_init_input/projection/weight': 'init_weight', D + 'rnn_initial_state/weight': 'init_weight',
             D + 'memory_layer/kernel': 'memory_kernel', D + 'value_layer/kernel': 'value_kernel',
             att + 'query_layer/kernel': 'query_kernel', att + 'attention_v': 'attention_v',
             att + 'LN_tanh/gamma': 'ln_gamma', att + 'LN_tanh/beta': 'ln_beta',
             D + 'softmax_temperature': 'temperature', D + 'output_projection/kernel': 'out_kernel',
             D + 'output_projection/bias': 'out_bias', D + 'embedding_map': 'embedding_map',
             D + 'a_layer/kernel': 'a_layer'}
        return m

    def dropout_masks(self, shape, keep, seed, stream_id):
        out = self.f32(*shape)
        self._check(self.lib.comic_dropout_masks(self._h, _ptr(out), out.numel(), float(keep), int(seed),
                                                 int(stream_id), self.stream()))
        return out

    def train_fwd_bwd(self, fm, im_embed, inputs_tm, targets_tm, coef_tm, lens, T_run, grad_views, masks=None,
                      keeps=(1.0, 1.0, 1.0), map_loss_scale=1.0, want_logits=False, want_attn=False):
        torch = self.torch
        d = self.dims
        T, B = inputs_tm.shape
        loss = torch.zeros(4, dtype=torch.float32, device=self.device)
        logits = self.f32(B, T, d.V) if want_logits else None
        attn = self.f32(B, d.H, T_run, d.M) if want_attn else None
        g = None
        if grad_views is not None:
            g = ComicDecoderGrads()
            for f in GRAD_FIELDS:
                t = grad_views.get(f)
                setattr(g, f, None if t is None else C.c_void_p(t.data_ptr()))
        mk = None
        if masks is not None:
            mk = ComicTrainMasks()
            for f in ('init_in', 'inp', 'out', 'att'):
                t = masks.get(f)
                setattr(mk, f, None if t is None else C.c_void_p(t.data_ptr()))
            mk.in_keep, mk.out_keep, mk.att_keep = [float(x) for x in keeps]
        n = C.c_size_t()
        self._check(self.lib.comic_train_workspace_bytes(self._h, B, T_run, C.byref(n)))
        ws = self._ws.get('train')
        if ws is None or ws.numel() < n.value:
            ws = self._ws['train'] = torch.empty(n.value, dtype=torch.uint8, device=self.device)
        self._check(self.lib.comic_train_fwd_bwd(
            self._h, _ptr(fm), _ptr(im_embed), B, _ptr(inputs_tm), _ptr(targets_tm), _ptr(coef_tm), _ptr(lens), T,
            int(T_run), None if mk is None else C.byref(mk), float(map_loss_scale), _ptr(loss), _ptr(logits),
            _ptr(attn), None if g is None else C.byref(g), _ptr(ws), ws.numel(), self.stream()))
        return loss, logits, attn

    def encode_train(self, images):
        torch = self.torch
        images = images.contiguous()
        if images.dim() != 4 or tuple(images.shape[1:]) != (224, 224, 3):
            raise ValueError('images must be [B,224,224,3] NHWC, got %s' % (tuple(images.shape),))
        B = images.shape[0]
        nt, nw = C.c_size_t(), C.c_size_t()
        self._check(self.lib.comic_encode_train_bytes(self._h, B, C.byref(nt), C.byref(nw)))
        for key, n in (('enc_tape', nt.value), ('enc_train_ws', nw.value)):
            if self._ws.get(key) is None or self._ws[key].numel() < n:
                self._ws[key] = torch.empty(n, dtype=torch.uint8, device=self.device)
        tape, ws = self._ws['enc_tape'], self._ws['enc_train_ws']
        fm = self.f32(B, self.dims.M, self.dims.C)
        emb = self.f32(B, self.dims.E)
        self._check(self.lib.comic_encode_train_fwd(self._h, _ptr(images), B, _ptr(fm), _ptr(emb), _ptr(tape),
                                                    tape.numel(), _ptr(ws), ws.numel(), self.stream()))
        return emb, fm

    def train_encoder_grads(self, B, T_run):
        dfm = self.f32(B, self.dims.M, self.dims.C)
        demb = self.f32(B, self.dims.E)
        ws = self._ws['train']
        self._check(self.lib.comic_train_encoder_grads(self._h, B, int(T_run), _ptr(dfm), _ptr(demb), _ptr(ws),
                                                       ws.numel(), self.stream()))
        return dfm, demb

    def legacy_head_bwd(self, mixed5c, d_im_embed, d_gamma, d_beta, d_weight):
        B = mixed5c.shape[0]
        n = C.c_size_t()
        self._check(self.lib.comic_legacy_head_bwd_bytes(self._h, B, C.byref(n)))
        ws = self._ws.get('legacy_head')
        if ws is None or ws.numel() < n.value:
            ws = self._ws['legacy_head'] = self.torch.empty(n.value, dtype=self.torch.uint8, device=self.device)
        self._check(self.lib.comic_legacy_head_bwd(self._h, _ptr(mixed5c.contiguous()), B, _ptr(d_im_embed.contiguous()),
                                                   _ptr(d_gamma), _ptr(d_beta), _ptr(d_weight), _ptr(ws), ws.numel(),
                                                   self.stream()))

    def encode_bwd(self, images, dfm, dim_embed, conv_grads, beta_grads):
        B = images.shape[0]
        g = ComicCnnGrads()
# ... 42 lines not shown
```

### include/comic_b200.h

```cpp
#ifndef COMIC_B200_H_
#define COMIC_B200_H_

#include <stddef.h>
#include <stdint.h>

#ifdef __cplusplus
extern "C" {
#endif

#define COMIC_OK             0
#define COMIC_E_BADARG      -1
#define COMIC_E_SHAPE       -2
#define COMIC_E_CUDA        -3
#define COMIC_E_UNSUPPORTED -4
#define COMIC_E_WORKSPACE   -5

#define COMIC_NUM_CONVS 57

typedef struct comic_handle_s* comic_handle_t;

typedef struct {
  int32_t rnn_size;
  int32_t word_size;
  int32_t num_heads;
  int32_t fm_channels;
  int32_t fm_positions;
  int32_t embed_size;
  int32_t vocab;
  int32_t fm_projection;
  int32_t context_layer;
  int32_t init_method;
  int32_t alignment;
  int32_t prob_fn;
  int32_t embed_lookup;
  int32_t legacy;
  int32_t go_id, eos_id;
} comic_cfg_t;

typedef struct {
  const float* lstm_kernel;
  const float* lstm_bias;
  const float* init_weight;
  const float* memory_kernel;
  const float* value_kernel;
  const float* query_kernel;
  const float* attention_v;
  const float* ln_gamma;
  const float* ln_beta;
  const float* temperature;
  const float* a_layer;
  const float* out_kernel;
  const float* out_bias;
  const float* embedding_map;
  const float* enc_ln_gamma;
  const float* enc_ln_beta;
  const float* enc_embed_weight;
  const float* conv_w[COMIC_NUM_CONVS];
  const float* bn_beta[COMIC_NUM_CONVS];
  const float* bn_mean[COMIC_NUM_CONVS];
  const float* bn_var[COMIC_NUM_CONVS];
} comic_weights_t;

typedef struct { int32_t k, stride, c_in, c_out; } comic_conv_desc_t;

const char* comic_last_error(void);
const char* comic_version(void);

const comic_conv_desc_t* comic_conv_table(void);

int comic_create(const comic_cfg_t* cfg, comic_handle_t* out);
int comic_destroy(comic_handle_t h);

int comic_packed_bytes(comic_handle_t h, size_t* bytes);
int comic_bind_weights(comic_handle_t h, const comic_weights_t* w, int with_cnn,
                       void* packed, size_t packed_bytes, void* stream);

int comic_set_precision(comic_handle_t h, int mode);

#define COMIC_OPT_FUSED_ATTN_MIN_IMAGES 0
#define COMIC_OPT_ENC_CHUNK_STEM 1
#define COMIC_OPT_ENC_CHUNK_28 2
#define COMIC_OPT_ENC_CHUNK_14 3
#define COMIC_OPT_PERSISTENT_MAX_ROWS 4
#define COMIC_OPT_PERSISTENT_TRACE 5
#define COMIC_OPT_ENC_PLANES 6
#define COMIC_OPT_GEMM_PAIR 7
#define COMIC_OPT_GEMM_PAIR_MIN_TILES 8
#define COMIC_OPT_STEM_S2D 9
#define COMIC_OPT_GEMM_RESIDENT_B 10
#define COMIC_OPT_ATTN2 12
#define COMIC_OPT_FUSE_LSTM 13
#define COMIC_OPT_TMA_A 15
#define COMIC_OPT_GEMM_SMALL_TILES 16
#define COMIC_OPT_PDL 17
#define COMIC_OPT_PERSISTENT_WATCHDOG_MS 18
#define COMIC_OPT_TC_SPLITK 19
#define COMIC_OPT_GEMM_MC 14
#define COMIC_OPT_TC_MIN_ROWS 11
int comic_set_option(comic_handle_t h, int option, int value);

int comic_decode_trace(comic_handle_t h, int64_t* out, int max_steps, int* steps, void* stream);

int comic_workspace_bytes(comic_handle_t h, int mode, int B, int k, int T, size_t* bytes);

int comic_encode_fwd(comic_handle_t h, const float* images, int B, float* fm_out,
                     float* im_embed_out, float* mixed5c_out, void* ws, size_t ws_bytes,
                     void* stream);

int comic_preprocess_eval(comic_handle_t h, const uint8_t* images, int B, int H, int W, int out_h, int out_w,
                          float* out, void* stream);

int comic_preprocess_train(comic_handle_t h, const uint8_t* images, int B, int H, int W, int out_h, int out_w,
                           const int32_t* crop_yx, const uint8_t* flip, float* out, void* stream);

int comic_project_fm(comic_handle_t h, const float* fm, int B, float* keys_out,
                     float* values_out, void* stream);

int comic_rnn_init(comic_handle_t h, const float* im_embed, int B, float* c0, float* h0,
                   const float* in_mask, float in_keep, void* ws, size_t ws_bytes, void* stream);

int comic_decode_step(comic_handle_t h, const float* keys, const float* values, int B, int k,
                      const int32_t* tokens, const float* c_in, const float* h_in,
                      const float* ctx_in, float* c_out, float* h_out, float* ctx_out,
                      float* align_out, float* logits_out,
                      const float* in_mask, const float* out_mask, const float* att_mask,
                      float in_keep, float out_keep, float att_keep,
                      void* ws, size_t ws_bytes, void* stream);

int comic_decode_greedy(comic_handle_t h, const float* keys, const float* values,
                        const float* c0, const float* h0, int B, int max_it,
                        int32_t* ids_out, float* logits_out, float* attn_out, int32_t* T_out,
                        void* ws, size_t ws_bytes, void* stream);

int comic_decode_beam(comic_handle_t h, const float* keys, const float* values,
                      const float* c0, const float* h0, int B, int k, float length_penalty_weight,
                      int max_it, int32_t* pred_ids_out, int32_t* step_ids_out,
                      int32_t* parent_ids_out, float* scores_out, int64_t* lengths_out,
                      float* attn_top_out, int32_t* T_out, void* ws, size_t ws_bytes, void* stream);

int comic_beam_step(comic_handle_t h, const float* logits, int ld_logits, int B, int k, int V,
                    int eos_id, float length_penalty_weight, float* log_probs,
                    uint8_t* finished, int64_t* lengths, float* scores_out,
                    int32_t* word_out, int32_t* parent_out, void* stream);

int comic_gather_tree(comic_handle_t h, const int32_t* step_ids, const int32_t* parent_ids,
                      const int32_t* max_seq_len, int T, int B, int k, int end_token,
                      int32_t* out, void* stream);

int comic_gemm_f32(comic_handle_t h, const float* A, int lda, const float* Bm, int ldb,
                   const float* bias, float* C, int ldc, int M, int N, int K,
                   void* ws, size_t ws_bytes, void* stream);



typedef struct {
  const float* init_in;
  const float* inp;
  const float* out;
  const float* att;
  float in_keep, out_keep, att_keep;
} comic_train_masks_t;

typedef struct {
  float* lstm_kernel; float* lstm_bias; float* init_weight; float* memory_kernel; float* value_kernel;
  float* query_kernel; float* attention_v; float* ln_gamma; float* ln_beta; float* temperature;
  float* out_kernel; float* out_bias; float* embedding_map;
  float* a_layer;
} comic_decoder_grads_t;

int comic_train_workspace_bytes(comic_handle_t h, int B, int T_run, size_t* bytes);

int comic_dropout_masks(comic_handle_t h, float* out, size_t n, float keep, uint64_t seed, uint64_t stream_id,
                        void* stream);

int comic_train_fwd_bwd(comic_handle_t h, const float* fm, const float* im_embed, int B,
                        const int32_t* inputs_tm, const int32_t* targets_tm, const float* coef_tm,
                        const int32_t* lens, int T, int T_run, const comic_train_masks_t* masks,
                        float map_loss_scale, float* loss_out, float* logits_out, float* attn_out,
                        const comic_decoder_grads_t* grads, void* ws, size_t ws_bytes, void* stream);

int comic_train_encoder_grads(comic_handle_t h, int B, int T_run, float* dfm_out, float* dim_embed_out,
                              void* ws, size_t ws_bytes, void* stream);

int comic_legacy_head_bwd_bytes(comic_handle_t h, int B, size_t* bytes);
int comic_legacy_head_bwd(comic_handle_t h, const float* mixed5c, int B, const float* d_im_embed, float* d_gamma,
                          float* d_beta, float* d_weight, void* ws, size_t ws_bytes, void* stream);

typedef struct {
  float* conv_w[COMIC_NUM_CONVS];
  float* bn_beta[COMIC_NUM_CONVS];
} comic_cnn_grads_t;

int comic_encode_train_bytes(comic_handle_t h, int B, size_t* tape_bytes, size_t* ws_bytes);

int comic_encode_train_fwd(comic_handle_t h, const float* images, int B, float* fm_out, float* im_embed_out,
                           void* tape, size_t tape_bytes, void* ws, size_t ws_bytes, void* stream);

int comic_encode_bwd(comic_handle_t h, const float* images, int B, const float* dfm, const float* dim_embed,
                     const void* tape, size_t tape_bytes, const comic_cnn_grads_t* grads, void* ws,
                     size_t ws_bytes, void* stream);

int comic_l2_regularise(comic_handle_t h, const float* params, float* grads, size_t n, float decay,
                        float* reg_out, void* ws, size_t ws_bytes, void* stream);

int comic_adam_step(comic_handle_t h, float* params, const float* grads, float* m, float* v, size_t n,
                    float lr, float beta1, float beta2, float eps, int step, float grad_scale, void* stream);

int comic_momentum_step(comic_handle_t h, float* params, const float* grads, float* accum, size_t n, float lr,
                        float momentum, float grad_scale, void* stream);

int comic_clip_by_norm(comic_handle_t h, float* grads, const int64_t* offsets, const int64_t* sizes, int nvars,
                       float max_norm, void* stream);

int comic_refresh_packed(comic_handle_t h, void* packed, size_t packed_bytes, void* stream);
int comic_refresh_packed_cnn(comic_handle_t h, void* packed, size_t packed_bytes, void* stream);

int comic_launch_count(comic_handle_t h, int64_t* count);

int comic_profile_enable(comic_handle_t h, uint32_t tag_mask);
int comic_profile_read(comic_handle_t h, int tag, double* total_ms, int64_t* count);

#ifdef __cplusplus
}
#endif
#endif
```

Before: 29310.

## Add TMA halo-tile implicit-GEMM path for stride-1 3x3 encoder convs

Adds a new A-operand mode in which each CTA loads a spatial halo band (rows plus one-pixel border) of pre-split bf16 hi/lo activation planes via 4D TMA into a shared-memory ring, then issues tcgen05 MMAs directly over it instead of gathering im2col rows. The producing 1x1 convs and grouped GEMMs now write bf16 hi/lo planes straight from their epilogue, so the 3x3 conv input needs no separate split pass. This is meant to cut redundant global reads and im2col address work for the 3x3 convs in the 56 and 28/14 stages. It adds a large shared-memory ring, constraints on width and channel count, and a new standalone conv_layer API.

```diff
diff --git a/comic-compact-image-captioning-with-attention_b200/csrc/api.cu b/comic-compact-image-captioning-with-attention_b200/csrc/api.cu
--- a/comic-compact-image-captioning-with-attention_b200/csrc/api.cu
+++ b/comic-compact-image-captioning-with-attention_b200/csrc/api.cu
@@ -149,6 +149,7 @@
       h->persist_watchdog_ms = value;
       return COMIC_OK;
     case COMIC_OPT_ENC_PLANES: h->enc_planes = value; return COMIC_OK;
+    case COMIC_OPT_CONV_HALO: h->conv_halo = value; return COMIC_OK;
     case COMIC_OPT_STEM_S2D: h->stem_s2d = value; return COMIC_OK;
     case COMIC_OPT_TC_MIN_ROWS: h->tc_min_rows = value; return COMIC_OK;
     case COMIC_OPT_TC_SPLITK: h->tc_splitk = value; return COMIC_OK;
diff --git a/comic-compact-image-captioning-with-attention_b200/csrc/comic_internal.cuh b/comic-compact-image-captioning-with-attention_b200/csrc/comic_internal.cuh
--- a/comic-compact-image-captioning-with-attention_b200/csrc/comic_internal.cuh
+++ b/comic-compact-image-captioning-with-attention_b200/csrc/comic_internal.cuh
@@ -83,6 +83,7 @@
   int tc_splitk = 3;
   int tc_min_rows = 64;
   int stem_s2d = 2;
+  int conv_halo = 1;
   int enc_planes = 0;
   int enc_chunk[3] = {256, 512, 512};
   comic::Packed pk;
@@ -159,12 +160,13 @@
 };
 void same_pads(int n, int k, int s, int* out, int* before);
 int run_conv(comic_handle_t h, const float* x, int B, int H, int W, int ldx, int ci, float* dst, int ld_dst, int coff,
-             int* Ho_out, int* Wo_out, cudaStream_t st);
+             int* Ho_out, int* Wo_out, cudaStream_t st, uint16_t* dhi = nullptr, uint16_t* dlo = nullptr);
 int run_maxpool(comic_handle_t h, const float* x, float* y, int B, int H, int W, int C, int k, int s, int* Ho_out,
                 int* Wo_out, cudaStream_t st);
 void run_pad_c3_c4(comic_handle_t h, const float* img, float* dst, size_t npix, cudaStream_t st);
 void run_avgpool_global(comic_handle_t h, const float* x, float* y, int B, int HW, int C, cudaStream_t st);
-int run_block(comic_handle_t h, int bi, const float* x, float* y, int B, int S, EncBufs& eb, cudaStream_t st);
+int run_block(comic_handle_t h, int bi, const float* x, float* y, int B, int S, EncBufs& eb, cudaStream_t st,
+              bool halo = false);
 
 struct StepBufs {
   float* gates;
diff --git a/comic-compact-image-captioning-with-attention_b200/csrc/encoder.cu b/comic-compact-image-captioning-with-attention_b200/csrc/encoder.cu
--- a/comic-compact-image-captioning-with-attention_b200/csrc/encoder.cu
+++ b/comic-compact-image-captioning-with-attention_b200/csrc/encoder.cu
@@ -28,6 +28,8 @@
   for (int i = 0; i < 6; ++i) b.conv[i] = first + i;
   return b;
 }
+
+static bool halo3_conv(int ci) { return ci >= 2 && ci < 3 + 6 * 7 && kConvs[ci].k == 3 && kConvs[ci].stride == 1; }
 
 static BlockDesc kBlocks[kNumBlocks];
 static bool kBlocksInit = false;
@@ -260,18 +262,6 @@
 }
 
 
-struct Planes {
-  uint16_t* hi;
-  uint16_t* lo;
-};
-
-static inline Planes planes_of(float* buf, size_t cap_elems) {
-  Planes p;
-  p.hi = reinterpret_cast<uint16_t*>(buf);
-  p.lo = p.hi + cap_elems;
-  return p;
-}
-static inline Planes planes_at(Planes p, size_t off) { return Planes{p.hi + off, p.lo + off}; }
 
 __device__ __forceinline__ void unpack8(const uint4& h, const uint4& l, float (&v)[8]) {
   const uint32_t hw[4] = {h.x, h.y, h.z, h.w}, lw[4] = {l.x, l.y, l.z, l.w};
@@ -422,8 +412,47 @@
   return COMIC_OK;
 }
 
+struct Planes {
+  uint16_t* hi;
+  uint16_t* lo;
+};
+
+static inline Planes planes_of(float* buf, size_t cap_elems) {
+  Planes p;
+  p.hi = reinterpret_cast<uint16_t*>(buf);
+  p.lo = p.hi + cap_elems;
+  return p;
+}
+static inline Planes planes_at(Planes p, size_t off) { return Planes{p.hi + off, p.lo + off}; }
+
+static int run_conv_halo(comic_handle_t h, Planes x, int B, int S, int ci, float* dst, int ld_dst, int coff,
+                         cudaStream_t st) {
+  const comic_conv_desc_t& d = kConvs[ci];
+  AHalo3 a;
+  COMIC_REQUIRE(tc::make_halo3(a, x.hi, x.lo, B, S, S, d.c_in, d.c_in), COMIC_E_CUDA,
+                "conv %d: halo tensor maps (%d x %d x %d) could not be encoded", ci, S, S, d.c_in);
+  Epi e{};
+  e.bias = h->pk.bn_shift[ci];
+  e.scale = h->pk.bn_scale[ci];
+  e.relu = 1;
+  e.nroute = 1;
+  e.r[0] = Route{0, d.c_out, dst, ld_dst, coff};
+  cudaError_t err;
+  {
+    Prof pf(h, T_CONV, st);
+    err = tc::launch_halo3(a, h->pk.tc_conv[ci], d.c_out, e, h->num_sms, st);
+  }
+  COMIC_CHECK_CUDA(err);
+  return COMIC_OK;
+}
+
+static bool use_halo3(comic_handle_t h, int ci, int M, int S) {
+  return h->conv_halo && halo3_conv(ci) && use_tc(h, h->pk.tc_conv[ci], M) &&
+         tc::halo3_fits(kConvs[ci].c_out, S, kConvs[ci].c_in);
+}
+
 int run_conv(comic_handle_t h, const float* x, int B, int H, int W, int ldx, int ci, float* dst,
-                    int ld_dst, int coff, int* Ho_out, int* Wo_out, cudaStream_t st) {
+                    int ld_dst, int coff, int* Ho_out, int* Wo_out, cudaStream_t st, uint16_t* dhi, uint16_t* dlo) {
   const comic_conv_desc_t& d = kConvs[ci];
   AConv a;
   a.x = x; a.H = H; a.W = W; a.Cin = (d.c_in == 3 && ldx == 4) ? 4 : d.c_in; a.ldx = ldx;
@@ -436,7 +465,7 @@
   e.scale = h->pk.bn_scale[ci];
   e.relu = 1;
   e.nroute = 1;
-  e.r[0] = Route{0, N, dst, ld_dst, coff};
+  e.r[0] = Route{0, N, dst, ld_dst, coff, dhi, dlo};
   e.split_stride = 0;
   GemmPlan p = plan_gemm(M, N, K, h->num_sms, false);
   cudaError_t err;
@@ -445,6 +474,7 @@
     err = tc::launch_gemm_tc<1>(a, h->pk.tc_conv[ci], M, N, e, h->num_sms, st);
   } else {
     Prof pf(h, T_CONV, st);
+    COMIC_REQUIRE(dhi == nullptr, COMIC_E_UNSUPPORTED, "conv %d: bf16-plane output needs the tensor path", ci);
     if (d.c_in % 4 == 0) err = launch_gemm<1, 4>(a, h->w.conv_w[ci], N, M, N, K, e, p, st);
     else err = launch_gemm<1, 1>(a, h->w.conv_w[ci], N, M, N, K, e, p, st);
   }
@@ -491,10 +521,14 @@
 }
 
 int run_block(comic_handle_t h, int bi, const float* x, float* y, int B, int S, EncBufs& eb,
-                     cudaStream_t st) {
+                     cudaStream_t st, bool halo) {
   const BlockDesc& bd = block_table()[bi];
   int cout = bd.b0 + bd.b1b + bd.b2b + bd.b3;
   int M = B * S * S;
+  const bool grp_tc = use_tc(h, h->pk.tc_grp[bi], M);
+  const bool h1 = halo && grp_tc && use_halo3(h, bd.conv[2], M, S);
+  const bool h2 = halo && grp_tc && use_halo3(h, bd.conv[4], M, S);
+  const Planes p1 = planes_of(eb.t1, (size_t)M * bd.b1a), p2 = planes_of(eb.t2, (size_t)M * bd.b2a);
   {
     APlain a{};
     a.nseg = 1;
@@ -506,20 +540,24 @@
     e.relu = 1;
     e.nroute = 3;
     e.r[0] = Route{0, bd.b0, y, cout, 0};
-    e.r[1] = Route{bd.b0, bd.b0 + bd.b1a, eb.t1, bd.b1a, 0};
-    e.r[2] = Route{bd.b0 + bd.b1a, ng, eb.t2, bd.b2a, 0};
+    e.r[1] = h1 ? Route{bd.b0, bd.b0 + bd.b1a, nullptr, bd.b1a, 0, p1.hi, p1.lo} : Route{bd.b0, bd.b0 + bd.b1a, eb.t1, bd.b1a, 0};
+    e.r[2] = h2 ? Route{bd.b0 + bd.b1a, ng, nullptr, bd.b2a, 0, p2.hi, p2.lo} : Route{bd.b0 + bd.b1a, ng, eb.t2, bd.b2a, 0};
     GemmPlan p = plan_gemm(M, ng, bd.cin, h->num_sms, false);
     cudaError_t err;
     {
       Prof pf(h, T_CONV, st);
-      if (use_tc(h, h->pk.tc_grp[bi], M)) err = tc::launch_gemm_tc<0>(a, h->pk.tc_grp[bi], M, ng, e, h->num_sms, st);
+      if (grp_tc) err = tc::launch_gemm_tc<0>(a, h->pk.tc_grp[bi], M, ng, e, h->num_sms, st);
       else err = launch_gemm<0, 4>(a, h->pk.grp_w[bi], ng, M, ng, bd.cin, e, p, st);
     }
     COMIC_CHECK_CUDA(err);
   }
   int rc;
-  if ((rc = run_conv(h, eb.t1, B, S, S, bd.b1a, bd.conv[2], y, cout, bd.b0, nullptr, nullptr, st))) return rc;
-  if ((rc = run_conv(h, eb.t2, B, S, S, bd.b2a, bd.conv[4], y, cout, bd.b0 + bd.b1b, nullptr, nullptr, st))) return rc;
+  if (h1) rc = run_conv_halo(h, p1, B, S, bd.conv[2], y, cout, bd.b0, st);
+  else rc = run_conv(h, eb.t1, B, S, S, bd.b1a, bd.conv[2], y, cout, bd.b0, nullptr, nullptr, st);
+  if (rc) return rc;
+  if (h2) rc = run_conv_halo(h, p2, B, S, bd.conv[4], y, cout, bd.b0 + bd.b1b, st);
+  else rc = run_conv(h, eb.t2, B, S, S, bd.b2a, bd.conv[4], y, cout, bd.b0 + bd.b1b, nullptr, nullptr, st);
+  if (rc) return rc;
   if ((rc = run_maxpool(h, x, eb.p, B, S, S, bd.cin, 3, 1, nullptr, nullptr, st))) return rc;
   if ((rc = run_conv(h, eb.p, B, S, S, bd.cin, bd.conv[5], y, cout, bd.b0 + bd.b1b + bd.b2b, nullptr, nullptr, st))) return rc;
   return COMIC_OK;
@@ -750,26 +788,33 @@
       if ((rc = run_conv(h, img, nb, 224, 224, 3, 0, eb.a, 64, 0, &Ho, &Wo, st))) return rc;
     }
     if ((rc = run_maxpool(h, eb.a, eb.b, nb, 112, 112, 64, 3, 2, &Ho, &Wo, st))) return rc;
-    if ((rc = run_conv(h, eb.b, nb, 56, 56, 64, 1, eb.a, 64, 0, nullptr, nullptr, st))) return rc;
-    if ((rc = run_conv(h, eb.a, nb, 56, 56, 64, 2, eb.b, 192, 0, nullptr, nullptr, st))) return rc;
+    const int m56 = nb * 56 * 56;
+    if (use_halo3(h, 2, m56, 56) && use_tc(h, h->pk.tc_conv[1], m56)) {
+      const Planes c2b = planes_of(eb.a, (size_t)m56 * 64);
+      if ((rc = run_conv(h, eb.b, nb, 56, 56, 64, 1, nullptr, 64, 0, nullptr, nullptr, st, c2b.hi, c2b.lo))) return rc;
+      if ((rc = run_conv_halo(h, c2b, nb, 56, 2, eb.b, 192, 0, st))) return rc;
+    } else {
+      if ((rc = run_conv(h, eb.b, nb, 56, 56, 64, 1, eb.a, 64, 0, nullptr, nullptr, st))) return rc;
+      if ((rc = run_conv(h, eb.a, nb, 56, 56, 64, 2, eb.b, 192, 0, nullptr, nullptr, st))) return rc;
+    }
     if ((rc = run_maxpool(h, eb.b, pool2 + (size_t)b0 * 28 * 28 * 192, nb, 56, 56, 192, 3, 2, nullptr, nullptr, st)))
       return rc;
   }
   for (int b0 = 0; b0 < B; b0 += pl.c3) {
     int nb = (B - b0 < pl.c3) ? (B - b0) : pl.c3;
-    if ((rc = run_block(h, 0, pool2 + (size_t)b0 * 28 * 28 * 192, eb.b, nb, 28, eb, st))) return rc;
-    if ((rc = run_block(h, 1, eb.b, eb.a, nb, 28, eb, st))) return rc;
+    if ((rc = run_block(h, 0, pool2 + (size_t)b0 * 28 * 28 * 192, eb.b, nb, 28, eb, st, true))) return rc;
+    if ((rc = run_block(h, 1, eb.b, eb.a, nb, 28, eb, st, true))) return rc;
     if ((rc = run_maxpool(h, eb.a, pool3 + (size_t)b0 * 14 * 14 * 480, nb, 28, 28, 480, 3, 2, nullptr, nullptr, st)))
       return rc;
   }
   for (int b0 = 0; b0 < B; b0 += pl.c4) {
     int nb = (B - b0 < pl.c4) ? (B - b0) : pl.c4;
-    if ((rc = run_block(h, 2, pool3 + (size_t)b0 * 14 * 14 * 480, eb.a, nb, 14, eb, st))) return rc;
-    if ((rc = run_block(h, 3, eb.a, eb.b, nb, 14, eb, st))) return rc;
-    if ((rc = run_block(h, 4, eb.b, eb.a, nb, 14, eb, st))) return rc;
-    if ((rc = run_block(h, 5, eb.a, eb.b, nb, 14, eb, st))) return rc;
+    if ((rc = run_block(h, 2, pool3 + (size_t)b0 * 14 * 14 * 480, eb.a, nb, 14, eb, st, true))) return rc;
+    if ((rc = run_block(h, 3, eb.a, eb.b, nb, 14, eb, st, true))) return rc;
+    if ((rc = run_block(h, 4, eb.b, eb.a, nb, 14, eb, st, true))) return rc;
+    if ((rc = run_block(h, 5, eb.a, eb.b, nb, 14, eb, st, true))) return rc;
     float* fm = fm_out + (size_t)b0 * 196 * 832;
-    if ((rc = run_block(h, 6, eb.b, fm, nb, 14, eb, st))) return rc;
+    if ((rc = run_block(h, 6, eb.b, fm, nb, 14, eb, st, true))) return rc;
     if ((rc = run_maxpool(h, fm, eb.a, nb, 14, 14, 832, 2, 2, nullptr, nullptr, st))) return rc;
     if ((rc = run_block(h, 7, eb.a, eb.b, nb, 7, eb, st))) return rc;
     float* m5c = mixed5c_out ? mixed5c_out + (size_t)b0 * 49 * 1024 : eb.a;
@@ -869,3 +914,38 @@
 }
 
 extern "C" const comic_conv_desc_t* comic_conv_table(void) { return comic::conv_table(); }
+
+namespace comic {
+__global__ void split_planes_kernel(const float* __restrict__ x, uint16_t* __restrict__ hi, uint16_t* __restrict__ lo,
+                                    size_t n4) {
+  const size_t i = (size_t)blockIdx.x * blockDim.x + threadIdx.x;
+  if (i >= n4) return;
+  uint2 h, l;
+  tc::split4(reinterpret_cast<const float4*>(x)[i], h, l);
+  reinterpret_cast<uint2*>(hi)[i] = h;
+  reinterpret_cast<uint2*>(lo)[i] = l;
+}
+}
+
+extern "C" int comic_conv_layer(comic_handle_t h, int conv, const float* x, int B, int S, float* y, void* ws,
+                                size_t ws_bytes, void* stream) {
+  using namespace comic;
+  COMIC_REQUIRE(h && x && y, COMIC_E_BADARG, "conv_layer: null argument");
+  COMIC_REQUIRE(h->cnn_bound, COMIC_E_BADARG, "conv_layer: CNN weights not bound");
+  COMIC_REQUIRE(conv >= 0 && conv < COMIC_NUM_CONVS && kConvs[conv].k == 3 && kConvs[conv].stride == 1, COMIC_E_BADARG,
+                "conv_layer: conv %d is not a stride-1 3x3 conv", conv);
+  COMIC_REQUIRE(B > 0 && S > 0, COMIC_E_SHAPE, "conv_layer: bad shape B=%d S=%d", B, S);
+  const comic_conv_desc_t& d = kConvs[conv];
+  cudaStream_t st = (cudaStream_t)stream;
+  const int M = B * S * S;
+  if (use_halo3(h, conv, M, S)) {
+    const size_t n = (size_t)M * d.c_in;
+    COMIC_REQUIRE(ws && ws_bytes >= n * 4, COMIC_E_WORKSPACE, "conv_layer: workspace %zu < %zu", ws_bytes, n * 4);
+    const Planes p = planes_of(static_cast<float*>(ws), n);
+    split_planes_kernel<<<(unsigned)((n / 4 + 255) / 256), 256, 0, st>>>(x, p.hi, p.lo, n / 4);
+    h->launches++;
+    COMIC_CHECK_CUDA(cudaGetLastError());
+    return run_conv_halo(h, p, B, S, conv, y, d.c_out, 0, st);
+  }
+  return run_conv(h, x, B, S, S, d.c_in, conv, y, d.c_out, 0, nullptr, nullptr, st);
+}
diff --git a/comic-compact-image-captioning-with-attention_b200/csrc/gemm_f32.cuh b/comic-compact-image-captioning-with-attention_b200/csrc/gemm_f32.cuh
--- a/comic-compact-image-captioning-with-attention_b200/csrc/gemm_f32.cuh
+++ b/comic-compact-image-captioning-with-attention_b200/csrc/gemm_f32.cuh
@@ -106,6 +106,14 @@
   CUtensorMap hi, lo;
 };
 template <> struct AParam<4> { typedef ATma type; };
+struct AHalo3 {
+  CUtensorMap hi, lo;
+  int nimg, H, W, Wp, rpt, tpi;
+  int groups;
+  int cps;
+  int nslots;
+};
+template <> struct AParam<5> { typedef AHalo3 type; };
 
 __device__ __forceinline__ float4 ldg4(const float* p) {
   return __ldg(reinterpret_cast<const float4*>(p));
diff --git a/comic-compact-image-captioning-with-attention_b200/csrc/gemm_tc.cuh b/comic-compact-image-captioning-with-attention_b200/csrc/gemm_tc.cuh
--- a/comic-compact-image-captioning-with-attention_b200/csrc/gemm_tc.cuh
+++ b/comic-compact-image-captioning-with-attention_b200/csrc/gemm_tc.cuh
@@ -67,6 +67,13 @@
       ::"r"(smem_dst), "l"(reinterpret_cast<uint64_t>(tm)), "r"(smem_u32(bar)), "r"(c0), "r"(c1)
       : "memory");
 }
+__device__ __forceinline__ void tma_load_4d(uint32_t smem_dst, const CUtensorMap* tm, uint64_t* bar, int c0, int c1,
+                                            int c2, int c3) {
+  asm volatile(
+      "cp.async.bulk.tensor.4d.shared::cluster.global.mbarrier::complete_tx::bytes [%0], [%1, {%3, %4, %5, %6}], [%2];"
+      ::"r"(smem_dst), "l"(reinterpret_cast<uint64_t>(tm)), "r"(smem_u32(bar)), "r"(c0), "r"(c1), "r"(c2), "r"(c3)
+      : "memory");
+}
 __device__ __forceinline__ void umma_bf16(uint32_t tmem_d, uint64_t adesc, uint64_t bdesc, uint32_t idesc,
                                           uint32_t accumulate) {
   asm volatile(
@@ -102,6 +109,15 @@
   d |= (uint64_t)(1024 >> 4) << 32;
   d |= (uint64_t)1 << 46;
   d |= (uint64_t)2 << 61;
+  return d;
+}
+
+__device__ __forceinline__ uint64_t make_desc_noswz(uint32_t smem_addr, uint32_t lbo, uint32_t sbo) {
+  uint64_t d = 0;
+  d |= (uint64_t)((smem_addr >> 4) & 0x3FFF);
+  d |= (uint64_t)((lbo >> 4) & 0x3FFF) << 16;
+  d |= (uint64_t)((sbo >> 4) & 0x3FFF) << 32;
+  d |= (uint64_t)1 << 46;
   return d;
 }
 
@@ -185,18 +201,25 @@
 constexpr int kHaloPlaneBytes = ((kHaloRows * kHaloCols * 32 + 127) / 128) * 128;
 constexpr int kHaloBytes = 2 * 2 * kHaloPlaneBytes;
 
-template <int BN, int STAGES, bool PAIR, int NKRES = 0, bool HALO = false>
+constexpr int kMaxHaloSlots = 16;
+constexpr int kHaloTail = 512;
+constexpr int kSmemMax = 232448;
+
+template <int BN, int STAGES, bool PAIR, int NKRES = 0, bool HALO = false, bool CONV_HALO = false>
 struct SmemLayout {
   static constexpr int B_TILE_BYTES = (PAIR ? BN / 2 : BN) * BK * 2;
-  static constexpr int STAGE_BYTES = 2 * A_TILE_BYTES + (NKRES ? 0 : 2 * B_TILE_BYTES);
+  static constexpr int A_STAGE_BYTES = CONV_HALO ? 0 : 2 * A_TILE_BYTES;
+  static constexpr int STAGE_BYTES = A_STAGE_BYTES + (NKRES ? 0 : 2 * B_TILE_BYTES);
   static constexpr int PANEL_OFF = STAGES * STAGE_BYTES;
   static constexpr int TILES_BYTES = PANEL_OFF + NKRES * 2 * B_TILE_BYTES;
-  static constexpr int ROWTAB_BYTES = BM * 3 * 8;
-  static constexpr int BAR_BYTES = ((3 * STAGES + 4) * 8 + 8 + 15) & ~15;
+  static constexpr int ROWTAB_BYTES = CONV_HALO ? 0 : BM * 3 * 8;
+  static constexpr int BAR_BYTES = ((3 * STAGES + 4 + (CONV_HALO ? 2 * kMaxHaloSlots : 0)) * 8 + 8 + 15) & ~15;
   static constexpr int EPI_STRIDE = 20;
   static constexpr int EPI_BYTES = kEpiWarps * 32 * EPI_STRIDE * 4;
-  static constexpr int HALO_OFF = TILES_BYTES + kLoaderGroups * ROWTAB_BYTES + BAR_BYTES + EPI_BYTES;
-  static constexpr int TOTAL = HALO_OFF + (HALO ? kHaloBytes : 0) + 1024;
+  static constexpr int HALO_ALIGN = CONV_HALO ? 128 : 1;
+  static constexpr int HALO_OFF = (TILES_BYTES + kLoaderGroups * ROWTAB_BYTES + BAR_BYTES + EPI_BYTES + HALO_ALIGN - 1) & ~(HALO_ALIGN - 1);
+  static constexpr int CHALO_RING = CONV_HALO ? ((kSmemMax - 1024 - HALO_OFF - 128 - kHaloTail) & ~127) : 0;
+  static constexpr int TOTAL = HALO_OFF + (HALO ? kHaloBytes : 0) + (CONV_HALO ? 128 + CHALO_RING + kHaloTail : 0) + 1024;
   static constexpr int TMEM_COLS = (2 * BN <= 32) ? 32 : (2 * BN <= 64) ? 64 : (2 * BN <= 128) ? 128 : (2 * BN <= 256) ? 256 : 512;
 };
 
@@ -209,7 +232,9 @@
   constexpr bool CL = PAIR || MC > 1;
   constexpr uint16_t kMcMask = (uint16_t)((1u << MC) - 1u);
   static_assert(AMODE != 3 || (NKRES > 0 && BN == 64), "halo loader: resident-panel stem kernel only");
-  using L = SmemLayout<BN, STAGES, PAIR, NKRES, AMODE == 3>;
+  static_assert(AMODE != 5 || (!PAIR && NKRES == 0 && MC == 1), "3x3 conv halo: plain kernel only");
+  using L = SmemLayout<BN, STAGES, PAIR, NKRES, AMODE == 3, AMODE == 5>;
+  static_assert(L::TOTAL <= kSmemMax, "tile ring + halo exceed the shared memory of an SM");
   constexpr int TM = (PAIR ? 2 : MC) * BM;
   constexpr int MMA_M = PAIR ? 2 * BM : BM;
   extern __shared__ uint8_t smem_raw[];
@@ -224,13 +249,17 @@
   uint64_t* tmem_full = bars + 3 * STAGES;
   uint64_t* tmem_empty = bars + 3 * STAGES + 2;
   uint32_t* tmem_slot = reinterpret_cast<uint32_t*>(bars + 3 * STAGES + 4);
+  uint64_t* halo_full = bars + 3 * STAGES + 5;
+  uint64_t* halo_empty = halo_full + kMaxHaloSlots;
+  const uint32_t halo_ring = smem + L::HALO_OFF + 128;
 
   const int tid = threadIdx.x, warp = tid >> 5, lane = tid & 31;
   const uint32_t rank = CL ? cluster_ctarank() : 0u;
   const bool leader = PAIR ? rank == 0 : true;
   const int nk = (K + BK - 1) / BK;
   const int n_tiles = (N + BN - 1) / BN;
-  const int m_tiles = (M + TM - 1) / TM;
+  int m_tiles = (M + TM - 1) / TM;
+  if constexpr (AMODE == 5) m_tiles = a.nimg * a.tpi;
   const int ksplit = (AMODE == 0 && !PAIR && MC == 1 && NKRES == 0 && epi.ksplit > 1) ? epi.ksplit : 1;
   const int mn_tiles = m_tiles * n_tiles;
   const int total_tiles = mn_tiles * ksplit;
@@ -246,6 +275,12 @@
     for (int i = 0; i < 2; ++i) {
       mbar_init(&tmem_full[i], 1);
       mbar_init(&tmem_empty[i], PAIR ? 2 * kEpiWarps : kEpiWarps);
+    }
+    if constexpr (AMODE == 5) {
+      for (int s = 0; s < kMaxHaloSlots; ++s) {
+        mbar_init(&halo_full[s], 1);
+        mbar_init(&halo_empty[s], 1);
+      }
     }
     fence_barrier_init();
   }
@@ -295,6 +330,11 @@
         if constexpr (AMODE == 3) {
           const int r = quad * 32 + row;
           return (t_img * 112 + t_y0 + (r >> 4)) * 112 + t_x0 + (r & 15);
+        } else if constexpr (AMODE == 5) {
+          const int mt = mn / n_tiles, img = mt / a.tpi, band = mt - img * a.tpi;
+          const int r = quad * 32 + row, yl = r / a.Wp, xp = r - yl * a.Wp, y = band * a.rpt + yl;
+          if (yl >= a.rpt || y >= a.H || xp < 1 || xp > a.W) return M;
+          return (img * a.H + y) * a.W + xp - 1;
         } else {
           return mw + row;
         }
@@ -316,6 +356,9 @@
           for (int q = 0; q < 4; ++q) if (cprow[q]) cp_next[q] = __ldg(cprow[q] + u0);
         }
       }
+      int mrow[4];
+#pragma unroll
+      for (int q = 0; q < 4; ++q) mrow[q] = row_to_m(q * 8 + srow);
 #pragma unroll 1
       for (int c0 = half * 16; c0 < n_umma; c0 += 32) {
         uint32_t r[16];
@@ -356,7 +399,7 @@
 #pragma unroll
             for (int q = 0; q < 4; ++q) {
               const int row = q * 8 + srow;
-              const int m = row_to_m(row);
+              const int m = mrow[q];
               if (m < M) {
                 const float4 v = *reinterpret_cast<const float4*>(stage_buf + row * L::EPI_STRIDE + scol);
                 const float cp = cp_cur[q];
@@ -372,7 +415,7 @@
 #pragma unroll
           for (int q = 0; q < 4; ++q) {
             const int row = q * 8 + srow;
-            const int m = row_to_m(row);
+            const int m = mrow[q];
             if (m < M) {
               float4 v = *reinterpret_cast<const float4*>(stage_buf + row * L::EPI_STRIDE + scol);
               if (epi.scale) { v.x *= sc.x; v.y *= sc.y; v.z *= sc.z; v.w *= sc.w; }
@@ -403,7 +446,7 @@
   } else if (warp == kMmaWarp) {
     if (leader && lane == 0) {
       int iter = 0;
-      uint32_t it = 0;
+      uint32_t it = 0, hts = 0;
       if constexpr (NKRES > 0) mbar_wait(&full_b[0], 0);
       for (int tile = first_tile; tile < total_tiles; tile += tile_step, ++iter) {
         const int kz = tile / mn_tiles, mn = tile - kz * mn_tiles;
@@ -416,6 +459,42 @@
         if constexpr (PAIR) mbar_wait_cluster(&tmem_empty[acc], (uint32_t)(((iter >> 1) & 1) ^ 1));
         else mbar_wait(&tmem_empty[acc], (uint32_t)(((iter >> 1) & 1) ^ 1));
         tc_fence_after();
+        if constexpr (AMODE == 5) {
+          const uint32_t cps = (uint32_t)a.cps, nslots = (uint32_t)a.nslots;
+          const uint64_t lo_step = (uint64_t)((2u * cps) >> 4), bl_step = (uint64_t)(L::B_TILE_BYTES >> 4);
+          const uint64_t piece_step = (uint64_t)((4u * cps) >> 4);
+          const uint64_t dah_base = make_desc_noswz(halo_ring - 16u, cps, 128);
+          const int G = a.groups, nsl = 9 * G;
+          const uint32_t slot0 = hts % nslots;
+          int sl = 0;
+          uint64_t db = 0;
+          uint32_t s = 0;
+#pragma unroll
+          for (int tap = 0; tap < 9; ++tap) {
+            const uint64_t toff = (uint64_t)(((tap / 3) * a.Wp + tap % 3) * 16 >> 4);
+            uint32_t slot = slot0;
+            for (int g = 0; g < G; ++g, ++sl) {
+              if (tap == 0) {
+                mbar_wait(&halo_full[slot], ((hts + (uint32_t)g) / nslots) & 1);
+                tc_fence_after();
+              }
+              if ((sl & 3) == 0) {
+                s = it % STAGES;
+                mbar_wait(&full_b[s], (it / STAGES) & 1);
+                tc_fence_after();
+                db = make_desc_sw128(smem + s * L::STAGE_BYTES);
+              }
+              const uint64_t dah = dah_base + slot * piece_step + toff, dbh = db + (uint64_t)((sl & 3) * 2);
+              umma_bf16(d_tmem, dah, dbh, idesc, sl > 0 ? 1u : 0u);
+              umma_bf16(d_tmem, dah + lo_step, dbh, idesc, 1u);
+              umma_bf16(d_tmem, dah, dbh + bl_step, idesc, 1u);
+              if ((sl & 3) == 3 || sl == nsl - 1) { umma_commit(&empty[s]); ++it; }
+              if (tap == 8) umma_commit(&halo_empty[slot]);
+              if (++slot == nslots) slot = 0;
+            }
+          }
+          hts += (uint32_t)G;
+        } else
         for (int kt = kt0; kt < kt1; ++kt, ++it) {
           const int s = it % STAGES;
           const uint32_t ph = (it / STAGES) & 1;
@@ -479,7 +558,7 @@
           const int s = it % STAGES;
           const uint32_t ph = (it / STAGES) & 1;
           mbar_wait(&empty[s], ph ^ 1);
-          const uint32_t b_hi = smem + s * L::STAGE_BYTES + 2 * A_TILE_BYTES;
+          const uint32_t b_hi = smem + s * L::STAGE_BYTES + L::A_STAGE_BYTES;
           const uint32_t b_lo = b_hi + L::B_TILE_BYTES;
           if constexpr (PAIR) {
             if (leader) mbar_arrive_expect_tx(&full_b[s], 4 * L::B_TILE_BYTES);
@@ -509,6 +588,27 @@
     __syncwarp();
   } else {
     if constexpr (AMODE == 4) {
+    } else if constexpr (AMODE == 5) {
+      if (warp == kFirstLoaderWarp && lane == 0) {
+        const uint32_t cps = (uint32_t)a.cps;
+        const uint32_t box_bytes = (uint32_t)(a.Wp * (a.rpt + 2) * 16);
+        uint32_t hts = 0;
+        for (int tile = first_tile; tile < total_tiles; tile += tile_step) {
+          const int mt = tile / n_tiles, img = mt / a.tpi, band = mt - img * a.tpi;
+          const int y0 = band * a.rpt - 1;
+          for (int g = 0; g < a.groups; ++g, ++hts) {
+            const int hs = (int)(hts % (uint32_t)a.nslots);
+            mbar_wait(&halo_empty[hs], ((hts / (uint32_t)a.nslots) & 1) ^ 1);
+            mbar_arrive_expect_tx(&halo_full[hs], 4u * box_bytes);
+            const uint32_t dst = halo_ring + (uint32_t)hs * 4u * cps;
+            tma_load_4d(dst, &a.hi, &halo_full[hs], g * 16, -1, y0, img);
+            tma_load_4d(dst + cps, &a.hi, &halo_full[hs], g * 16 + 8, -1, y0, img);
+            tma_load_4d(dst + 2u * cps, &a.lo, &halo_full[hs], g * 16, -1, y0, img);
+            tma_load_4d(dst + 3u * cps, &a.lo, &halo_full[hs], g * 16 + 8, -1, y0, img);
+          }
+        }
+      }
+      __syncwarp();
     } else if constexpr (AMODE == 3) {
       const int lw = warp - kFirstLoaderWarp;
       const int tg = lw * 32 + lane;
@@ -938,6 +1038,70 @@
   return cudaGetLastError();
 }
 
+inline bool make_halo3(AHalo3& a, const uint16_t* hi, const uint16_t* lo, int nimg, int H, int W, int Cin, int ldx) {
+  a.nimg = nimg; a.H = H; a.W = W; a.Wp = W + 2;
+  a.rpt = BM / a.Wp;
+  if (a.rpt < 1 || Cin % 16 || ldx % 8) return false;
+  a.tpi = (H + a.rpt - 1) / a.rpt;
+  a.groups = Cin / 16;
+  a.cps = (a.Wp * (a.rpt + 2) * 16 + 127) & ~127;
+  a.nslots = 0;
+  EncodeTiledFn enc = get_encode_fn();
+  if (!enc) return false;
+  cuuint64_t dims[4] = {(cuuint64_t)Cin, (cuuint64_t)W, (cuuint64_t)H, (cuuint64_t)nimg};
+  cuuint64_t strides[3] = {(cuuint64_t)ldx * 2, (cuuint64_t)W * ldx * 2, (cuuint64_t)H * W * ldx * 2};
+  cuuint32_t box[4] = {8, (cuuint32_t)a.Wp, (cuuint32_t)(a.rpt + 2), 1};
+  cuuint32_t estr[4] = {1, 1, 1, 1};
+  CUresult r1 = enc(&a.hi, CU_TENSOR_MAP_DATA_TYPE_BFLOAT16, 4, const_cast<uint16_t*>(hi), dims, strides, box, estr,
+                    CU_TENSOR_MAP_INTERLEAVE_NONE, CU_TENSOR_MAP_SWIZZLE_NONE, CU_TENSOR_MAP_L2_PROMOTION_L2_128B,
+                    CU_TENSOR_MAP_FLOAT_OOB_FILL_NONE);
+  CUresult r2 = enc(&a.lo, CU_TENSOR_MAP_DATA_TYPE_BFLOAT16, 4, const_cast<uint16_t*>(lo), dims, strides, box, estr,
+                    CU_TENSOR_MAP_INTERLEAVE_NONE, CU_TENSOR_MAP_SWIZZLE_NONE, CU_TENSOR_MAP_L2_PROMOTION_L2_128B,
+                    CU_TENSOR_MAP_FLOAT_OOB_FILL_NONE);
+  return r1 == CUDA_SUCCESS && r2 == CUDA_SUCCESS;
+}
+
+template <int BN, int STAGES>
+inline cudaError_t launch_halo3_bn(AHalo3 a, const TcWeight& w, int bn_idx, int N, const Epi& epi, int num_sms,
+                                   cudaStream_t st) {
+  using L = SmemLayout<BN, STAGES, false, 0, false, true>;
+  static_assert(L::TOTAL <= kSmemMax, "3x3 halo kernel exceeds the shared memory of an SM");
+  a.nslots = L::CHALO_RING / (4 * a.cps);
+  if (a.nslots > kMaxHaloSlots) a.nslots = kMaxHaloSlots;
+  if (a.nslots < a.groups) return cudaErrorInvalidValue;
+  static PerDeviceOnce once;
+  {
+    cudaError_t e = once([&] { return cudaFuncSetAttribute(gemm_bf16x3_kernel<BN, STAGES, 5>,
+                                         cudaFuncAttributeMaxDynamicSharedMemorySize, L::TOTAL); });
+    if (e != cudaSuccess) return e;
+  }
+  const int tiles = ((N + BN - 1) / BN) * a.nimg * a.tpi;
+  const int grid = tiles < num_sms ? tiles : num_sms;
+  gemm_bf16x3_kernel<BN, STAGES, 5><<<grid, kThreads, L::TOTAL, st>>>(a, w.tm_hi[bn_idx], w.tm_lo[bn_idx],
+                                                                      a.nimg * a.H * a.W, N, w.K, epi);
+  return cudaGetLastError();
+}
+
+inline cudaError_t launch_halo3(const AHalo3& a, const TcWeight& w, int N, const Epi& epi, int num_sms, cudaStream_t st) {
+  if (N > 256) return cudaErrorInvalidValue;
+  if (N <= 64) return launch_halo3_bn<64, 4>(a, w, 0, N, epi, num_sms, st);
+  if (N <= 128) return launch_halo3_bn<128, 3>(a, w, 1, N, epi, num_sms, st);
+  if (N <= 192) return launch_halo3_bn<192, 2>(a, w, 4, N, epi, num_sms, st);
+  return launch_halo3_bn<256, 2>(a, w, 2, N, epi, num_sms, st);
+}
+
+inline bool halo3_fits(int N, int W, int Cin) {
+  const int Wp = W + 2, rpt = BM / Wp;
+  if (N > 256 || rpt < 1 || Cin % 16) return false;
+  const int ring = N <= 64 ? SmemLayout<64, 4, false, 0, false, true>::CHALO_RING
+                 : N <= 128 ? SmemLayout<128, 3, false, 0, false, true>::CHALO_RING
+                 : N <= 192 ? SmemLayout<192, 2, false, 0, false, true>::CHALO_RING
+                            : SmemLayout<256, 2, false, 0, false, true>::CHALO_RING;
+  const int cps = (Wp * (rpt + 2) * 16 + 127) & ~127;
+  const int slots = ring / (4 * cps);
+  return Cin / 16 <= (slots < kMaxHaloSlots ? slots : kMaxHaloSlots);
+}
+
 inline int& bres_mode() { static int v = 1; return v; }
 
 template <int BN, int STAGES, int AMODE>
diff --git a/comic-compact-image-captioning-with-attention_b200/engine.py b/comic-compact-image-captioning-with-attention_b200/engine.py
--- a/comic-compact-image-captioning-with-attention_b200/engine.py
+++ b/comic-compact-image-captioning-with-attention_b200/engine.py
@@ -74,6 +74,7 @@
     'comic_bind_weights': (_I, [_P, C.POINTER(ComicWeights), _I, _P, _SZ, _P]),
     'comic_workspace_bytes': (_I, [_P, _I, _I, _I, _I, C.POINTER(_SZ)]),
     'comic_encode_fwd': (_I, [_P, _P, _I, _P, _P, _P, _P, _SZ, _P]),
+    'comic_conv_layer': (_I, [_P, _I, _P, _I, _I, _P, _P, _SZ, _P]),
     'comic_preprocess_eval': (_I, [_P, _P, _I, _I, _I, _I, _I, _P, _P]),
     'comic_project_fm': (_I, [_P, _P, _I, _P, _P, _P]),
     'comic_rnn_init': (_I, [_P, _P, _I, _P, _P, _P, _F, _P, _SZ, _P]),
@@ -287,6 +288,15 @@
                                               _ptr(ws), ws.numel(), self.stream()))
         return (emb, fm, m5c) if want_mixed5c else (emb, fm)
 
+    def conv_layer(self, conv, x):
+        x = x.contiguous()
+        B, S, cout = x.shape[0], x.shape[1], self.lib.comic_conv_table()[conv].c_out
+        y = self.f32(B, S, S, cout)
+        ws = self.torch.empty(x.numel(), dtype=self.torch.float32, device=x.device)
+        self._check(self.lib.comic_conv_layer(self._h, int(conv), _ptr(x), B, S, _ptr(y), _ptr(ws), ws.numel() * 4,
+                                              self.stream()))
+        return y
+
     def preprocess_eval(self, images_u8, out_hw=(224, 224)):
         torch = self.torch
         images_u8 = images_u8.contiguous()
@@ -423,7 +433,7 @@
         self._check(self.lib.comic_set_precision(self._h, {'f32': 0, 'tf32x3': 1, 'split': 1, 'fast': 2}[mode]))
 
     def set_option(self, name, value):
-        self._check(self.lib.comic_set_option(self._h, {'fused_attn_min_images': 0, 'enc_chunk_stem': 1, 'enc_chunk_28': 2, 'enc_chunk_14': 3, 'persistent_max_rows': 4, 'persistent_trace': 5, 'enc_planes': 6, 'gemm_pair': 7, 'gemm_pair_min_tiles': 8, 'stem_s2d': 9, 'gemm_resident_b': 10, 'tc_min_rows': 11, 'attn2': 12, 'fuse_lstm': 13, 'gemm_mc': 14, 'tma_a': 15, 'gemm_small_tiles': 16, 'pdl': 17, 'persistent_watchdog_ms': 18, 'tc_splitk': 19}[name], int(value)))
+        self._check(self.lib.comic_set_option(self._h, {'fused_attn_min_images': 0, 'enc_chunk_stem': 1, 'enc_chunk_28': 2, 'enc_chunk_14': 3, 'persistent_max_rows': 4, 'persistent_trace': 5, 'enc_planes': 6, 'gemm_pair': 7, 'gemm_pair_min_tiles': 8, 'stem_s2d': 9, 'gemm_resident_b': 10, 'tc_min_rows': 11, 'attn2': 12, 'fuse_lstm': 13, 'gemm_mc': 14, 'tma_a': 15, 'gemm_small_tiles': 16, 'pdl': 17, 'persistent_watchdog_ms': 18, 'tc_splitk': 19, 'conv_halo': 20}[name], int(value)))
 
     def decode_trace(self, max_steps=256):
         import numpy as np
diff --git a/include/comic_b200.h b/include/comic_b200.h
--- a/include/comic_b200.h
+++ b/include/comic_b200.h
@@ -96,8 +96,12 @@
 #define COMIC_OPT_PERSISTENT_WATCHDOG_MS 18
 #define COMIC_OPT_TC_SPLITK 19
 #define COMIC_OPT_GEMM_MC 14
+#define COMIC_OPT_CONV_HALO 20
 #define COMIC_OPT_TC_MIN_ROWS 11
 int comic_set_option(comic_handle_t h, int option, int value);
+
+int comic_conv_layer(comic_handle_t h, int conv, const float* x, int B, int S, float* y, void* ws, size_t ws_bytes,
+                     void* stream);
 
 int comic_decode_trace(comic_handle_t h, int64_t* out, int max_steps, int* steps, void* stream);
 
```

Measured after the change: 28570, median of 6. -2.5%, worse.
